# AdrienC21/CCSD

Measured on AMD Instinct MI355X. Metric: sampled complexes/sec at 1000 PC steps, QM9_CC batch=1024, 1/2/4/8 GPU, higher is better.
Workload: dtype f32; 1 GPU; qm9_CC N=9 F=4 E=36 K=466, B=1024 per GPU, VE x3, Reverse+Langevin snr=0.2 scale_eps=0.7 n_steps=1, 1000 scales; global_batch=1024, parallelism=batch-sharded x1, per-shard Langevin norms, all-gather at end, finite=True

## Files before the change

### ccsd_amd/_lib.py

```python
from __future__ import annotations

import ctypes as C
import os
from typing import Optional

HERE = os.path.dirname(os.path.abspath(__file__))
HIP_LIB_PATH = os.path.join(HERE, "libccsd_hip.so")

ABI_VERSION = 5
OK, ERR_INVALID, ERR_UNSUPPORTED, ERR_WEIGHTS, ERR_RUNTIME, ERR_WORKSPACE = range(6)
SDE_VP, SDE_VE, SDE_SUBVP = 0, 1, 2
PRED_EULER, PRED_REVERSE, PRED_S4 = 0, 1, 2
CORR_NONE, CORR_LANGEVIN = 0, 1
TARGET_X, TARGET_ADJ, TARGET_RANK2 = 0, 1, 2

EXPORTS = [
    "ccsd_plan_create", "ccsd_plan_destroy", "ccsd_weight_count", "ccsd_rank2_dims", "ccsd_workspace_bytes",
    "ccsd_last_error", "ccsd_score", "ccsd_init_state", "ccsd_corrector_norms", "ccsd_corrector_apply",
    "ccsd_predictor", "ccsd_s4_apply", "ccsd_sampler_run", "ccsd_quantize", "ccsd_rank2_cells", "ccsd_profile_kernel", "ccsd_profile_stride", "ccsd_profile_read", "ccsd_profile_launches", "ccsd_debug_stamps",
    "ccsd_noise_draws", "ccsd_plan_query",
]
QUERIES = {"fused_r2": 0, "xa_variant": 1, "r2_lds_bytes": 2, "xa_lds_bytes": 3, "fused_loop": 4, "merged_r2": 5, "ew1": 6, "large_graph": 7,
           "r2_family": 8, "r2_instance": 9, "loop_form": 10, "h_full": 11, "hp_full": 12, "p0_narrow": 13, "tiled_fuse": 14, "ew1_fuse": 15,
           "h_general": 16, "geo_ek": 17}
KERNEL_IDS = {"k_xa": 0, "k_gemm_p": 1, "k_hf_score": 2, "k_gemm_h": 3, "k_langevin_apply": 4, "k_r2": 5, "k_s4_apply": 6, "k_ew1": 7}


class StepCoef(C.Structure):
    _fields_ = [(n, C.c_float) for n in ("sscale", "alpha", "pa", "pb", "pc", "m1", "s1", "d", "m2", "s2")]


class Config(C.Structure):
    _fields_ = (
        [(n, C.c_int32) for n in (
            "abi_version", "N", "F", "is_cc", "d_min", "d_max",
            "x_depth", "x_nhid",
            "a_num_layers", "a_num_linears", "a_c_init", "a_c_hid", "a_c_final", "a_nhid", "a_adim", "a_num_heads",
            "a_is_cc_net", "h_num_layers", "h_num_linears", "h_nhid", "h_adim", "h_c_hid", "h_c_final", "h_num_heads",
            "f_num_layers", "f_num_linears", "f_nhid", "f_c_hid", "f_c_final", "f_cnum", "f_num_layers_mlp",
            "f_use_hodge_mask",
            "predictor", "corrector", "n_corr_steps", "probability_flow", "denoise")]
        + [("snr", C.c_float), ("scale_eps", C.c_float), ("diff_steps", C.c_int32), ("batch_hint", C.c_int32)]
        + [(n, C.c_int32) for n in ("x_gmh", "x_num_linears", "x_c_init", "x_c_hid", "x_c_final", "x_adim", "x_num_heads",
                                    "a_conv_mlp", "x_conv_mlp")]
    )


class State(C.Structure):
    _fields_ = [("x", C.c_void_p), ("adj", C.c_void_p), ("rank2", C.c_void_p)]


class Noise(C.Structure):
    _fields_ = [("zx", C.c_void_p), ("zadj", C.c_void_p), ("zrank2", C.c_void_p)]


class CcsdError(RuntimeError):
    pass


def raise_status(lib, status: int):
    if status == OK:
        return
    msg = lib.ccsd_last_error().decode("utf-8", "replace")
    if status == ERR_UNSUPPORTED:
        raise NotImplementedError(msg)
    if status in (ERR_INVALID, ERR_WEIGHTS, ERR_WORKSPACE):
        raise ValueError(msg)
    raise CcsdError(msg)


class Library:

    def __init__(self, path: str, is_hip: bool):
        if not os.path.exists(path):
            raise FileNotFoundError(path)
        self.path = path
        self.is_hip = is_hip
        L = self.c = C.CDLL(path)
        vp, i32, i64, u64, f32, sz = C.c_void_p, C.c_int32, C.c_int64, C.c_uint64, C.c_float, C.c_size_t
        P = C.POINTER
        L.ccsd_plan_create.argtypes = [P(Config), P(C.c_float), sz, P(StepCoef), P(vp)]
        L.ccsd_plan_create.restype = C.c_int
        L.ccsd_plan_destroy.argtypes = [vp]
        L.ccsd_plan_destroy.restype = None
        L.ccsd_weight_count.argtypes = [P(Config)]
        L.ccsd_weight_count.restype = sz
        L.ccsd_rank2_dims.argtypes = [P(Config), P(i32), P(i64)]
        L.ccsd_rank2_dims.restype = None
        L.ccsd_workspace_bytes.argtypes = [vp, i32]
        L.ccsd_workspace_bytes.restype = sz
        L.ccsd_last_error.argtypes = []
        L.ccsd_last_error.restype = C.c_char_p
        L.ccsd_score.argtypes = [vp, i32, i32, P(State), vp, f32, vp, vp, sz, vp]
        L.ccsd_score.restype = C.c_int
        L.ccsd_init_state.argtypes = [vp, i32, vp, P(Noise), u64, i64, P(State), vp]
        L.ccsd_init_state.restype = C.c_int
        L.ccsd_corrector_norms.argtypes = [vp, i32, i32, i32, P(State), P(State), vp, P(Noise), u64, i64, vp, vp, sz, vp]
        L.ccsd_corrector_norms.restype = C.c_int
        L.ccsd_corrector_apply.argtypes = [vp, i32, i32, i32, P(State), vp, P(Noise), u64, i64, vp, P(State), vp, sz, vp]
        L.ccsd_corrector_apply.restype = C.c_int
        L.ccsd_predictor.argtypes = [vp, i32, i32, P(State), vp, P(Noise), u64, i64, P(State), P(State), vp, sz, vp]
        L.ccsd_predictor.restype = C.c_int
        L.ccsd_s4_apply.argtypes = [vp, i32, i32, P(State), vp, P(Noise), P(Noise), P(Noise), u64, i64, vp, P(State), P(State), vp, sz, vp]
        L.ccsd_s4_apply.restype = C.c_int
        L.ccsd_sampler_run.argtypes = [vp, i32, vp, u64, i64, i32, i32, P(State), P(State), P(State), vp, vp, sz, vp]
        L.ccsd_sampler_run.restype = C.c_int
        L.ccsd_quantize.argtypes = [vp, i64, f32, vp, vp]
        L.ccsd_quantize.restype = C.c_int
        L.ccsd_rank2_cells.argtypes = [vp, i32, i32, i64, f32, vp, vp, vp]
        L.ccsd_rank2_cells.restype = C.c_int
        L.ccsd_profile_kernel.argtypes = [vp, i32]
        L.ccsd_profile_kernel.restype = C.c_int
        L.ccsd_profile_stride.argtypes = [vp, i32]
        L.ccsd_profile_stride.restype = C.c_int
        L.ccsd_profile_read.argtypes = [vp, i32, P(i64), P(C.c_double)]
        L.ccsd_profile_read.restype = C.c_int
        L.ccsd_profile_launches.argtypes = [vp, i32, P(i64)]
        L.ccsd_profile_launches.restype = C.c_int
        L.ccsd_debug_stamps.argtypes = [vp, vp]
        L.ccsd_debug_stamps.restype = C.c_int
        L.ccsd_noise_draws.argtypes = [vp, i32, vp, u64, i64, i32, i32, P(State), vp]
        L.ccsd_noise_draws.restype = C.c_int
        L.ccsd_plan_query.argtypes = [vp, i32, P(i64)]
        L.ccsd_plan_query.restype = C.c_int

    def __getattr__(self, name):
        return getattr(self.c, name)

    def check(self, status: int):
        raise_status(self.c, status)


_hip: Optional[Library] = None


def get_library() -> Library:
    global _hip
    if _hip is None:
        import torch

        path = os.environ.get("CCSD_LIB_PATH") or HIP_LIB_PATH
        if not os.path.exists(path):
            raise CcsdError(
                f"{path} is missing: build it with `python -c 'import __graft_entry__ as g; g.build()'` "
                "(hipcc --offload-arch=gfx950).  ccsd_amd has no CPU fallback."
            )
        _hip = Library(path, is_hip=True)
    return _hip
```

### ccsd_amd/csrc/ccsd_api.h

```cpp
#pragma once
#include "ccsd_kernels.h"
#define CCSD_INST_TABLES
#include "ccsd_instances.h"
#include <stdio.h>
#include <stdlib.h>
#include <string>
#include <vector>

static thread_local std::string g_last_error;
static int set_err(int st, const std::string& m) { g_last_error = m; return st; }

static inline int fnet_width(const PlanD& p) {
    int fw = p.f_fdim > p.f_cnum ? p.f_fdim : p.f_cnum;
    for (int l = 0; l < p.f_L; ++l) {
        const MlpD& m = p.fl[l];
        const int wd = m.n > 1 && m.hid > m.in ? (m.hid > m.out ? m.hid : m.out) : (m.in > m.out ? m.in : m.out);
        if (wd > fw) fw = wd;
    }
    if (p.f_fin.n > 1 && p.f_fin.hid > fw) fw = p.f_fin.hid;
    return fw;
}

struct Knobs {
    int no_fused_r2 = 0, hodge_general = 0, geo_off = 0, no_fused_apply = 0, no_h_full = 0, no_hp_full = 0, hp_full_norms = 0, split_bf16 = 0;
    int xa_threads = 0, xa_prio = 0, xa_stagger_mask = 0, xa_stagger_sleep = 0, r2_stagger_mask = 0, r2_stagger_sleep = 0;
    int lg_force = 0, xa_pass = -1, xa_gch = 0, no_mlp_wt = 0, verbose = 0;
    const char *dump_plan = nullptr, *dump_plan_name = nullptr;
};
static Knobs read_knobs() {
    Knobs k;
    auto on = [](const char* name) { return getenv(name) != nullptr; };
    k.no_fused_r2 = on("CCSD_NO_FUSED_R2"); k.hodge_general = on("CCSD_HODGE_GENERAL");
    k.geo_off = on("CCSD_NO_GEO") ? 1 : on("CCSD_NO_BAKE") ? 2 : 0;
    k.no_fused_apply = on("CCSD_NO_FUSED_APPLY"); k.no_h_full = on("CCSD_NO_H_FULL"); k.no_hp_full = on("CCSD_NO_HP_FULL");
    k.hp_full_norms = on("CCSD_HP_FULL_NORMS");
    if (const char* v = getenv("CCSD_SPLIT_BF16")) k.split_bf16 = atoi(v) == 3 ? 3 : 0;
    if (const char* v = getenv("CCSD_XA_THREADS")) { const int t = atoi(v); if (t >= 64 && t <= 1024 && t % 64 == 0) k.xa_threads = t; }
    if (const char* v = getenv("CCSD_XA_PRIO")) k.xa_prio = atoi(v);
    if (const char* v = getenv("CCSD_XA_STAGGER")) sscanf(v, "%d,%d", &k.xa_stagger_mask, &k.xa_stagger_sleep);
    if (const char* v = getenv("CCSD_R2_STAGGER")) sscanf(v, "%d,%d", &k.r2_stagger_mask, &k.r2_stagger_sleep);
    if (const char* v = getenv("CCSD_LARGE_GRAPH")) k.lg_force = atoi(v) == 1;
    if (const char* v = getenv("CCSD_XA_PASS")) k.xa_pass = atoi(v);
    k.xa_gch = on("CCSD_XA_GCH"); k.no_mlp_wt = on("CCSD_NO_MLP_WT"); k.verbose = on("CCSD_VERBOSE");
    k.dump_plan = getenv("CCSD_DUMP_PLAN"); k.dump_plan_name = getenv("CCSD_DUMP_PLAN_NAME");
    return k;
}

enum { R2_NONE = 0, R2_FUSED = 1, R2_EW1 = 2, R2_TILED = 3 };
enum { LOOP_PRED_ONLY = 0, LOOP_LANGEVIN = 1, LOOP_LANGEVIN_FUSED = 2, LOOP_S4 = 3, LOOP_STEPWISE = 4 };
struct Route {
    int lg = 0;
    int xa_variant = 0;
    const XaEntry* xa = nullptr;
    const XaEntry* xa_twin = nullptr;
    int xa_threads = 0;
    int r2_family = R2_NONE;
    const R2Entry* r2 = nullptr;
    int r2_ldk = 0, r2_ldh = 0;
    size_t r2_lds = 0;
    int h_general = 0;
    int geo = 0;
    int p0 = -1;
    int h_full = 0;
    unsigned hp_full_modes = 0;
    int loop = LOOP_PRED_ONLY;
    int merged = 0;
    int tiled_fuse = 0;
    int ew1_fuse = 0;
    int corrector_flat = 0, predictor_flat = 0;
};

struct ccsd_plan {
    ccsd_config_t cfg;
    PlanD h;
    PlanD* d = nullptr;
    float* w = nullptr;
    float* wp = nullptr;
    unsigned char* hpairs = nullptr;
    size_t npacked = 0;
    unsigned char* edges = nullptr;
    unsigned long long* cells = nullptr;
    std::vector<ccsd_step_coef_t> coef;
    size_t nweights = 0;
    long long* dbg = nullptr;
    unsigned long long* init_off = nullptr;
    size_t init_off_cap = 0;
    Knobs knobs;
    Route rt;
    unsigned prof_mask = 0;
    size_t prof_used[8] = {0, 0, 0, 0, 0, 0, 0, 0};
    int prof_stride = 1;
    size_t prof_calls[8] = {0, 0, 0, 0, 0, 0, 0, 0};
#ifndef CCSD_EMU
    std::vector<hipEvent_t> prof_ev[8];
#endif
};

enum { KID_XA = 0, KID_GEMM_P = 1, KID_HF = 2, KID_GEMM_H = 3, KID_LANGEVIN = 4, KID_R2 = 5, KID_S4 = 6, KID_EW1 = 7 };
static void prof_mark(ccsd_plan* pl, int kid, void* stream) {
#ifndef CCSD_EMU
    if (!(pl->prof_mask & (1u << kid))) return;
    const size_t call = pl->prof_calls[kid]++;
    if (pl->prof_stride > 1 && (call >> 1) % (size_t)pl->prof_stride != 0) return;
    std::vector<hipEvent_t>& ev = pl->prof_ev[kid];
    if (pl->prof_used[kid] == ev.size()) {
        hipEvent_t e;
        if (hipEventCreate(&e) != hipSuccess) return;
        ev.push_back(e);
    }
    (void)hipEventRecord(ev[pl->prof_used[kid]++], (hipStream_t)stream);
#else
    (void)pl; (void)kid; (void)stream;
#endif
}
#define RT_CHECK(expr)                                                                    \
    do {                                                                                  \
        rtError_t _e = (expr);                                                            \
        if (_e != RT_OK) return set_err(CCSD_ERR_RUNTIME, std::string(#expr) + ": " + rt_error_string(_e)); \
    } while (0)
#define LAUNCH_CHECK()                                                                    \
    do {                                                                                  \
        rtError_t _e = rt_last_error();                                                   \
        if (_e != RT_OK) return set_err(CCSD_ERR_RUNTIME, std::string("kernel launch: ") + rt_error_string(_e)); \
    } while (0)

static int resolve_route(ccsd_plan* pl) {
    const PlanD& p = pl->h;
    const ccsd_config_t& c = pl->cfg;
    const Knobs& k = pl->knobs;
    Route& r = pl->rt;
    const int E = p.E, K = p.K;
    const bool s4 = c.predictor == CCSD_PRED_S4, langevin = c.corrector == CCSD_CORR_LANGEVIN;
    unsigned char arch[sizeof(PlanD)];
    ccsd_plan_arch_bytes(p, arch);
    auto baked = [&](const unsigned char* plan, size_t size) { return size == sizeof(PlanD) && p.geo_off == 0 && memcmp(arch, plan, size) == 0; };

    bool conv_mlp = false;
    for (int l = 0; l < p.a_L; ++l) conv_mlp = conv_mlp || p.al[l].conv_mlp;
    if (p.x_gmh) for (int l = 0; l < p.x_depth; ++l) conv_mlp = conv_mlp || p.gl[l].conv_mlp;
    int v = p.hb_L ? XA_HB : p.x_gmh ? XA_GMH : XA_PLAIN;
    if (conv_mlp || (p.hb_L && p.x_gmh) || p.h_L > 2 || (!p.chan_global && !p.hb_L && p.a_fin.chain >= 5)) v = XA_GEN;
    if (v == XA_PLAIN && !p.chan_global && baked(CCSD_BAKED_QM9_PLAN, CCSD_BAKED_QM9_SIZE)) v = XA_BAKED9;
    else if (v == XA_PLAIN && p.chan_global && baked(CCSD_BAKED_CS_PLAN, CCSD_BAKED_CS_SIZE)) v = XA_BAKED20;
    else if (v == XA_PLAIN && p.chan_global && baked(CCSD_BAKED_Z_PLAN, CCSD_BAKED_Z_SIZE)) v = XA_BAKED38;
    else if (v == XA_GEN && !p.chan_global && baked(CCSD_BAKED_ENZ_PLAN, CCSD_BAKED_ENZ_SIZE)) v = XA_BAKEDENZ;
    else if (v == XA_PLAIN && p.geo_off != 1)
        for (const auto& g : XA_GEO_TABLE)
            if ((p.chan_global != 0) == (g.gch != 0) && p.N == g.N && (!g.F || p.F == g.F) && E == g.E && p.ldn == g.ldn) v = g.var;
    r.xa_variant = v;
    r.xa_threads = k.xa_threads;
    for (const XaEntry& e : XA_TABLE) {
        if ((e.gch != 0) != (p.chan_global != 0)) continue;
        if (e.var == v) r.xa = &e;
        if (e.var == XA_PLAIN) r.xa_twin = &e;
    }
    if (!r.xa || !r.xa_twin) return set_err(CCSD_ERR_RUNTIME, "k_xa variant " + std::to_string(v) + " has no instance in CCSD_XA_LIST");
    if (!r.xa->fixed256) r.xa_twin = nullptr;

    const bool aff = p.f_affine != 0, gen1 = p.h_L > 1 && p.hl[0].mval.n > 1;
    const int mt = (E + 15) / 16, rem = E & 15, rs = (!aff || rem == 0 || rem > 12) ? 0 : (rem + 3) / 4;
    auto r2_find = [&](int qm9) -> const R2Entry* {
        for (const R2Entry& e : R2_TABLE)
            if (e.mt == mt && e.rs == rs && (e.affine != 0) == aff && (e.gen1 != 0) == gen1 && e.qm9 == qm9) return &e;
        return nullptr;
    };
    bool fused = false;
    if (c.is_cc && E <= 64 && !k.no_fused_r2) {
        const int Kp4 = (K + 31) & ~31, Ep4 = (E + 3) & ~3;
        int ldk = Kp4; while ((ldk & 31) != 8 && (ldk & 31) != 24) ldk += 4;
        const int ldh = Ep4;
        const size_t fl = (size_t)E * ldk + (size_t)E * ldh + 64 * 2 + (size_t)p.a_cinit * E + 3 * c.N * c.N + 64 + (Kp4 + 3) / 4 + 4;
        if (fl * 4 + 64 <= 160 * 1024 && fnet_width(p) <= CCSD_FW && r2_find(0) && p.f_cnum <= 2) {
            fused = true; r.r2_ldk = ldk; r.r2_ldh = ldh; r.r2_lds = fl * 4;
            const bool qm9 = p.geo_off != 1 && !gen1 && E == CCSD_R2_QM9_E && K == CCSD_R2_QM9_K && p.N == CCSD_R2_QM9_N &&
                             ldk == CCSD_R2_QM9_LDK && ldh == CCSD_R2_QM9_LDH;
            r.r2 = r2_find(!qm9 ? 0 : aff && baked(CCSD_BAKED_QM9_PLAN, CCSD_BAKED_QM9_SIZE) ? 2 : 1);
            if (!r.r2) return set_err(CCSD_ERR_RUNTIME, "k_r2: the qm9-geometry instance is missing from CCSD_R2_LIST_*");
        }
    }
    if (p.h_L > 2) {
        bool affine_values = true;
        for (int l = 0; l + 1 < p.h_L; ++l) affine_values = affine_values && ccsd_hl(p, l).mval.n == 1;
        if (!affine_values || !fused || p.h_L > 4 || k.hodge_general) { r.h_general = 1; fused = false; r.r2 = nullptr; }
    }
    const bool ew1 = c.is_cc && !fused && aff && p.f_cnum == 1 && !s4;
    r.r2_family = !c.is_cc ? R2_NONE : fused ? R2_FUSED : ew1 ? R2_EW1 : R2_TILED;
    if (p.geo_off != 1) for (const GeoEntry& g : GEO_TABLE) if (E == g.E && K == g.K) r.geo = g.idx;
    if (p.h_L >= 1) {
        auto p0_find = [&](int kc) {
            for (int i = 0; i < (int)(sizeof(P0_TABLE) / sizeof(P0_TABLE[0])); ++i)
                if (P0_TABLE[i].nt == (p.hl[0].wc + 15) / 16 && P0_TABLE[i].kc == kc) return i;
            return -1;
        };
        if (p.geo_off != 1) r.p0 = p0_find(K);
        if (r.p0 < 0) r.p0 = p0_find(0);
    }
    r.tiled_fuse = r.r2_family == R2_TILED && p.h_L == 1 && (K & 3) == 0 && !s4 && langevin;
    r.ew1_fuse = ew1 && p.h_L == 1 && (K & 3) == 0 && langevin;
    const bool full_geo = c.is_cc && E == CCSD_FULL_E && K == CCSD_FULL_K && p.geo_off != 1 && !k.no_h_full;
    r.h_full = full_geo && r.r2_family == R2_TILED && p.f_cnum >= 2;

    const bool fused_apply = (fused || (ew1 && p.h_L <= 1) || r.tiled_fuse) && !k.no_fused_apply;
    r.loop = s4 ? LOOP_S4 : !langevin ? LOOP_PRED_ONLY : c.n_corr_steps != 1 ? LOOP_STEPWISE : fused_apply ? LOOP_LANGEVIN_FUSED : LOOP_LANGEVIN;
    if (full_geo && r.tiled_fuse && p.hl[0].wc <= 16 && p.f_cnum == 2 && !k.no_hp_full)
        r.hp_full_modes = (r.loop == LOOP_LANGEVIN_FUSED ? 1u << 2 : 0u) | (k.hp_full_norms ? 1u << 1 : 0u);
    r.merged = r.loop == LOOP_LANGEVIN_FUSED && fused && mt == 3 && rs == 1 && aff && !gen1 && (K & 1) == 0 && ((E * K) & 3) == 0;
    r.corrector_flat = !s4;
    r.predictor_flat = ew1;
    return CCSD_OK;
}
static inline bool use_h_full(const Route& r, int B) { return r.h_full && B >= 256; }
static inline bool use_hp_full(const Route& r, int B, int mode) { return B >= 256 && ((r.hp_full_modes >> mode) & 1u); }
#define HP_FULL_LDS ((size_t)(2 * 192 * H_LD + 2 * 16 * H_LD) * 4)
static inline const XaEntry* xa_launch(const Route& r, int B, int* threads) {
    const XaEntry* e = r.xa;
    int t = r.xa_threads;
    if (t == 0) t = e->max_threads == 256 ? 256 : B <= 256 ? 1024 : B <= 512 ? 512 : 256;
    if (e->fixed256 && t != 256) e = r.xa_twin;
    *threads = t > e->max_threads ? e->max_threads : t;
    return e;
}
static inline int normsum_threads(int B) { return B > 512 ? 1024 : B > 256 ? 512 : 256; }

extern "C" const char* ccsd_last_error(void) { return g_last_error.c_str(); }

extern "C" void ccsd_rank2_dims(const ccsd_config_t* cfg, int32_t* E, int64_t* K) {
    int e = 0; int64_t k = 0;
    if (cfg) ccsd_dims(cfg, &e, &k);
    if (E) *E = e;
    if (K) *K = k;
}

extern "C" size_t ccsd_weight_count(const ccsd_config_t* cfg) {
    PlanD p; PlanBuilder pb;
    size_t n = ccsd_build_plan(cfg, &p, pb);
    if (pb.status != CCSD_OK) { set_err(pb.status, pb.err); return 0; }
    return n;
}

extern "C" int ccsd_debug_stamps(ccsd_plan_t* plan, void* dev_buffer) {
    if (!plan) return set_err(CCSD_ERR_INVALID, "NULL plan");
    plan->dbg = (long long*)dev_buffer;
    return CCSD_OK;
}
extern "C" int ccsd_profile_kernel(ccsd_plan_t* plan, int32_t kernel_id) {
    if (!plan) return set_err(CCSD_ERR_INVALID, "NULL plan");
    if (kernel_id < 0) plan->prof_mask = 0;
    else if (kernel_id < 8) plan->prof_mask |= 1u << kernel_id;
    for (int k = 0; k < 8; ++k) { plan->prof_used[k] = 0; plan->prof_calls[k] = 0; }
    return CCSD_OK;
}
extern "C" int ccsd_profile_stride(ccsd_plan_t* plan, int32_t stride) {
    if (!plan || stride < 1) return set_err(CCSD_ERR_INVALID, "bad argument");
    plan->prof_stride = stride;
    for (int k = 0; k < 8; ++k) plan->prof_calls[k] = 0;
    return CCSD_OK;
}
extern "C" int ccsd_profile_launches(ccsd_plan_t* plan, int32_t kernel_id, int64_t* launches) {
    if (!plan || !launches || kernel_id < 0 || kernel_id >= 8) return set_err(CCSD_ERR_INVALID, "bad argument");
    *launches = (int64_t)(plan->prof_calls[kernel_id] >> 1);
    return CCSD_OK;
}
extern "C" int ccsd_profile_read(ccsd_plan_t* plan, int32_t kernel_id, int64_t* launches, double* total_ms) {
    if (!plan || !launches || !total_ms || kernel_id < 0 || kernel_id >= 8) return set_err(CCSD_ERR_INVALID, "bad argument");
    *launches = 0; *total_ms = 0.0;
#ifndef CCSD_EMU
    for (size_t i = 0; i + 1 < plan->prof_used[kernel_id]; i += 2) {
        float ms = 0.f;
        RT_CHECK(hipEventSynchronize(plan->prof_ev[kernel_id][i + 1]));
        RT_CHECK(hipEventElapsedTime(&ms, plan->prof_ev[kernel_id][i], plan->prof_ev[kernel_id][i + 1]));
        *total_ms += ms; *launches += 1;
    }
#endif
    plan->prof_used[kernel_id] = 0;
    return CCSD_OK;
}

extern "C" void ccsd_plan_destroy(ccsd_plan_t* plan) {
    if (!plan) return;
#ifndef CCSD_EMU
    for (int k = 0; k < 8; ++k) for (hipEvent_t e : plan->prof_ev[k]) (void)hipEventDestroy(e);
#endif
    if (plan->d) (void)rt_free(plan->d);
    if (plan->w) (void)rt_free(plan->w);
    if (plan->wp) (void)rt_free(plan->wp);
    if (plan->hpairs) (void)rt_free(plan->hpairs);
    if (plan->edges) (void)rt_free(plan->edges);
    if (plan->cells) (void)rt_free(plan->cells);
    if (plan->init_off) (void)rt_free(plan->init_off);
    delete plan;
}

extern "C" int ccsd_plan_create(const ccsd_config_t* cfg, const float* weights, size_t n_weights,
                                const ccsd_step_coef_t* step_coef, ccsd_plan_t** out) {
    if (!cfg || !weights || !step_coef || !out) return set_err(CCSD_ERR_INVALID, "NULL argument");
    *out = nullptr;
    ccsd_plan* pl = new ccsd_plan();
    pl->cfg = *cfg;
    const Knobs& k = pl->knobs = read_knobs();
    PlanBuilder pb;
    pb.lg_force = k.lg_force; pb.xa_pass = k.xa_pass; pb.xa_gch = k.xa_gch; pb.no_mlp_wt = k.no_mlp_wt; pb.verbose = k.verbose;
    pl->nweights = ccsd_build_plan(cfg, &pl->h, pb);
    if (pb.status != CCSD_OK) { delete pl; return set_err(pb.status, pb.err); }
    pl->rt.lg = pb.lg;
    pl->h.geo_off = k.geo_off;
    pl->npacked = (size_t)pb.pcur;
    if (pl->nweights != n_weights) {
        delete pl;
        return set_err(CCSD_ERR_WEIGHTS, "weight blob has " + std::to_string(n_weights) + " floats, config needs " +
                                             std::to_string(pl->nweights));
    }
    if (cfg->predictor != CCSD_PRED_EULER && cfg->predictor != CCSD_PRED_REVERSE && cfg->predictor != CCSD_PRED_S4) { delete pl; return set_err(CCSD_ERR_UNSUPPORTED, "unknown predictor"); }
    if (cfg->corrector != CCSD_CORR_NONE && cfg->corrector != CCSD_CORR_LANGEVIN) { delete pl; return set_err(CCSD_ERR_UNSUPPORTED, "unknown corrector"); }
    if (cfg->diff_steps < 1 || cfg->n_corr_steps < 0) { delete pl; return set_err(CCSD_ERR_INVALID, "bad step counts"); }
    ccsd_fold_fnet(&pl->h, weights);
    pl->coef.assign(step_coef, step_coef + (size_t)cfg->diff_steps * 3);
    const int N = cfg->N, E = pl->h.E, K = pl->h.K;
    std::vector<unsigned char> edges((size_t)2 * E + 2);
    {
        int e = 0;
        for (int i = 0; i < N; ++i)
            for (int j = i + 1; j < N; ++j) { edges[2 * e] = (unsigned char)i; edges[2 * e + 1] = (unsigned char)j; ++e; }
    }
    std::vector<unsigned long long> cells((size_t)K + 1);
    if (cfg->is_cc) {
        size_t c = 0;
        std::vector<int> idx;
        for (int k = cfg->d_min; k <= cfg->d_max; ++k) {
            idx.resize(k);
            for (int i = 0; i < k; ++i) idx[i] = i;
            while (true) {
                unsigned long long m = 0;
                for (int i = 0; i < k; ++i) m |= 1ull << idx[i];
                cells[c++] = m;
                int i = k - 1;
                while (i >= 0 && idx[i] == N - k + i) --i;
                if (i < 0) break;
                ++idx[i];
                for (int j = i + 1; j < k; ++j) idx[j] = idx[j - 1] + 1;
            }
        }
        if ((int)c != K) { delete pl; return set_err(CCSD_ERR_INVALID, "cell enumeration mismatch"); }
    }
#define PC(expr) do { rtError_t _e = (expr); if (_e != RT_OK) { ccsd_plan_destroy(pl); return set_err(CCSD_ERR_RUNTIME, std::string(#expr) + ": " + rt_error_string(_e)); } } while (0)
    PC(rt_malloc((void**)&pl->d, sizeof(PlanD)));
    PC(rt_h2d(pl->d, &pl->h, sizeof(PlanD)));
    {
        const size_t wtotal = pl->h.f_blk >= 0 ? (size_t)pl->h.f_blk + CCSD_FBLK_FLOATS : n_weights;
        PC(rt_malloc((void**)&pl->w, wtotal * sizeof(float)));
        PC(rt_h2d(pl->w, weights, n_weights * sizeof(float)));
        if (pl->h.f_blk >= 0) {
            std::vector<float> blk(CCSD_FBLK_FLOATS);
            ccsd_pack_fnet_blocks(&pl->h, weights, blk.data());
            PC(rt_h2d(pl->w + pl->h.f_blk, blk.data(), blk.size() * sizeof(float)));
        }
    }
    {
        std::vector<float> packed(pl->npacked + 4, 0.f);
        ccsd_pack_mlp(pl->h.x_fin, weights, packed.data());
        for (int l = 0; l < pl->h.a_L; ++l) {
            ccsd_pack_mlp(pl->h.al[l].mlp, weights, packed.data()); ccsd_pack_mlp(pl->h.al[l].mc, weights, packed.data());
            ccsd_pack_qkv(pl->h.al[l], weights, packed.data()); ccsd_pack_mc(pl->h.al[l], weights, packed.data());
        }
        if (pl->h.x_gmh) for (int l = 0; l < pl->h.x_depth; ++l) {
            ccsd_pack_mlp(pl->h.gl[l].mlp, weights, packed.data()); ccsd_pack_mlp(pl->h.gl[l].mc, weights, packed.data());
            ccsd_pack_qkv(pl->h.gl[l], weights, packed.data()); ccsd_pack_mc(pl->h.gl[l], weights, packed.data());
        }
        if (pl->h.hb_L) ccsd_pack_mlp(pl->h.hb[0].mh, weights, packed.data());
        for (int l = 0; l < pl->h.hb_L; ++l) {
            const HodgeBaseD& h = pl->h.hb[l];
            for (int c = 0; c < h.cin; ++c) {
                const float* blk = weights + h.blk_base + (size_t)c * h.blk_stride;
                const float* w2 = blk + h.hid * E + h.hid;
                for (int e = 0; e < E; ++e)
                    for (int hh = 0; hh < h.hid; ++hh) {
                        packed[(size_t)h.w2t + ((size_t)c * h.hid + hh) * E + e] = w2[e * h.hid + hh];
                        packed[(size_t)h.w1t + ((size_t)c * E + e) * h.hid + hh] = blk[hh * E + e];
                    }
            }
        }
        ccsd_pack_mlp(pl->h.a_fin, weights, packed.data());
        for (int l = 0; l < pl->h.h_L; ++l) {
            const HodgeLayerD& h = ccsd_hl(pl->h, l);
            const int Kp = (K + 31) & ~31;
            for (int k = 0; k < K; ++k)
                for (int n = 0; n < h.wc; ++n) packed[(size_t)h.wcatT + (size_t)n * Kp + k] = weights[(size_t)h.wcat + (size_t)k * h.wc + n];
        }
        PC(rt_malloc((void**)&pl->wp, packed.size() * sizeof(float)));
        PC(rt_h2d(pl->wp, packed.data(), packed.size() * sizeof(float)));
    }
    if (pl->h.h_L > 1) {
        if (E > 255) { ccsd_plan_destroy(pl); return set_err(CCSD_ERR_UNSUPPORTED, "dense hodge layer needs E <= 255"); }
        std::vector<unsigned char> hp;
        for (int e = 0; e < E; ++e)
            for (int e2 = e; e2 < E; ++e2) { hp.push_back((unsigned char)e); hp.push_back((unsigned char)e2); }
        PC(rt_malloc((void**)&pl->hpairs, hp.size()));
        PC(rt_h2d(pl->hpairs, hp.data(), hp.size()));
    }
    PC(rt_malloc((void**)&pl->edges, edges.size()));
    PC(rt_h2d(pl->edges, edges.data(), edges.size()));
    PC(rt_malloc((void**)&pl->cells, cells.size() * sizeof(unsigned long long)));
    PC(rt_h2d(pl->cells, cells.data(), cells.size() * sizeof(unsigned long long)));
    if (int st = resolve_route(pl)) { ccsd_plan_destroy(pl); return st; }
    {
        const Route& r = pl->rt;
        const size_t xlds = (size_t)pl->h.xa_lds_floats * 4;
        if (xlds > 64 * 1024) {
            PC(rt_set_max_dyn_smem((const void*)r.xa->fn, xlds));
            if (r.xa_twin) PC(rt_set_max_dyn_smem((const void*)r.xa_twin->fn, xlds));
        }
        if (r.r2 && r.r2_lds > 64 * 1024) PC(rt_set_max_dyn_smem((const void*)r.r2->fn, r.r2_lds));
        if (r.lg && lg_nmlp_lds(pl->h) > 64 * 1024) PC(rt_set_max_dyn_smem((const void*)k_lg_nmlp, lg_nmlp_lds(pl->h)));
#ifndef CCSD_EMU
        if (r.hp_full_modes) {
            PC(rt_set_max_dyn_smem((const void*)k_hp_full<CCSD_FULL_E, CCSD_FULL_K, 1>, HP_FULL_LDS));
            PC(rt_set_max_dyn_smem((const void*)k_hp_full<CCSD_FULL_E, CCSD_FULL_K, 2>, HP_FULL_LDS));
        }
#endif
    }
#undef PC
    if (const char* path = k.dump_plan) {
        const char* nm = k.dump_plan_name ? k.dump_plan_name : "QM9";
        std::vector<unsigned char> bytes(sizeof(PlanD));
        ccsd_plan_arch_bytes(pl->h, bytes.data());
        if (FILE* f = fopen(path, "w")) {
            fprintf(f, "// GENERATED by tools/bake_plan.py (do not edit): the PlanD of a shipped configuration at its bench batch as a compile-time\n"
                       "// constant (architecture bytes: ccsd_plan_arch_bytes, the weight-derived affine fold zeroed).  The baked kernel instances read\n"
                       "// their plan from it instead of from memory; the host selects them only for plans whose architecture bytes are equal.\n"
                       "#pragma once\n#define CCSD_BAKED_%s_SIZE %zu\n#define CCSD_BAKED_%s_A_L %d      /* AttentionLayers of ScoreNetworkA: unroll count */\n"
                       "alignas(16) static constexpr unsigned char CCSD_BAKED_%s_PLAN[CCSD_BAKED_%s_SIZE] = {", nm, sizeof(PlanD), nm, pl->h.a_L, nm, nm);
            for (size_t i = 0; i < bytes.size(); ++i) fprintf(f, "%s%u,", (i % 40) ? "" : "\n    ", (unsigned)bytes[i]);
            fprintf(f, "\n};\n");
            fclose(f);
        }
    }
    *out = pl;
    return CCSD_OK;
}


#define CCSD_P_SPLITS 8

struct Workspace {
    unsigned long long* offbits;
    unsigned char *mfr, *mfl;
    int Kp, Ep;
    float *H, *P0, *P1, *U1, *acoef, *net_x, *net_adj, *net_r, *norm2, *part, *sums, *chan, *zpart, *part2;
    float* psplit; size_t psplit_floats;
    float *P0b, *P1b, *U1b;
    int ntiles, nchunk;
    float *hgH, *hgR[2], *hgP[CCSD_MAXHL + CCSD_MAXHLX - 1];
    size_t hg_hstride;
    float *lg_S, *lg_att, *lg_dis, *lg_Y, *lg_QKV, *lg_x[2], *lg_xcat, *lg_xY, *lg_xnet, *lg_part;
    int lg_tiles;
    size_t bytes;
};
struct Pass {
    const float* h_src = nullptr;
    int p1_raw = 0;
};
static inline int r2_p1_raw(const PlanD& p) { return p.h_L > 1 && p.hl[0].mval.n == 1; }
static Workspace carve_ws(const ccsd_plan* pl, int B, void* base) {
    const PlanD& p = pl->h;
    Workspace w{};
    size_t o = 0;
    auto take = [&](size_t nbytes) { size_t r = o; o += (nbytes + 255) / 256 * 256; return base ? (char*)base + r : (char*)nullptr; };
    w.offbits = (unsigned long long*)take((size_t)B * 8);
    const size_t E = p.E, K = p.K;
    w.Kp = p.is_cc ? (p.K + 3) & ~3 : 0; w.Ep = p.is_cc ? (p.E + 3) & ~3 : 0;
    w.mfr = (unsigned char*)take((size_t)B * w.Kp);
    w.mfl = (unsigned char*)take((size_t)B * w.Ep);
    w.H = (float*)take(p.is_cc ? (size_t)B * E * h_ld((int)E) * 4 * (p.f_cnum > 2 ? p.f_cnum - 1 : 1) : 0);
    w.P0 = (float*)take(p.h_L > 0 ? (size_t)B * E * p.hl[0].wc * 4 : 0);
    w.P1 = (float*)take(p.h_L > 1 ? (size_t)B * E * p.h_pw * 4 : 0);
    w.U1 = (float*)take(p.h_L > 1 ? (size_t)B * p.h_pw * 4 : 0);
    w.psplit_floats = p.h_L > 1 ? (size_t)CCSD_P_SPLITS * B * E * p.h_pw : 0;
    w.psplit = (float*)take(w.psplit_floats * 4);
    const bool two = pl->rt.r2_family == R2_FUSED;
    w.P0b = (float*)take(two && p.h_L > 0 ? (size_t)B * E * p.hl[0].wc * 4 : 0);
    w.P1b = (float*)take(two && p.h_L > 1 ? (size_t)B * E * p.h_pw * 4 : 0);
    w.U1b = (float*)take(two && p.h_L > 1 ? (size_t)B * p.h_pw * 4 : 0);
    w.acoef = (float*)take(p.h_L > 1 ? (size_t)B * p.a_cinit * E * 4 : 0);
    if (pl->rt.h_general) {
        int cmax = 1;
        for (int l = 0; l + 1 < p.h_L; ++l) cmax = ccsd_hl(p, l).cout > cmax ? ccsd_hl(p, l).cout : cmax;
        w.hg_hstride = (size_t)cmax * E * E;
        w.hgH = (float*)take((size_t)B * w.hg_hstride * 4);
        w.hgR[0] = (float*)take((size_t)B * E * K * 4);
        w.hgR[1] = (float*)take((size_t)B * E * K * 4);
        for (int l = 1; l < p.h_L; ++l) w.hgP[l - 1] = (float*)take((size_t)B * E * ccsd_hl(p, l).wc * 4);
    }
    w.net_x = (float*)take((size_t)B * p.N * p.F * 4);
    w.net_adj = (float*)take((size_t)B * p.N * p.N * 4);
    w.net_r = (float*)take(p.is_cc ? (size_t)B * E * K * 4 : 0);
    w.norm2 = (float*)take((size_t)B * 4 * 4);
    w.ntiles = p.is_cc ? ((p.K + T_BN - 1) / T_BN) * ((p.E + T_BM - 1) / T_BM) : 0;
    w.nchunk = p.is_cc ? (int)((((size_t)p.E * p.K + 3) / 4 + CCSD_NN_CH - 1) / CCSD_NN_CH) : 0;
    { int np = w.ntiles > w.nchunk ? w.ntiles : w.nchunk; if ((int)E > np) np = (int)E;
      w.part = (float*)take((size_t)B * (np ? np : 1) * 2 * 4); }
    w.zpart = (float*)take((size_t)B * ((size_t)w.nchunk > E ? (size_t)w.nchunk : E ? E : 1) * 4);
    w.part2 = (float*)take((size_t)B * 2 * 4);
    w.sums = (float*)take(64);
    w.chan = (float*)take(p.chan_global ? (size_t)B * p.chan_rows * p.N * p.N * 4 : 0);
    if (pl->rt.lg) {
        const size_t N = p.N, NN = N * N;
        int cin = 1, cp = 1, fx = p.F > p.x_nhid ? p.F : p.x_nhid;
        for (int l = 0; l < p.a_L; ++l) {
            if (p.al[l].cin > cin) cin = p.al[l].cin;
            if (p.al[l].cp > cp) cp = p.al[l].cp;
            if (p.al[l].fout > fx) fx = p.al[l].fout;
        }
        w.lg_tiles = (int)((NN + CCSD_LG_FIN_ROWS - 1) / CCSD_LG_FIN_ROWS);
        w.lg_S = (float*)take((size_t)B * p.a_fdim * NN * 4);
        w.lg_att = (float*)take((size_t)B * cin * NN * 4);
        w.lg_dis = (float*)take((size_t)B * cin * N * 4);
        w.lg_Y = (float*)take((size_t)B * cin * N * cp * 4);
        w.lg_QKV = (float*)take((size_t)B * cin * N * cp * 4);
        w.lg_x[0] = (float*)take((size_t)B * N * fx * 4);
        w.lg_x[1] = (float*)take((size_t)B * N * fx * 4);
        w.lg_xcat = (float*)take((size_t)B * N * p.x_fdim * 4);
        w.lg_xY = (float*)take((size_t)B * N * p.x_nhid * 4);
        w.lg_xnet = (float*)take((size_t)B * N * p.F * 4);
        w.lg_part = (float*)take((size_t)B * w.lg_tiles * 2 * 4);
    }
    w.bytes = o;
    return w;
}
extern "C" size_t ccsd_workspace_bytes(const ccsd_plan_t* plan, int32_t B) {
    if (!plan || B < 1) return 0;
    return carve_ws(plan, B, nullptr).bytes;
}

static int grid_for(long long n, int block) {
    long long g = (n + block - 1) / block;
    if (g > 2048) g = 2048;
    if (g < 1) g = 1;
    return (int)g;
}

static int check_common(const ccsd_plan* pl, int B, const void* flags, const void* ws, size_t ws_bytes) {
    if (!pl) return set_err(CCSD_ERR_INVALID, "NULL plan");
    if (B < 1) return set_err(CCSD_ERR_INVALID, "B must be >= 1");
    if (!flags) return set_err(CCSD_ERR_INVALID, "NULL flags");
    if (!ws || ws_bytes < carve_ws(pl, B, nullptr).bytes) return set_err(CCSD_ERR_WORKSPACE, "workspace too small");
    return CCSD_OK;
}
static int check_state(const ccsd_plan* pl, const ccsd_state_t* s, const char* what) {
    if (!s || !s->x || !s->adj || (pl->h.is_cc && !s->rank2)) return set_err(CCSD_ERR_INVALID, std::string("NULL tensor in ") + what);
    return CCSD_OK;
}

static int launch_flagbits(const ccsd_plan* pl, int B, const float* flags, Workspace& w, void* stream) {
    if (pl->rt.lg) return CCSD_OK;
    CCSD_LAUNCH(k_flagbits, dim3(grid_for(B, 256)), dim3(CCSD_NTHREADS), 0, stream, flags, w.offbits, B, pl->h.N);
    LAUNCH_CHECK();
    if (pl->h.is_cc) {
        CCSD_LAUNCH(k_masktab, dim3(grid_for((long long)B * (w.Kp + w.Ep), 256)), dim3(CCSD_NTHREADS), 0, stream,
                    (const unsigned long long*)w.offbits, (const unsigned char*)pl->edges, (const unsigned long long*)pl->cells, w.mfr, w.mfl,
                    B, pl->h.E, pl->h.K, w.Kp, w.Ep);
        LAUNCH_CHECK();
    }
    return CCSD_OK;
}

static int launch_h(const ccsd_plan* pl, int B, const float* rank2, Pass& ps, Workspace& w, void* stream) {
    const PlanD& p = pl->h;
    if (!p.is_cc || p.f_cnum < 2) return CCSD_OK;
    if (ps.h_src == rank2) return CCSD_OK;
    const bool full = use_h_full(pl->rt, B);
    const int nth_ = (p.E + T_BM - 1) / T_BM;
    dim3 g(xcd_grid(B, nth_ * (nth_ + 1) / 2));
    prof_mark(const_cast<ccsd_plan*>(pl), KID_GEMM_H, stream);
#ifndef CCSD_EMU
    if (full && pl->knobs.split_bf16 == 3) hipLaunchKernelGGL((k_gemm_h_full<CCSD_FULL_E, CCSD_FULL_K, 2>), dim3(B), dim3(256), 0, (hipStream_t)stream, rank2, w.H, p.f_hmask);
    else if (full) hipLaunchKernelGGL((k_gemm_h_full<CCSD_FULL_E, CCSD_FULL_K>), dim3(B), dim3(256), 0, (hipStream_t)stream, rank2, w.H, p.f_hmask);
    else
#endif
    {
        (void)full;
#define H_GO(EC_, KC_) CCSD_LAUNCH((k_gemm_h<EC_, KC_>), g, dim3(CCSD_NTHREADS), 0, stream, rank2, w.H, p.E, p.K, p.f_hmask, B)
        GEO_EK(pl->rt.geo, H_GO);
#undef H_GO
    }
    prof_mark(const_cast<ccsd_plan*>(pl), KID_GEMM_H, stream);
    LAUNCH_CHECK();
    for (int j = 2; j < p.f_cnum; ++j) {
        const size_t slab = (size_t)B * p.E * h_ld(p.E);
        const int nt = (p.E + 15) / 16, per = CCSD_NTHREADS >= 64 ? CCSD_NTHREADS / 64 : 1;
        CCSD_LAUNCH(k_gemm_pow, dim3((nt * nt + per - 1) / per, 1, B), dim3(CCSD_NTHREADS), 0, stream,
                    (const float*)(w.H + (size_t)(j - 2) * slab), (const float*)w.H, w.H + (size_t)(j - 1) * slab, p.E);
        LAUNCH_CHECK();
    }
    return CCSD_OK;
}
struct RankEpi;
static int launch_r2(const ccsd_plan* pl, int B, const float* rank2, const float* adj, const float* flags, int want_p,
                     RankEpi& ep, NoiseArgs& na, Pass& ps, Workspace& w, void* stream, const CorrFuse* cf, int merge_draw);
static int launch_p(const ccsd_plan* pl, int B, const float* adj, const float* rank2, Pass& ps, Workspace& w, void* stream, const P0Fuse* fuse = nullptr) {
    const PlanD& p = pl->h;
    const Route& rt = pl->rt;
    if (p.h_L < 1) return CCSD_OK;
    if (p.h_L > 2 && !rt.h_general) {
        RankEpi ep{};
        ep.mode = MODE_SCORE; ep.sscale = 0.f; ep.out = w.net_r;
        NoiseArgs na0{};
        return launch_r2(pl, B, rank2, adj, nullptr, 1, ep, na0, ps, w, stream, nullptr, -1);
    }
    ps.p1_raw = 0;
    const int rows = B * p.E;
    const bool hp_full = fuse && use_hp_full(rt, B, fuse->mode);
#ifndef CCSD_EMU
    if (hp_full) {
        const HodgeLayerD& h = p.hl[0];
        const float* WT = (const float*)pl->wp + h.wcatT;
        prof_mark(const_cast<ccsd_plan*>(pl), KID_GEMM_H, stream);
        if (fuse->mode == 1)
            hipLaunchKernelGGL((k_hp_full<CCSD_FULL_E, CCSD_FULL_K, 1>), dim3(B), dim3(512), HP_FULL_LDS, (hipStream_t)stream, rank2, WT, w.H, w.P0, h.wc, p.f_hmask, *fuse);
        else
            hipLaunchKernelGGL((k_hp_full<CCSD_FULL_E, CCSD_FULL_K, 2>), dim3(B), dim3(512), HP_FULL_LDS, (hipStream_t)stream, rank2, WT, w.H, w.P0, h.wc, p.f_hmask, *fuse);
        prof_mark(const_cast<ccsd_plan*>(pl), KID_GEMM_H, stream);
        LAUNCH_CHECK();
        ps.h_src = fuse->mode == 2 ? fuse->f1 : rank2;
        return CCSD_OK;
    }
#endif
    (void)hp_full;
    {
        const HodgeLayerD& h = p.hl[0];
        dim3 g((h.wc + T_BN - 1) / T_BN, (rows + T_BM - 1) / T_BM, 1);
        prof_mark(const_cast<ccsd_plan*>(pl), KID_GEMM_P, stream);
        P0Fuse pf{};
        if (fuse) pf = *fuse;
#ifndef CCSD_EMU
        if (rt.p0 >= 0)
            hipLaunchKernelGGL(P0_TABLE[rt.p0].fn[pf.mode], dim3((rows + T_BM - 1) / T_BM), dim3(256), 0, (hipStream_t)stream, rank2,
                               (const float*)pl->wp + h.wcatT, w.P0, rows, p.K, (p.K + 31) & ~31, h.wc, pf);
        else
#endif
        {
            const float* src = rank2;
            if (pf.mode) {
                CCSD_LAUNCH(k_p0_fuse_ew, dim3(grid_for(rows, 256)), dim3(CCSD_NTHREADS), 0, stream, rank2, pf, rows, p.K);
                LAUNCH_CHECK();
                if (pf.mode == 2 || pf.mode == 4) src = pf.f1;
            }
            CCSD_LAUNCH(k_gemm_p, g, dim3(CCSD_NTHREADS), 0, stream, src, (const float*)pl->w, w.P0, rows, p.E, p.K, h.wc,
                        h.wcat, 0, h.mval, h.cin, (const float*)nullptr, (const unsigned long long*)w.offbits,
                        (const unsigned char*)pl->edges, (const unsigned long long*)pl->cells, p.K);
        }
        prof_mark(const_cast<ccsd_plan*>(pl), KID_GEMM_P, stream);
        LAUNCH_CHECK();
    }
    if (p.h_L > 1) {
        CCSD_LAUNCH(k_edgecoef, dim3(B), dim3(CCSD_NTHREADS), (size_t)3 * p.N * p.N * 4, stream, adj, w.acoef, p.N, p.E,
                    p.a_cinit, (const unsigned char*)pl->edges);
        LAUNCH_CHECK();
        const HodgeLayerD& h0 = p.hl[0];
        const HodgeLayerD& h = p.hl[1];
        dim3 g((h.wc + T_BN - 1) / T_BN, (rows + T_BM - 1) / T_BM, 1);
        const int nslab = (p.K + T_BK - 1) / T_BK;
        int S = CCSD_P_SPLITS < nslab ? CCSD_P_SPLITS : nslab;
        if ((size_t)S * rows * h.wc > w.psplit_floats) S = 1;
        const int kchunk = ((nslab + S - 1) / S) * T_BK;
        S = (p.K + kchunk - 1) / kchunk;
        g.z = S;
        float* P1 = rt.h_general ? w.hgP[0] : w.P1;
        CCSD_LAUNCH(k_gemm_p, g, dim3(CCSD_NTHREADS), 0, stream, rank2, (const float*)pl->w, S > 1 ? w.psplit : P1, rows, p.E, p.K, h.wc,
                    h.wcat, 1, h0.mval, h0.cin, (const float*)w.acoef, (const unsigned long long*)w.offbits,
                    (const unsigned char*)pl->edges, (const unsigned long long*)pl->cells, kchunk);
        LAUNCH_CHECK();
        if (S > 1) {
            const long long n = (long long)rows * h.wc;
            CCSD_LAUNCH(k_sum_splits, dim3(grid_for(n, 256)), dim3(CCSD_NTHREADS), 0, stream, (const float*)w.psplit, P1, n, S);
            LAUNCH_CHECK();
        }
        if (rt.h_general) {
            const int cw = p.E > 128 ? 32 : 64;
            CCSD_LAUNCH(k_hodge_value, dim3((p.K + cw - 1) / cw, B), dim3(CCSD_NTHREADS), (size_t)p.E * cw * 4, stream, rank2, (const float*)nullptr, 0,
                        (const float*)w.acoef, (const float*)pl->w, h0.mval, h0.cin, w.hgR[0], p.E, p.K, cw,
                        (const unsigned long long*)w.offbits, (const unsigned char*)pl->edges, (const unsigned long long*)pl->cells);
            LAUNCH_CHECK();
        }
    }
    return CCSD_OK;
}
static int launch_lg(const ccsd_plan* pl, int B, XaArgs& xa, NoiseArgs& na, Workspace& w, void* stream);
static int launch_xa(const ccsd_plan* pl, int B, XaArgs& xa, NoiseArgs& na, const Pass& ps, Workspace& w, void* stream, bool set_b = false) {
    const Route& rt = pl->rt;
    if (rt.lg) return launch_lg(pl, B, xa, na, w, stream);
    xa.P0 = set_b ? w.P0b : w.P0; xa.P1 = set_b ? w.P1b : w.P1; xa.U1 = set_b ? w.U1b : w.U1; xa.chan_ws = w.chan;
    xa.p1_raw = ps.p1_raw; xa.dbg = pl->dbg ? pl->dbg + 32 : nullptr;
    xa.stagger_mask = pl->knobs.xa_stagger_mask; xa.stagger_sleep = pl->knobs.xa_stagger_sleep; xa.prio_mode = pl->knobs.xa_prio;
    int xa_threads;
    const XaEntry* inst = xa_launch(rt, B, &xa_threads);
    prof_mark(const_cast<ccsd_plan*>(pl), KID_XA, stream);
    xa.wp = pl->wp; xa.hpairs = pl->hpairs;
    const dim3 xblk(CCSD_NTHREADS == 1 ? 1 : xa_threads);
    const size_t xlds = (size_t)pl->h.xa_lds_floats * 4;
#define XA_LAUNCH(XA_) CCSD_LAUNCH(inst->fn, dim3(B), xblk, xlds, stream, (const PlanD*)pl->d, (const float*)pl->w, (const unsigned char*)pl->edges, XA_, na)
    if (rt.h_general) {
        const PlanD& p = pl->h;
        if (rt.xa_variant != XA_GEN) return set_err(CCSD_ERR_RUNTIME, "general hodge stack needs k_xa<., XA_GEN>");
        xa.pdirect = 1;
        for (int l = 1; l < p.h_L; ++l) xa.Pd[l - 1] = w.hgP[l - 1];
        const int rows = B * p.E;
        for (int l = 2; l < p.h_L; ++l) {
            XaArgs pre = xa;
            pre.hdump_layer = l - 1; pre.hdump = w.hgH; pre.hdump_stride = (int)w.hg_hstride;
            XA_LAUNCH(pre);
            LAUNCH_CHECK();
            const HodgeLayerD& hp = ccsd_hl(p, l - 1);
            const HodgeLayerD& h = ccsd_hl(p, l);
            float* Rl = w.hgR[(l - 1) & 1];
            const int cw = p.E > 128 ? 32 : 64;
            CCSD_LAUNCH(k_hodge_value, dim3((p.K + cw - 1) / cw, B), dim3(CCSD_NTHREADS), (size_t)p.E * cw * 4, stream, (const float*)w.hgR[(l - 2) & 1],
                        (const float*)w.hgH, (int)w.hg_hstride, (const float*)nullptr, (const float*)pl->w, hp.mval, hp.cin, Rl, p.E, p.K, cw,
                        (const unsigned long long*)w.offbits, (const unsigned char*)pl->edges, (const unsigned long long*)pl->cells);
            LAUNCH_CHECK();
            CCSD_LAUNCH(k_gemm_p, dim3((h.wc + T_BN - 1) / T_BN, (rows + T_BM - 1) / T_BM, 1), dim3(CCSD_NTHREADS), 0, stream, (const float*)Rl,
                        (const float*)pl->w, w.hgP[l - 1], rows, p.E, p.K, h.wc, h.wcat, 0, h.mval, h.cin, (const float*)nullptr,
                        (const unsigned long long*)w.offbits, (const unsigned char*)pl->edges, (const unsigned long long*)pl->cells, p.K);
            LAUNCH_CHECK();
        }
    }
    XA_LAUNCH(xa);
#undef XA_LAUNCH
    prof_mark(const_cast<ccsd_plan*>(pl), KID_XA, stream);
    LAUNCH_CHECK();
    return CCSD_OK;
}
static int launch_lg(const ccsd_plan* pl, int B, XaArgs& xa, NoiseArgs& na, Workspace& w, void* stream) {
    const PlanD& p = pl->h;
    if (xa.cf.on) return set_err(CCSD_ERR_RUNTIME, "tiled graph-network route: no fused corrector apply");
    const int N = p.N, F = p.F, NN = N * N, H = p.x_nhid, XF = p.x_fdim;
    const int rt = (N + 15) / 16, gt = (N + CCSD_LG_GT - 1) / CCSD_LG_GT, at = (N + CCSD_LG_AT - 1) / CCSD_LG_AT;
    const dim3 blk(CCSD_NTHREADS);
    auto cdiv = [](int a, int b_) { return (a + b_ - 1) / b_; };
    prof_mark(const_cast<ccsd_plan*>(pl), KID_XA, stream);
    if (xa.do_x) {
        CCSD_LAUNCH(k_lg_dis, dim3(grid_for(N, 256), B), blk, 0, stream, xa.adjX, (long long)NN, 0, 1, N, w.lg_dis);
        CCSD_LAUNCH(k_lg_put, dim3(grid_for((long long)B * N * F, 256)), blk, 0, stream, xa.xX, F, w.lg_xcat, XF, B * N);
        for (int l = 0; l < p.x_depth; ++l) {
            const int fin = l ? H : F;
            const float* src = l ? w.lg_xcat + F + (l - 1) * H : xa.xX;
            CCSD_LAUNCH(k_lg_xw, dim3(grid_for((long long)N * H, 256), B), blk, 0, stream, src, (long long)N * (l ? XF : F), l ? XF : F, fin,
                        (const float*)pl->w + p.x_gw[l], 0, H, 1, N, (const float*)w.lg_dis, w.lg_xY);
            CCSD_LAUNCH(k_lg_gcn, dim3(gt * cdiv(H, CCSD_LG_GT), 1, B), blk, 0, stream, xa.adjX, (long long)NN, 0, (const float*)w.lg_xY,
                        (const float*)w.lg_dis, (const float*)pl->w + p.x_gb[l], 0, H, H, 1, N, w.lg_xcat, (long long)N * XF, 0, XF, F + l * H, 1);
        }
        CCSD_LAUNCH(k_lg_nmlp, dim3(rt, B), blk, lg_nmlp_lds_of(p.x_fin), stream, p.x_fin, (const float*)pl->w,
                    (LgGather{w.lg_xcat, (long long)N * XF, 0, XF, 0, XF}), N, xa.flags, 0, w.lg_xnet);
        LAUNCH_CHECK();
    }
    if (xa.do_a) {
        const long long ss = (long long)p.a_fdim * NN;
        for (int c = 0; c < p.a_cinit; ++c)
            CCSD_LAUNCH(k_lg_pow, dim3(grid_for(NN, 256), B), blk, 0, stream, xa.adjA, w.lg_S, ss, N, c);
        for (int l = 0; l < p.a_L; ++l) {
            const AttnLayerD& L = p.al[l];
            const float* xin = l ? w.lg_x[(l - 1) & 1] : xa.xA;
            const float* wq = pl->wp + L.qkvp;
            const int wcs = L.fin * L.cp + L.cp;
            CCSD_LAUNCH(k_lg_dis, dim3(grid_for((long long)L.cin * N, 256), B), blk, 0, stream, (const float*)w.lg_S, ss, L.ci0, L.cin, N, w.lg_dis);
            CCSD_LAUNCH(k_lg_xw, dim3(grid_for((long long)L.cin * N * L.cp, 256), B), blk, 0, stream, xin, (long long)N * L.fin, L.fin, L.fin,
                        wq, wcs, L.cp, L.cin, N, (const float*)w.lg_dis, w.lg_Y);
            CCSD_LAUNCH(k_lg_gcn, dim3(gt * cdiv(L.cp, CCSD_LG_GT), L.cin, B), blk, 0, stream, (const float*)w.lg_S, ss, L.ci0, (const float*)w.lg_Y,
                        (const float*)w.lg_dis, wq + L.fin * L.cp, wcs, L.cp, L.cp, L.cin, N, w.lg_QKV, (long long)L.cin * N * L.cp, N * L.cp, L.cp, 0, 0);
            CCSD_LAUNCH(k_lg_nmlp, dim3(rt, B), blk, lg_nmlp_lds_of(L.mc), stream, L.mc, (const float*)pl->w,
                        (LgGather{w.lg_QKV, (long long)L.cin * N * L.cp, N * L.cp, L.cp, 2 * L.adim, L.fout}), N, xa.flags, 1, w.lg_x[l & 1]);
            const float inv_scale = (float)sqrt((double)L.fout);
            CCSD_LAUNCH(k_lg_att, dim3(at * at, L.cin, B), blk, 0, stream, (const float*)w.lg_QKV, L.cp, L.adim, L.nchunk, L.dsplit, 1.0f / inv_scale,
                        0.5f / (float)L.nchunk, L.cin, N, w.lg_att);
            CCSD_LAUNCH(k_lg_edge, dim3(w.lg_tiles, B), blk, 0, stream, L.mlp, (const float*)pl->wp, (const float*)w.lg_att, w.lg_S, ss, L.ci0, L.co0,
                        L.cin, N);
            CCSD_LAUNCH(k_lg_sym, dim3(grid_for((long long)L.cout * NN, 256), B), blk, 0, stream, w.lg_S, ss, L.co0, L.cout, N, xa.flags);
            LAUNCH_CHECK();
        }
        CCSD_LAUNCH(k_lg_fin, dim3(w.lg_tiles, B), blk, 0, stream, p.a_fin, (const float*)pl->wp, (const float*)w.lg_S, ss, N, xa.flags, xa.adjA,
                    xa, na, w.lg_part);
        LAUNCH_CHECK();
    }
    CCSD_LAUNCH(k_lg_epi, dim3(B), blk, 0, stream, (const float*)w.lg_xnet, xa.xX, xa.flags, xa, na, (const float*)w.lg_part, w.lg_tiles, N, F);
    prof_mark(const_cast<ccsd_plan*>(pl), KID_XA, stream);
    LAUNCH_CHECK();
    return CCSD_OK;
}

static int launch_hf(const ccsd_plan* pl, int B, const float* rank2, RankEpi& ep, NoiseArgs& na, Workspace& w, void* stream) {
    const PlanD& p = pl->h;
    dim3 g(xcd_grid(B, ((p.K + T_BN - 1) / T_BN) * ((p.E + T_BM - 1) / T_BM)));
    prof_mark(const_cast<ccsd_plan*>(pl), KID_HF, stream);
#define HF_ARGS (const PlanD*)pl->d, (const float*)pl->w, rank2, (const float*)w.H, (const unsigned long long*)w.offbits, \
                (const unsigned char*)pl->edges, (const unsigned long long*)pl->cells, ep, na, B, (MaskTab{w.mfr, w.mfl, w.Kp, w.Ep})
    const int fw = fnet_width(p);
#define HF_AFF1(EC_, KC_) CCSD_LAUNCH((k_hf_score<true, 8, 1, EC_, KC_>), g, dim3(CCSD_NTHREADS), 0, stream, HF_ARGS)
#define HF_GEN1(EC_, KC_) CCSD_LAUNCH((k_hf_score<false, 8, 1, EC_, KC_>), g, dim3(CCSD_NTHREADS), 0, stream, HF_ARGS)
#define HF_GO(NP_) \
    do { \
        if (p.f_affine && NP_ == 1) GEO_EK(pl->rt.geo, HF_AFF1); \
        else if (p.f_affine) CCSD_LAUNCH((k_hf_score<true, 8, NP_>), g, dim3(CCSD_NTHREADS), 0, stream, HF_ARGS); \
        else if (fw <= 8 && NP_ == 1) GEO_EK(pl->rt.geo, HF_GEN1); \
        else if (fw <= 8) CCSD_LAUNCH((k_hf_score<false, 8, NP_>), g, dim3(CCSD_NTHREADS), 0, stream, HF_ARGS); \
        else if (fw <= CCSD_FW) CCSD_LAUNCH((k_hf_score<false, CCSD_FW, NP_>), g, dim3(CCSD_NTHREADS), 0, stream, HF_ARGS); \
        else CCSD_LAUNCH((k_hf_score<false, CCSD_FWMAX, NP_>), g, dim3(CCSD_NTHREADS), 0, stream, HF_ARGS); \
    } while (0)
    if (p.f_cnum <= 2) HF_GO(1); else HF_GO(CCSD_MAXCN - 1);
#undef HF_GO
#undef HF_AFF1
#undef HF_GEN1
#undef HF_ARGS
    prof_mark(const_cast<ccsd_plan*>(pl), KID_HF, stream);
    LAUNCH_CHECK();
    return CCSD_OK;
}

static int launch_ew1(const ccsd_plan* pl, int B, const float* rank2, RankEpi& ep, NoiseArgs& na, Workspace& w, void* stream,
                      float* net_out = nullptr, const CorrFuse* cf = nullptr, float* f1 = nullptr) {
    const PlanD& p = pl->h;
    Ew1Args a{};
    a.r = rank2; a.out = ep.out; a.mean = ep.mean; a.f1 = f1; a.net_out = net_out; a.part = ep.part;
    a.mode = ep.mode; a.apply = (cf && cf->on) ? 1 : 0;
    a.sscale = ep.sscale; a.pa = ep.pa; a.pb = ep.pb; a.pc = ep.pc; a.alpha = p.f_alpha; a.gamma = p.f_gamma;
    if (a.apply) { a.sums = cf->sums; a.ss = cf->ss[2]; a.sde_alpha = cf->alpha[2]; a.snr = cf->snr; a.seps = cf->seps; a.draw_corr = cf->draw_r; }
    a.E = p.E; a.K = p.K; a.mt = MaskTab{w.mfr, w.mfl, w.Kp, w.Ep};
    prof_mark(const_cast<ccsd_plan*>(pl), KID_EW1, stream);
#define EW1_GO(EC_, KC_) CCSD_LAUNCH((k_ew1<EC_, KC_>), dim3(w.nchunk, B), dim3(CCSD_NTHREADS), 0, stream, a, na)
    GEO_EK(pl->rt.geo, EW1_GO);
#undef EW1_GO
    prof_mark(const_cast<ccsd_plan*>(pl), KID_EW1, stream);
    LAUNCH_CHECK();
    return CCSD_OK;
}

static int launch_r2(const ccsd_plan* pl, int B, const float* rank2, const float* adj, const float* flags, int want_p,
                     RankEpi& ep, NoiseArgs& na, Pass& ps, Workspace& w, void* stream, const CorrFuse* cf = nullptr, int merge_draw = -1) {
    const Route& rt = pl->rt;
    R2Args ra{};
    if (cf) ra.cf = *cf;
    ra.masked = (cf && cf->on) ? 1 : 0;
    if (merge_draw >= 0) {
        ra.merge = 1; ra.draw_r2 = (unsigned)merge_draw;
        ra.P0b = w.P0b; ra.P1b = w.P1b; ra.U1b = w.U1b; ra.net2 = w.net_r; ra.part2 = w.part;
    }
    ra.rank2 = rank2; ra.adj = adj; ra.flags = flags; ra.offbits = w.offbits; ra.P0 = w.P0; ra.P1 = w.P1; ra.U1 = w.U1; ra.want_p = want_p;
    ra.ldk = rt.r2_ldk; ra.ldh = rt.r2_ldh; ra.dbg = pl->dbg; ra.wp = pl->wp;
    ra.stagger_mask = pl->knobs.r2_stagger_mask; ra.stagger_sleep = pl->knobs.r2_stagger_sleep;
    if (want_p && pl->h.h_L > 1) ps.p1_raw = r2_p1_raw(pl->h);
    prof_mark(const_cast<ccsd_plan*>(pl), KID_R2, stream);
    CCSD_LAUNCH(rt.r2->fn, dim3(B), dim3(CCSD_NTHREADS == 1 ? 1 : 512), rt.r2_lds, stream, (const PlanD*)pl->d, (const float*)pl->w,
                (const unsigned char*)pl->edges, (const unsigned long long*)pl->cells, ra, ep, na);
    prof_mark(const_cast<ccsd_plan*>(pl), KID_R2, stream);
    LAUNCH_CHECK();
    return CCSD_OK;
}

static unsigned int draw_base(const ccsd_plan* pl, int step, int phase) {
    const int per_step = pl->cfg.predictor == CCSD_PRED_S4 ? 3 : pl->cfg.n_corr_steps + 1;
    return 3u + (unsigned)((step * per_step + phase) * 3);
}
static NoiseArgs make_noise(const ccsd_noise_t* n, uint64_t seed, int64_t off, unsigned int base, int flat_r = 0) {
    NoiseArgs na{};
    if (n) { na.zx = n->zx; na.zadj = n->zadj; na.zr = n->zrank2; }
    na.seed = seed; na.b_off = off;
    na.draw_x = base; na.draw_adj = base + 1; na.draw_r = base + 2;
    na.flat_r = flat_r;
    return na;
}

extern "C" int ccsd_score(ccsd_plan_t* pl, int32_t target, int32_t B, const ccsd_state_t* in, const float* flags,
                          float sscale, float* out, void* workspace, size_t ws_bytes, void* stream) {
    int st = check_common(pl, B, flags, workspace, ws_bytes);
    if (st) return st;
    if ((st = check_state(pl, in, "in"))) return st;
    if (!out) return set_err(CCSD_ERR_INVALID, "NULL out");
    Workspace w = carve_ws(pl, B, workspace);
    if ((st = launch_flagbits(pl, B, flags, w, stream))) return st;
    NoiseArgs na{};
    Pass ps;
    if (target == CCSD_TARGET_X || target == CCSD_TARGET_ADJ) {
        XaArgs xa{};
        xa.xX = xa.xA = in->x; xa.adjX = xa.adjA = in->adj; xa.flags = flags;
        xa.do_x = target == CCSD_TARGET_X; xa.do_a = !xa.do_x; xa.mode = MODE_SCORE;
        xa.ss_x = xa.ss_a = sscale; xa.out_x = xa.out_a = out;
        if (xa.do_a && (st = launch_p(pl, B, in->adj, in->rank2, ps, w, stream))) return st;
        return launch_xa(pl, B, xa, na, ps, w, stream);
    }
    if (target == CCSD_TARGET_RANK2) {
        if (!pl->h.is_cc) return set_err(CCSD_ERR_INVALID, "rank2 score requested from a graph-only plan");
        RankEpi ep{};
        ep.mode = MODE_SCORE; ep.sscale = sscale; ep.out = out;
        if (pl->rt.r2_family == R2_FUSED) return launch_r2(pl, B, in->rank2, in->adj, flags, 0, ep, na, ps, w, stream);
        if (pl->rt.r2_family == R2_EW1) return launch_ew1(pl, B, in->rank2, ep, na, w, stream);
        if ((st = launch_h(pl, B, in->rank2, ps, w, stream))) return st;
        return launch_hf(pl, B, in->rank2, ep, na, w, stream);
    }
    return set_err(CCSD_ERR_UNSUPPORTED, "Object not yet supported. Select from [x, adj, rank2].");
}

static int draws_to_state(ccsd_plan* pl, int32_t B, const float* flags, const ccsd_noise_t* raw, uint64_t seed, int64_t sample_offset,
                          unsigned int base, ccsd_state_t* state, void* stream, int flat_r = 0) {
    if (!pl || B < 1 || !flags) return set_err(CCSD_ERR_INVALID, "bad argument");
    int st = check_state(pl, state, "state");
    if (st) return st;
    const PlanD& p = pl->h;
    if (pl->init_off_cap < (size_t)B) {
        if (pl->init_off) {
#ifndef CCSD_EMU
            (void)hipDeviceSynchronize();
#endif
            (void)rt_free(pl->init_off);
            pl->init_off = nullptr; pl->init_off_cap = 0;
        }
        RT_CHECK(rt_malloc((void**)&pl->init_off, (size_t)B * 8));
        pl->init_off_cap = (size_t)B;
    }
    unsigned long long* offbits = pl->init_off;
    if (!pl->rt.lg) CCSD_LAUNCH(k_flagbits, dim3(grid_for(B, 256)), dim3(CCSD_NTHREADS), 0, stream, flags, offbits, B, p.N);
    NoiseArgs na = make_noise(raw, seed, sample_offset, base, flat_r);
    const long long total = (long long)B * (p.N * p.F + p.N * p.N) +
                            (p.is_cc ? (flat_r ? (long long)B * (((long long)p.E * p.K + 3) / 4) : (long long)B * ((p.E + 3) / 4) * p.K) : 0);
    CCSD_LAUNCH(k_init_state, dim3(grid_for(total, 256)), dim3(CCSD_NTHREADS), 0, stream, state->x, state->adj, state->rank2,
                flags, na, (const unsigned long long*)offbits, (const unsigned char*)pl->edges,
                (const unsigned long long*)pl->cells, B, p.N, p.F, p.E, p.K, p.is_cc);
    LAUNCH_CHECK();
    return CCSD_OK;
}

extern "C" int ccsd_init_state(ccsd_plan_t* pl, int32_t B, const float* flags, const ccsd_noise_t* prior, uint64_t seed,
                               int64_t sample_offset, ccsd_state_t* state, void* stream) {
    return draws_to_state(pl, B, flags, prior, seed, sample_offset, 0, state, stream);
}

extern "C" int ccsd_noise_draws(ccsd_plan_t* pl, int32_t B, const float* flags, uint64_t seed, int64_t sample_offset, int32_t step,
                                int32_t phase, ccsd_state_t* out, void* stream) {
    if (!pl) return set_err(CCSD_ERR_INVALID, "NULL plan");
    const int per_step = pl->cfg.predictor == CCSD_PRED_S4 ? 3 : pl->cfg.n_corr_steps + 1;
    if (step < 0 || step >= pl->cfg.diff_steps || phase < 0 || phase >= per_step) return set_err(CCSD_ERR_INVALID, "step / phase out of range");
    const bool corr = pl->cfg.predictor != CCSD_PRED_S4 && phase < pl->cfg.n_corr_steps && pl->cfg.corrector == CCSD_CORR_LANGEVIN;
    return draws_to_state(pl, B, flags, nullptr, seed, sample_offset, draw_base(pl, step, phase), out, stream,
                          corr ? pl->rt.corrector_flat : pl->rt.predictor_flat);
}

extern "C" int ccsd_plan_query(const ccsd_plan_t* pl, int32_t what, int64_t* value) {
    if (!pl || !value) return set_err(CCSD_ERR_INVALID, "NULL argument");
    const Route& r = pl->rt;
    const int hint = pl->cfg.batch_hint;
    switch (what) {
        case CCSD_QUERY_FUSED_R2: *value = r.r2_family == R2_FUSED; break;
        case CCSD_QUERY_XA_VARIANT: *value = r.xa_variant; break;
        case CCSD_QUERY_R2_LDS_BYTES: *value = (int64_t)r.r2_lds; break;
        case CCSD_QUERY_XA_LDS_BYTES: *value = (int64_t)pl->h.xa_lds_floats * 4; break;
        case CCSD_QUERY_FUSED_LOOP: *value = r.loop == LOOP_LANGEVIN_FUSED; break;
        case CCSD_QUERY_MERGED_R2: *value = r.merged; break;
        case CCSD_QUERY_EW1: *value = r.r2_family == R2_EW1; break;
        case CCSD_QUERY_LARGE_GRAPH: *value = r.lg; break;
        case CCSD_QUERY_R2_FAMILY: *value = r.r2_family; break;
        case CCSD_QUERY_R2_INSTANCE: *value = r.r2 ? ((((int64_t)r.r2->mt * 10 + r.r2->rs) * 10 + r.r2->affine) * 10 + r.r2->gen1) * 10 + r.r2->qm9 : -1; break;
        case CCSD_QUERY_LOOP_FORM: *value = r.loop; break;
        case CCSD_QUERY_H_FULL: *value = use_h_full(r, hint); break;
        case CCSD_QUERY_HP_FULL: *value = (use_hp_full(r, hint, 2) ? 1 : 0) | (use_hp_full(r, hint, 1) ? 2 : 0); break;
        case CCSD_QUERY_P0_NARROW: *value = r.p0 >= 0 ? (int64_t)P0_TABLE[r.p0].nt * 100000 + P0_TABLE[r.p0].kc : 0; break;
        case CCSD_QUERY_TILED_FUSE: *value = r.tiled_fuse; break;
        case CCSD_QUERY_EW1_FUSE: *value = r.ew1_fuse; break;
        case CCSD_QUERY_H_GENERAL: *value = r.h_general; break;
        case CCSD_QUERY_GEO_EK: *value = r.geo; break;
        default: return set_err(CCSD_ERR_INVALID, "unknown query");
    }
    return CCSD_OK;
}

static int corrector_norms(ccsd_plan* pl, int B, int step, int it, const ccsd_state_t* base, const ccsd_state_t* cur,
                           const float* flags, const ccsd_noise_t* noise, uint64_t seed, int64_t off, float* sums,
                           Workspace& w, void* stream, bool keep_net = true, bool r2_done = false) {
    const PlanD& p = pl->h;
    int st;
    NoiseArgs na = make_noise(noise, seed, off, draw_base(pl, step, it), pl->rt.corrector_flat);
    const Route& rt = pl->rt;
    Pass ps;
    const bool fused = rt.r2_family == R2_FUSED && cur->rank2 == base->rank2;
    const bool zfuse = !fused && rt.tiled_fuse && na.flat_r && !na.zr;
    const bool e1fuse = !fused && rt.ew1_fuse && na.flat_r && !na.zr;
    int ntiles = w.ntiles;
    if (fused) {
        RankEpi ep{};
        ep.mode = MODE_NORMS; ep.out = w.net_r; ep.part = w.part;
        if (r2_done) ps.p1_raw = r2_p1_raw(p);
        else if ((st = launch_r2(pl, B, cur->rank2, cur->adj, flags, 1, ep, na, ps, w, stream))) return st;
        ntiles = 1;
    } else {
        P0Fuse pf{};
        if (zfuse) {
            pf.mode = 1; pf.zrow = w.zpart; pf.seed = na.seed; pf.b_off = na.b_off; pf.draw = na.draw_r;
            pf.mt = MaskTab{w.mfr, w.mfl, w.Kp, w.Ep}; pf.E = p.E;
        }
        if (e1fuse && cur->rank2 == base->rank2) {
            pf.mode = 3; pf.zrow = w.part; pf.seed = na.seed; pf.b_off = na.b_off; pf.draw = na.draw_r;
            pf.mt = MaskTab{w.mfr, w.mfl, w.Kp, w.Ep}; pf.E = p.E; pf.alpha = p.f_alpha; pf.gamma = p.f_gamma;
            pf.net_out = keep_net ? w.net_r : nullptr;
        }
        if ((st = launch_p(pl, B, cur->adj, base->rank2, ps, w, stream, pf.mode ? &pf : nullptr))) return st;
    }
    XaArgs xa{};
    xa.xX = cur->x; xa.adjX = base->adj;
    xa.xA = base->x; xa.adjA = cur->adj;
    xa.flags = flags; xa.do_x = xa.do_a = 1; xa.mode = MODE_NORMS;
    xa.out_x = w.net_x; xa.out_a = w.net_adj; xa.norm2 = w.norm2;
    if ((st = launch_xa(pl, B, xa, na, ps, w, stream, fused && r2_done))) return st;
    const bool ew1 = rt.r2_family == R2_EW1;
    if (p.is_cc && !fused && ew1 && e1fuse && cur->rank2 == base->rank2) {
        ntiles = p.E;
    } else if (p.is_cc && !fused && ew1) {
        RankEpi ep{};
        ep.mode = MODE_NORMS; ep.out = w.net_r; ep.part = w.part;
        if ((st = launch_ew1(pl, B, cur->rank2, ep, na, w, stream, keep_net ? w.net_r : nullptr))) return st;
        ntiles = w.nchunk;
    } else if (p.is_cc && !fused) {
        if ((st = launch_h(pl, B, cur->rank2, ps, w, stream))) return st;
        RankEpi ep{};
        ep.mode = MODE_NORMS; ep.out = w.net_r; ep.part = w.part;
        if ((st = launch_hf(pl, B, cur->rank2, ep, na, w, stream))) return st;
    }
    const float* part = w.part;
    if (p.is_cc && !fused) {
        const bool zk = na.flat_r && !na.zr && !ew1;
        if (zk && !zfuse) {
#define NN_GO(EC_, KC_) CCSD_LAUNCH((k_noise_norm<EC_, KC_>), dim3(w.nchunk, B), dim3(CCSD_NTHREADS), 0, stream, na, (MaskTab{w.mfr, w.mfl, w.Kp, w.Ep}), p.E, p.K, w.zpart)
            GEO_EK(pl->rt.geo, NN_GO);
#undef NN_GO
            LAUNCH_CHECK();
        }
        if (zk || ntiles > 8) {
            CCSD_LAUNCH(k_normpart, dim3(B), dim3(CCSD_NTHREADS), 0, stream, (const float*)w.part, ntiles, zk ? (const float*)w.zpart : (const float*)nullptr,
                        zfuse ? p.E : w.nchunk, w.part2);
            LAUNCH_CHECK();
            part = w.part2; ntiles = 1;
        }
    }
    CCSD_LAUNCH(k_normsum, dim3(1), dim3(CCSD_NTHREADS == 1 ? 1 : normsum_threads(B)), 0, stream, (const float*)w.norm2, part, B, ntiles,
                p.is_cc, sums);
    LAUNCH_CHECK();
    return CCSD_OK;
}
static int corrector_apply(ccsd_plan* pl, int B, int step, int it, const ccsd_state_t* cur, const float* flags,
                           const ccsd_noise_t* noise, uint64_t seed, int64_t off, const float* sums, ccsd_state_t* out,
                           Workspace& w, void* stream) {
    const PlanD& p = pl->h;
    NoiseArgs na = make_noise(noise, seed, off, draw_base(pl, step, it), pl->rt.corrector_flat);
    LangArgs a{};
    a.x = cur->x; a.adj = cur->adj; a.r = cur->rank2;
    a.nx = w.net_x; a.nadj = w.net_adj; a.nr = w.net_r;
    a.ox = out->x; a.oadj = out->adj; a.orr = out->rank2;
    a.flags = flags; a.sums = sums;
    for (int t = 0; t < 3; ++t) {
        const ccsd_step_coef_t& c = pl->coef[(size_t)step * 3 + t];
        a.ss[t] = c.sscale; a.alpha[t] = c.alpha;
    }
    a.snr = p.snr; a.seps = p.seps;
    a.B = B; a.N = p.N; a.F = p.F; a.E = p.E; a.K = p.K; a.is_cc = p.is_cc;
    const long long total = (long long)B * (p.N * p.F + p.N * p.N) + (p.is_cc ? (long long)B * (((long long)p.E * p.K + 3) / 4) : 0);
    prof_mark(pl, KID_LANGEVIN, stream);
#define LA_GO(EC_, KC_) CCSD_LAUNCH((k_langevin_apply<EC_, KC_>), dim3(grid_for(total, 256)), dim3(CCSD_NTHREADS), 0, stream, a, na, (MaskTab{w.mfr, w.mfl, w.Kp, w.Ep}))
    GEO_EK(pl->rt.geo, LA_GO);
#undef LA_GO
    prof_mark(pl, KID_LANGEVIN, stream);
    LAUNCH_CHECK();
    return CCSD_OK;
}
static int predictor(ccsd_plan* pl, int B, int step, const ccsd_state_t* in, const float* flags, const ccsd_noise_t* noise,
                     uint64_t seed, int64_t off, ccsd_state_t* out, ccsd_state_t* mean, Workspace& w, void* stream,
                     const float* fuse_sums = nullptr, bool merge_next = false) {
    const PlanD& p = pl->h;
    int st;
    NoiseArgs na = make_noise(noise, seed, off, draw_base(pl, step, pl->cfg.n_corr_steps), pl->rt.predictor_flat);
    const ccsd_step_coef_t* c = &pl->coef[(size_t)step * 3];
    const Route& rt = pl->rt;
    Pass ps;
    const bool fused = rt.r2_family == R2_FUSED, ew1 = rt.r2_family == R2_EW1;
    const float* r2_in = in->rank2;
    CorrFuse cf{};
    if (fuse_sums) {
        cf.on = 1; cf.net_x = w.net_x; cf.net_adj = w.net_adj; cf.net_r = w.net_r; cf.sums = fuse_sums;
        for (int t = 0; t < 3; ++t) { cf.ss[t] = c[t].sscale; cf.alpha[t] = c[t].alpha; }
        cf.snr = p.snr; cf.seps = p.seps;
        const unsigned int cb = draw_base(pl, step, 0);
        cf.draw_x = cb; cf.draw_adj = cb + 1; cf.draw_r = cb + 2;
    }
    if (fused) {
        RankEpi ep{};
        ep.mode = MODE_PRED; ep.pa = c[2].pa; ep.pb = c[2].pb; ep.pc = c[2].pc;
        ep.out = out->rank2; ep.mean = mean ? mean->rank2 : nullptr;
        const int md = merge_next ? (int)draw_base(pl, step + 1, 0) + 2 : -1;
        if ((st = launch_r2(pl, B, in->rank2, in->adj, flags, 1, ep, na, ps, w, stream, &cf, md))) return st;
    } else if (ew1 && cf.on && rt.ew1_fuse && !na.zr) {
        P0Fuse pf{};
        pf.mode = 4; pf.seed = na.seed; pf.b_off = na.b_off; pf.draw = cf.draw_r; pf.draw_pred = na.draw_r;
        pf.mt = MaskTab{w.mfr, w.mfl, w.Kp, w.Ep}; pf.E = p.E; pf.cf = cf;
        pf.alpha = p.f_alpha; pf.gamma = p.f_gamma; pf.pa = c[2].pa; pf.pb = c[2].pb; pf.pc = c[2].pc;
        pf.out = out->rank2; pf.mean = mean ? mean->rank2 : nullptr;
        pf.f1 = w.net_r;
        if ((st = launch_p(pl, B, in->adj, in->rank2, ps, w, stream, &pf))) return st;
    } else if (ew1) {
        RankEpi ep{};
        ep.mode = MODE_PRED; ep.pa = c[2].pa; ep.pb = c[2].pb; ep.pc = c[2].pc;
        ep.out = out->rank2; ep.mean = mean ? mean->rank2 : nullptr;
        if ((st = launch_ew1(pl, B, in->rank2, ep, na, w, stream, nullptr, &cf, w.net_r))) return st;
        if ((st = launch_p(pl, B, in->adj, cf.on ? (const float*)w.net_r : in->rank2, ps, w, stream))) return st;
    } else if (cf.on && rt.tiled_fuse) {
        P0Fuse pf{};
        pf.mode = 2; pf.net = w.net_r; pf.f1 = w.net_r; pf.seed = na.seed; pf.b_off = na.b_off; pf.draw = cf.draw_r;
        pf.mt = MaskTab{w.mfr, w.mfl, w.Kp, w.Ep}; pf.E = p.E; pf.cf = cf;
        if ((st = launch_p(pl, B, in->adj, in->rank2, ps, w, stream, &pf))) return st;
        r2_in = w.net_r;
    } else if ((st = launch_p(pl, B, in->adj, in->rank2, ps, w, stream))) return st;
    XaArgs xa{};
    xa.xX = xa.xA = in->x; xa.adjX = xa.adjA = in->adj; xa.flags = flags;
    xa.do_x = xa.do_a = 1; xa.mode = MODE_PRED;
    xa.pa_x = c[0].pa; xa.pb_x = c[0].pb; xa.pc_x = c[0].pc;
    xa.pa_a = c[1].pa; xa.pb_a = c[1].pb; xa.pc_a = c[1].pc;
    xa.out_x = out->x; xa.out_a = out->adj;
    xa.mean_x = mean ? mean->x : nullptr; xa.mean_a = mean ? mean->adj : nullptr;
    xa.cf = cf;
    if ((st = launch_xa(pl, B, xa, na, ps, w, stream))) return st;
    if (p.is_cc && !fused && !ew1) {
        if ((st = launch_h(pl, B, r2_in, ps, w, stream))) return st;
        RankEpi ep{};
        ep.mode = MODE_PRED; ep.pa = c[2].pa; ep.pb = c[2].pb; ep.pc = c[2].pc;
        ep.out = out->rank2; ep.mean = mean ? mean->rank2 : nullptr;
        if ((st = launch_hf(pl, B, r2_in, ep, na, w, stream))) return st;
    }
    return CCSD_OK;
}

static int s4_apply(ccsd_plan* pl, int B, int step, const ccsd_state_t* cur, const float* flags, const ccsd_noise_t* n1,
                    const ccsd_noise_t* n2, const ccsd_noise_t* n3, uint64_t seed, int64_t off, const float* sums,
                    ccsd_state_t* out, ccsd_state_t* mean, Workspace& w, void* stream) {
    const PlanD& p = pl->h;
    S4Args q{};
    LangArgs& a = q.a;
    a.x = cur->x; a.adj = cur->adj; a.r = cur->rank2;
    a.nx = w.net_x; a.nadj = w.net_adj; a.nr = w.net_r;
    a.ox = out->x; a.oadj = out->adj; a.orr = out->rank2;
    a.flags = flags; a.sums = sums;
    for (int t = 0; t < 3; ++t) {
        const ccsd_step_coef_t& c = pl->coef[(size_t)step * 3 + t];
        a.ss[t] = c.sscale; a.alpha[t] = c.alpha;
        q.m1[t] = c.m1; q.s1[t] = c.s1; q.d[t] = c.d; q.m2[t] = c.m2; q.s2[t] = c.s2;
    }
    a.snr = p.snr; a.seps = p.seps;
    a.B = B; a.N = p.N; a.F = p.F; a.E = p.E; a.K = p.K; a.is_cc = p.is_cc;
    q.mx = mean ? mean->x : nullptr; q.madj = mean ? mean->adj : nullptr; q.mr = mean ? mean->rank2 : nullptr;
    NoiseArgs na1 = make_noise(n1, seed, off, draw_base(pl, step, 0));
    NoiseArgs na2 = make_noise(n2, seed, off, draw_base(pl, step, 1));
    NoiseArgs na3 = make_noise(n3, seed, off, draw_base(pl, step, 2));
    const long long total = (long long)B * (p.N * p.F + p.N * p.N) + (p.is_cc ? (long long)B * ((p.E + 3) / 4) * p.K : 0);
    prof_mark(pl, KID_S4, stream);
    CCSD_LAUNCH(k_s4_apply, dim3(grid_for(total, 256)), dim3(CCSD_NTHREADS), 0, stream, q, na1, na2, na3,
                (const unsigned long long*)w.offbits, (const unsigned char*)pl->edges, (const unsigned long long*)pl->cells);
    prof_mark(pl, KID_S4, stream);
    LAUNCH_CHECK();
    return CCSD_OK;
}

static int check_step(const ccsd_plan* pl, int step) {
    if (step < 0 || step >= pl->cfg.diff_steps) return set_err(CCSD_ERR_INVALID, "step out of range");
    return CCSD_OK;
}

extern "C" int ccsd_corrector_norms(ccsd_plan_t* pl, int32_t B, int32_t step, int32_t corr_iter, const ccsd_state_t* base,
                                    const ccsd_state_t* cur, const float* flags, const ccsd_noise_t* noise, uint64_t seed,
                                    int64_t sample_offset, float* norm_sums, void* workspace, size_t ws_bytes, void* stream) {
    int st = check_common(pl, B, flags, workspace, ws_bytes);
    if (st || (st = check_step(pl, step)) || (st = check_state(pl, base, "base")) || (st = check_state(pl, cur, "cur"))) return st;
    if (!norm_sums) return set_err(CCSD_ERR_INVALID, "NULL norm_sums");
    Workspace w = carve_ws(pl, B, workspace);
    if ((st = launch_flagbits(pl, B, flags, w, stream))) return st;
    return corrector_norms(pl, B, step, corr_iter, base, cur, flags, noise, seed, sample_offset, norm_sums, w, stream);
}
extern "C" int ccsd_corrector_apply(ccsd_plan_t* pl, int32_t B, int32_t step, int32_t corr_iter, const ccsd_state_t* cur,
                                    const float* flags, const ccsd_noise_t* noise, uint64_t seed, int64_t sample_offset,
                                    const float* norm_sums, ccsd_state_t* out, void* workspace, size_t ws_bytes, void* stream) {
    int st = check_common(pl, B, flags, workspace, ws_bytes);
    if (st || (st = check_step(pl, step)) || (st = check_state(pl, cur, "cur")) || (st = check_state(pl, out, "out"))) return st;
    if (!norm_sums) return set_err(CCSD_ERR_INVALID, "NULL norm_sums");
    Workspace w = carve_ws(pl, B, workspace);
    if ((st = launch_flagbits(pl, B, flags, w, stream))) return st;
    return corrector_apply(pl, B, step, corr_iter, cur, flags, noise, seed, sample_offset, norm_sums, out, w, stream);
}
extern "C" int ccsd_predictor(ccsd_plan_t* pl, int32_t B, int32_t step, const ccsd_state_t* in, const float* flags,
                              const ccsd_noise_t* noise, uint64_t seed, int64_t sample_offset, ccsd_state_t* out,
                              ccsd_state_t* mean, void* workspace, size_t ws_bytes, void* stream) {
    int st = check_common(pl, B, flags, workspace, ws_bytes);
    if (!st && pl->cfg.predictor == CCSD_PRED_S4) return set_err(CCSD_ERR_INVALID, "S4 plans step with ccsd_corrector_norms + ccsd_s4_apply");
    if (st || (st = check_step(pl, step)) || (st = check_state(pl, in, "in")) || (st = check_state(pl, out, "out"))) return st;
    if (mean && (st = check_state(pl, mean, "mean"))) return st;
    if (in->x == out->x || in->adj == out->adj || (pl->h.is_cc && in->rank2 == out->rank2))
        return set_err(CCSD_ERR_INVALID, "predictor cannot run in place");
    Workspace w = carve_ws(pl, B, workspace);
    if ((st = launch_flagbits(pl, B, flags, w, stream))) return st;
    return predictor(pl, B, step, in, flags, noise, seed, sample_offset, out, mean, w, stream);
}

extern "C" int ccsd_s4_apply(ccsd_plan_t* pl, int32_t B, int32_t step, const ccsd_state_t* cur, const float* flags,
                             const ccsd_noise_t* noise1, const ccsd_noise_t* noise2, const ccsd_noise_t* noise3, uint64_t seed,
                             int64_t sample_offset, const float* norm_sums, ccsd_state_t* out, ccsd_state_t* mean,
                             void* workspace, size_t ws_bytes, void* stream) {
    int st = check_common(pl, B, flags, workspace, ws_bytes);
    if (st || (st = check_step(pl, step)) || (st = check_state(pl, cur, "cur")) || (st = check_state(pl, out, "out"))) return st;
    if (mean && (st = check_state(pl, mean, "mean"))) return st;
    if (pl->cfg.predictor != CCSD_PRED_S4) return set_err(CCSD_ERR_INVALID, "ccsd_s4_apply needs a plan created with CCSD_PRED_S4");
    if (!norm_sums) return set_err(CCSD_ERR_INVALID, "NULL norm_sums");
    Workspace w = carve_ws(pl, B, workspace);
    if ((st = launch_flagbits(pl, B, flags, w, stream))) return st;
    return s4_apply(pl, B, step, cur, flags, noise1, noise2, noise3, seed, sample_offset, norm_sums, out, mean, w, stream);
}

extern "C" int ccsd_sampler_run(ccsd_plan_t* pl, int32_t B, const float* flags, uint64_t seed, int64_t sample_offset,
                                int32_t first_step, int32_t last_step, ccsd_state_t* state, ccsd_state_t* scratch,
                                ccsd_state_t* result, float* traj, void* workspace, size_t ws_bytes, void* stream) {
    int st = check_common(pl, B, flags, workspace, ws_bytes);
    if (st || (st = check_state(pl, state, "state")) || (st = check_state(pl, scratch, "scratch")) ||
        (st = check_state(pl, result, "result"))) return st;
    if (first_step < 0 || last_step > pl->cfg.diff_steps || first_step >= last_step) return set_err(CCSD_ERR_INVALID, "bad step range");
    const Route& rt = pl->rt;
    if (rt.loop == LOOP_STEPWISE)
        return set_err(CCSD_ERR_UNSUPPORTED, "ccsd_sampler_run handles n_steps == 1; drive other values step by step");
    const PlanD& p = pl->h;
    Workspace w = carve_ws(pl, B, workspace);
    if ((st = launch_flagbits(pl, B, flags, w, stream))) return st;
    const size_t nx = (size_t)p.N * p.F, na = (size_t)p.N * p.N, nr = p.is_cc ? (size_t)p.E * p.K : 0;
    ccsd_state_t a = *state, b = *scratch;
    for (int step = first_step; step < last_step; ++step) {
        const bool lastone = step == last_step - 1;
        const bool want_mean = pl->cfg.denoise && (lastone || traj);
        if (rt.loop == LOOP_S4) {
            if ((st = corrector_norms(pl, B, step, 0, &a, &a, flags, nullptr, seed, sample_offset, w.sums, w, stream))) return st;
            if ((st = s4_apply(pl, B, step, &a, flags, nullptr, nullptr, nullptr, seed, sample_offset, w.sums, &b,
                               want_mean ? result : nullptr, w, stream))) return st;
            ccsd_state_t t = a; a = b; b = t;
        } else if (rt.loop == LOOP_LANGEVIN_FUSED) {
            const bool r2_done = rt.merged && step > first_step;
            const bool merge_next = rt.merged && !lastone;
            if ((st = corrector_norms(pl, B, step, 0, &a, &a, flags, nullptr, seed, sample_offset, w.sums, w, stream, rt.r2_family == R2_FUSED, r2_done))) return st;
            if (rt.merged && !r2_done && r2_p1_raw(p))
                RT_CHECK(rt_d2d_async(w.U1b, w.U1, (size_t)B * p.h_pw * 4, stream));
            if ((st = predictor(pl, B, step, &a, flags, nullptr, seed, sample_offset, &b, want_mean ? result : nullptr, w, stream, w.sums, merge_next))) return st;
            ccsd_state_t t = a; a = b; b = t;
        } else if (rt.loop == LOOP_LANGEVIN) {
            if ((st = corrector_norms(pl, B, step, 0, &a, &a, flags, nullptr, seed, sample_offset, w.sums, w, stream))) return st;
            if ((st = corrector_apply(pl, B, step, 0, &a, flags, nullptr, seed, sample_offset, w.sums, &b, w, stream))) return st;
            if ((st = predictor(pl, B, step, &b, flags, nullptr, seed, sample_offset, &a, want_mean ? result : nullptr, w, stream))) return st;
        } else {
            if ((st = predictor(pl, B, step, &a, flags, nullptr, seed, sample_offset, &b, want_mean ? result : nullptr, w, stream))) return st;
            ccsd_state_t t = a; a = b; b = t;
        }
        if (traj) {
            const ccsd_state_t* src = pl->cfg.denoise ? result : &a;
            float* slot = traj + (size_t)step * (nx + na + nr);
            RT_CHECK(rt_d2d_async(slot, src->x, nx * 4, stream));
            RT_CHECK(rt_d2d_async(slot + nx, src->adj, na * 4, stream));
            if (nr) RT_CHECK(rt_d2d_async(slot + nx + na, src->rank2, nr * 4, stream));
        }
    }
    if (a.x != state->x) {
        RT_CHECK(rt_d2d_async(state->x, a.x, (size_t)B * nx * 4, stream));
        RT_CHECK(rt_d2d_async(state->adj, a.adj, (size_t)B * na * 4, stream));
        if (nr) RT_CHECK(rt_d2d_async(state->rank2, a.rank2, (size_t)B * nr * 4, stream));
    }
    if (!pl->cfg.denoise) {
        RT_CHECK(rt_d2d_async(result->x, a.x, (size_t)B * nx * 4, stream));
        RT_CHECK(rt_d2d_async(result->adj, a.adj, (size_t)B * na * 4, stream));
        if (nr) RT_CHECK(rt_d2d_async(result->rank2, a.rank2, (size_t)B * nr * 4, stream));
    }
    return CCSD_OK;
}

extern "C" int ccsd_quantize(const float* in, int64_t n, float thr, int64_t* out, void* stream) {
    if (!in || !out || n < 0) return set_err(CCSD_ERR_INVALID, "bad argument");
    if (n == 0) return CCSD_OK;
    CCSD_LAUNCH(k_quantize, dim3(grid_for(n, 256)), dim3(CCSD_NTHREADS), 0, stream, in, (long long)n, thr, (long long*)out);
    LAUNCH_CHECK();
    return CCSD_OK;
}

extern "C" int ccsd_rank2_cells(const float* rank2, int32_t B, int32_t E, int64_t K, float thr, uint64_t* bits, int32_t* counts,
                                void* stream) {
    if (!rank2 || !bits || !counts || B < 1 || E < 1 || K < 1 || K > (1 << 24)) return set_err(CCSD_ERR_INVALID, "bad argument");
    CCSD_LAUNCH(k_rank2_cells, dim3(B), dim3(CCSD_NTHREADS), 0, stream, rank2, (int)E, (int)K, thr, (unsigned long long*)bits, (int*)counts);
    LAUNCH_CHECK();
    return CCSD_OK;
}
```

### ccsd_amd/csrc/ccsd_k_r2.h

```cpp
#pragma once
#include "ccsd_baked_qm9.h"
#include "ccsd_rank2_common.h"

#ifndef CCSD_R2_LB
#define CCSD_R2_LB 4
#endif
struct R2Args {
    const float* rank2; const float* adj; const float* flags;
    const unsigned long long* offbits;
    float* P0; float* P1;
    float* U1;
    int want_p;
    int masked;
    int stagger_mask, stagger_sleep;
    int merge;
    unsigned int draw_r2;
    float* P0b; float* P1b; float* U1b;
    float* net2; float* part2;
    int ldk, ldh;
    long long* dbg;
    const float* wp;
    CorrFuse cf;
};

template <int MT, int RS, bool AFFINE, bool GEN1, int QM9 = 0>
__global__ __launch_bounds__(512, 4) void k_r2(const PlanD* __restrict__ plan, const float* __restrict__ w,
                                            const unsigned char* __restrict__ edges,
                                            const unsigned long long* __restrict__ cells, R2Args ra, RankEpi ep,
                                            NoiseArgs na) {
    CCSD_DYN_SMEM(sm);
    constexpr bool BAKED = QM9 == 2 && CCSD_BAKED_QM9_SIZE == sizeof(PlanD);
    const PlanD& pw = *plan;
    const PlanD& p = BAKED ? *reinterpret_cast<const PlanD*>(CCSD_BAKED_QM9_PLAN) : *plan;
    const int E = QM9 ? 36 : p.E, K = QM9 ? 466 : p.K, N = QM9 ? 9 : p.N, NN = N * N, ldk = QM9 ? 488 : ra.ldk, ldh = QM9 ? 36 : ra.ldh;
    const int b = blockIdx.x, tid = threadIdx.x, nth = blockDim.x;
    const int Kp4 = (K + 31) & ~31, Ep4 = (E + 3) & ~3;
    float* sF = sm;
    float* sH = sF + E * ldk;
    float* sFl = sH + E * ldh;
    float* sRow = sFl + 64;
    float* sAco = sRow + 64;
    float* sAdj = sAco + p.a_cinit * E;
    float* sRed = sAdj + 3 * NN;
    unsigned char* sFrb = reinterpret_cast<unsigned char*>(sRed + 64);
#ifndef CCSD_EMU
    __shared__ int s_hdone;
#endif
    const float* Fg = ra.rank2 + (size_t)b * E * K;
    const FastDiv dK(K);
    constexpr bool ST = AFFINE && !GEN1 && MT == 3 && RS == 1;
    constexpr int MTF = ST ? MT - 1 : MT;
    constexpr int E0 = 16 * MTF;

    stamp(ra.dbg, 0);
#ifndef CCSD_EMU
    if (tid == 0) s_hdone = 0;
#endif
    const unsigned long long off = ra.offbits[b];
    const int hodge2 = (p.h_L > 1) && ra.want_p;
    const bool adjpow = hodge2 && p.hl[0].mval.n > 1;
    auto build_tables = [&](auto&& between) {
        unsigned long long cw[2];
        unsigned int ew = 0;
#pragma unroll
        for (int u = 0; u < 2; ++u) { const int k = tid + u * nth; cw[u] = cells[k < K ? k : K - 1]; }
        if (tid < 64) ew = *reinterpret_cast<const unsigned short*>(edges + 2 * (tid < E ? tid : E - 1));
        between();
#pragma unroll
        for (int u = 0; u < 2; ++u) { const int k = tid + u * nth; if (k < Kp4) sFrb[k] = (k < K && !(cw[u] & off)) ? 1 : 0; }
        for (int k = tid + 2 * nth; k < Kp4; k += nth) sFrb[k] = (k < K && !(cells[k] & off)) ? 1 : 0;
        if (tid < 64) sFl[tid] = (tid < E && !(((off >> (ew & 0xffu)) | (off >> (ew >> 8))) & 1ull)) ? 1.f : 0.f;
        for (int e = tid + nth; e < 64; e += nth) sFl[e] = e < E ? edge_on(off, edges, e) : 0.f;
        for (int t = tid; t < E * (Kp4 - K); t += nth) { const int e = t / (Kp4 - K), k = K + t % (Kp4 - K); sF[e * ldk + k] = 0.f; }
        if (adjpow) {
            float c1a = 0.f, c2a = 0.f;
            if (ra.cf.on) corr_coef(ra.cf, 1, &c1a, &c2a);
            for (int i = tid; i < NN; i += nth) {
                float v = ra.adj[(size_t)b * NN + i];
                if (ra.cf.on) {
                    NoiseArgs nc = na;
                    nc.zadj = nullptr; nc.draw_adj = ra.cf.draw_adj;
                    const int ii = i / N, jj = i % N;
                    const float z = raw_noise_adj(nc, b, ii, jj, N) * ra.flags[(size_t)b * N + ii] * ra.flags[(size_t)b * N + jj];
                    v = fmaf(c2a, z, fmaf(c1a, ra.cf.net_adj[(size_t)b * NN + i], v));
                }
                sAdj[i] = v; sAdj[NN + i] = v;
            }
        }
        __syncthreads();
        stamp(ra.dbg, 8);
    };
    float s_net = 0.f, s_z = 0.f;
    {
        float c1f = 0.f, c2f = 0.f;
        if (ra.cf.on) corr_coef(ra.cf, 2, &c1f, &c2f);
        NoiseArgs nc = na;
        if (ra.cf.on) { nc.zr = nullptr; nc.draw_r = ra.cf.draw_r; }
        const bool znorm = ep.mode == MODE_NORMS && na.flat_r, zuse = znorm || ra.cf.on;
        const float* Ng = ra.cf.on ? ra.cf.net_r + (size_t)b * E * K : Fg;
        const int EK = E * K;
        if ((EK & 3) == 0 && (K & 1) == 0) {
            const float4* F4 = reinterpret_cast<const float4*>(Fg);
            const float4* N4 = reinterpret_cast<const float4*>(Ng);
            const float4* Z4 = reinterpret_cast<const float4*>(nc.zr ? nc.zr + (size_t)b * EK : Fg);
            const int n4 = EK >> 2;
            const FastDiv dK2(K >> 1);
            auto phase0 = [&](auto LB_, auto CF_, auto ZN_) {
                constexpr int LB = decltype(LB_)::value;
                constexpr bool CF = decltype(CF_)::value;
                constexpr bool ZN = decltype(ZN_)::value;
                constexpr int LN = CF ? LB : 1;
                float4 va[LB], vb[LB], qa[LN], qb[LN];
                auto issue = [&](float4* v, float4* q, int base) {
#pragma unroll
                    for (int u = 0; u < LB; ++u) { const int i4 = base + u * nth; v[u] = F4[i4 < n4 ? i4 : n4 - 1]; }
                    if (CF) {
#pragma unroll
                        for (int u = 0; u < LB; ++u) { const int i4 = base + u * nth; q[CF ? u : 0] = N4[i4 < n4 ? i4 : n4 - 1]; }
                    }
                };
                auto consume = [&](const float4* v, const float4* q, int base) {
#pragma unroll
                    for (int u = 0; u < LB; ++u) {
                        const int i4 = base + u * nth;
                        if (i4 < n4) {
                            int e, kp;
                            dK2.divmod(2 * i4, e, kp);
                            const int k = 2 * kp;
                            const bool wrap = k + 2 == K;
                            const int e1 = wrap ? e + 1 : e, k1 = wrap ? 0 : k + 2;
                            float vv[4] = {v[u].x, v[u].y, v[u].z, v[u].w};
                            if (CF || ZN) {
                                float z[4];
                                if (nc.zr) { const float4 z4 = Z4[i4]; z[0] = z4.x; z[1] = z4.y; z[2] = z4.z; z[3] = z4.w; }
                                else philox_normal4(nc.seed, nc.draw_r, nc.b_off + b, (unsigned)i4, z);
                                const unsigned f0 = *reinterpret_cast<const unsigned short*>(sFrb + k), f1 = *reinterpret_cast<const unsigned short*>(sFrb + k1);
                                const float fl0 = sFl[e], fl1 = sFl[e1];
                                const float m[4] = {fl0 * (float)(f0 & 0xffu), fl0 * (float)(f0 >> 8), fl1 * (float)(f1 & 0xffu), fl1 * (float)(f1 >> 8)};
                                const float4 n4v = q[CF ? u : 0];
                                const float nn[4] = {n4v.x, n4v.y, n4v.z, n4v.w};
#pragma unroll
                                for (int j = 0; j < 4; ++j) {
                                    const float zz = z[j] * m[j];
                                    if (ZN && !CF) s_z = fmaf(zz, zz, s_z);
                                    if (CF) vv[j] = fmaf(c2f, zz, fmaf(c1f, nn[j], vv[j]));
                                }
                                if (CF && ZN) {
                                    float z2[4];
                                    philox_normal4(na.seed, ra.draw_r2, na.b_off + b, (unsigned)i4, z2);
#pragma unroll
                                    for (int j = 0; j < 4; ++j) { const float zz = z2[j] * m[j]; s_z = fmaf(zz, zz, s_z); }
                                }
                            }
                            *reinterpret_cast<float2*>(sF + e * ldk + k) = make_float2(vv[0], vv[1]);
                            *reinterpret_cast<float2*>(sF + e1 * ldk + k1) = make_float2(vv[2], vv[3]);
                        }
                    }
                };
                const int step = LB * nth;
                int base = tid;
                build_tables([&]() { issue(va, qa, base); });
                while (true) {
                    const bool more_b = base - tid + step < n4;
                    if (more_b) issue(vb, qb, base + step);
                    consume(va, qa, base);
                    if (!more_b) break;
                    base += step;
                    const bool more_a = base - tid + step < n4;
                    if (more_a) issue(va, qa, base + step);
                    consume(vb, qb, base);
                    if (!more_a) break;
                    base += step;
                }
            };
            typedef std::integral_constant<bool, true> T_;
            typedef std::integral_constant<bool, false> F_;
            if (ra.cf.on && ra.merge) phase0(std::integral_constant<int, 3>{}, T_{}, T_{});
            else if (ra.cf.on) phase0(std::integral_constant<int, 3>{}, T_{}, F_{});
            else if (znorm) phase0(std::integral_constant<int, 3>{}, F_{}, T_{});
            else phase0(std::integral_constant<int, 3>{}, F_{}, F_{});
        } else {
            build_tables([]() {});
            for (int t = tid; t < EK; t += nth) {
                int e, k;
                dK.divmod(t, e, k);
                float v = Fg[t];
                if (zuse) {
                    const float z = nc.zr ? nc.zr[(size_t)b * EK + t] : philox_normal1(nc.seed, nc.draw_r, nc.b_off + b, (unsigned)t);
                    const float zz = z * sFl[e] * (float)sFrb[k];
                    if (znorm) s_z = fmaf(zz, zz, s_z);
                    if (ra.cf.on) v = fmaf(c2f, zz, fmaf(c1f, Ng[t], v));
                }
                sF[e * ldk + k] = v;
            }
        }
    }
    stamp(ra.dbg, 9);
    if (adjpow) {
        float* A = sAdj; float* P0_ = sAdj + NN; float* P1_ = sAdj + 2 * NN;
        for (int c = 0; c < p.a_cinit; ++c) {
            for (int e = tid; e < E; e += nth) sAco[c * E + e] = P0_[edges[2 * e] * N + edges[2 * e + 1]];
            if (c + 1 < p.a_cinit) {
                for (int i = tid; i < NN; i += nth) {
                    const int r = i / N, cc = i % N;
                    float acc = 0.f;
                    for (int kk = 0; kk < N; ++kk) acc = fmaf(P0_[r * N + kk], A[kk * N + cc], acc);
                    P1_[i] = acc;
                }
                __syncthreads();
                float* t2 = P0_; P0_ = P1_; P1_ = t2;
            }
            __syncthreads();
        }
    }
    __syncthreads();
    const int npass = ra.merge ? 2 : 1;
    for (int pass = 0; pass < npass; ++pass) {
    const bool wb = ra.merge && pass == 0;
    if (pass == 1) {
        __syncthreads();
        ep.mode = MODE_NORMS; ep.out = ra.net2; ep.mean = nullptr; ep.part = ra.part2;
        na.zr = nullptr; na.draw_r = ra.draw_r2; na.flat_r = 1;
        ra.P0 = ra.P0b; ra.P1 = ra.P1b; ra.U1 = ra.U1b;
#ifndef CCSD_EMU
        if (tid == 0) s_hdone = 0;
#endif
        __syncthreads();
    }
    stamp(ra.dbg, 1);
#ifdef CCSD_STOP_DIAG
    const int diag = ra.dbg ? (int)ra.dbg[((size_t)gridDim.x + 254) * 64 + 62] : 0;
#else
    constexpr int diag = 0;
#endif
    const HodgeLayerD& h0 = p.hl[0];
    const HodgeLayerD& h1 = p.hl[1];
    const bool doP0 = ra.want_p && p.h_L > 0, doP1 = hodge2;
    const bool lin1 = doP1 && h0.mval.n == 1;
    const bool pm = !GEN1 && lin1 && ra.masked;
    const int wc0 = doP0 ? h0.wc : 0, wc1 = doP1 ? p.h_pw : 0;

    stamp(ra.dbg, 2);
    const int ks = Kp4 >> 2;
    int nHtasks = 0;
    const int nHf = p.f_cnum == 2 ? MTF * (MTF + 1) / 2 : 0, nHs = (ST && p.f_cnum == 2) ? MT : 0;
    const int nH = nHf + nHs;
    const int nt0 = doP0 ? (wc0 + 15) >> 4 : 0, nt1 = doP1 ? (wc1 + 15) >> 4 : 0;
    const int nPf = MTF * (nt0 + nt1);
    const int ntask = nH + nPf + (ST ? nt0 + nt1 : 0);
#ifdef CCSD_EMU
    (void)ks; (void)ntask;
    for (int m = 0; m < E; ++m) {
        for (int n = 0; n < E; ++n) {
            float acc = 0.f;
            if (p.f_cnum == 2) for (int kk = 0; kk < K; ++kk) acc = fmaf(sF[m * ldk + kk], sF[n * ldk + kk], acc);
            sH[m * ldh + n] = (p.f_hmask && m == n) ? 0.f : acc;
        }
        for (int n = 0; n < wc0; ++n) {
            float acc = 0.f;
            for (int kk = 0; kk < K; ++kk) acc = fmaf(sF[m * ldk + kk], w[h0.wcat + (size_t)kk * wc0 + n], acc);
            ra.P0[((size_t)b * E + m) * wc0 + n] = acc;
        }
        for (int n = 0; n < wc1; ++n) {
            float acc = 0.f, un = 0.f;
            int ll = 1;
            while (ll + 1 < p.h_L && n >= p.h_poff[ll + 1]) ++ll;
            const HodgeLayerD& hn = ccsd_hl(p, ll);
            const int nl = n - p.h_poff[ll];
            for (int kk = 0; kk < K; ++kk) {
                const float frk = (float)sFrb[kk], wv = nl < hn.wc ? w[hn.wcat + (size_t)kk * hn.wc + nl] : 0.f;
                float a;
                if (lin1) a = sF[m * ldk + kk] * frk;
                else {
                    float in[CCSD_SMALLW], out[CCSD_SMALLW];
                    for (int c = 0; c < CCSD_SMALLW; ++c) in[c] = c < h0.cin ? sAco[c * E + m] * sF[m * ldk + kk] : 0.f;
                    small_mlp<CCSD_SMALLW>(h0.mval, w, in, out);
                    a = sFl[m] * out[0] * frk;
                }
                acc = fmaf(a, wv, acc);
                un = fmaf(frk, wv, un);
            }
            ra.P1[((size_t)b * E + m) * wc1 + n] = acc;
            if (lin1 && m == 0 && !pm) ra.U1[(size_t)b * wc1 + n] = un;
        }
    }
#endif
#ifndef CCSD_EMU
    typedef float r2_f32x4 __attribute__((ext_vector_type(4)));
    const int nblk = Kp4 >> 4;
    const float* WT0 = ra.wp + h0.wcatT;
    const float* WT1 = ra.wp + h1.wcatT;
    const bool hmask = p.f_hmask != 0;
    auto run_tile = [&](int t) {
        const int lane = tid & 63, l15 = lane & 15, kq = lane >> 4;
        int type, i, c;
        bool strip = false;
        if (t < nHf) {
            type = 0; i = 0;
            int rem = t;
            while (rem >= MTF - i) { rem -= MTF - i; ++i; }
            c = i + rem;
        } else if (t < nH) {
            type = 0; i = MTF; c = t - nHf; strip = true;
        } else if (t < nH + MTF * nt0) {
            type = 1; i = (t - nH) / nt0; c = (t - nH) % nt0;
        } else if (t < nH + nPf) {
            type = 2; i = (t - nH - MTF * nt0) / nt1; c = (t - nH - MTF * nt0) % nt1;
        } else if (t < nH + nPf + nt0) {
            type = 1; i = MTF; c = t - nH - nPf; strip = true;
        } else {
            type = 2; i = MTF; c = t - nH - nPf - nt0; strip = true;
        }
        const int ra_ = strip ? E0 + (l15 & 3) : 16 * i + l15;
        const int arow = ra_ < E ? ra_ : E - 1;
        const float* pa = sF + arow * ldk + 4 * kq;
        int offB = 0;
        const float* wtp = WT0;
        if (type == 0) {
            const int rb_ = 16 * c + l15;
            offB = (rb_ < E ? rb_ : E - 1) * ldk + 4 * kq;
        } else {
            const int wcn = type == 1 ? wc0 : wc1, n = 16 * c + l15;
            wtp = (type == 1 ? WT0 : WT1) + (size_t)(n < wcn ? n : wcn - 1) * Kp4 + 4 * kq;
        }
        r2_f32x4 acc0 = {0.f, 0.f, 0.f, 0.f}, acc1 = {0.f, 0.f, 0.f, 0.f};
        float upart = 0.f;
        auto kloop = [&](auto LB, auto K1, auto SR) {
            constexpr bool lb = decltype(LB)::v, k1 = decltype(K1)::v, sr = decltype(SR)::v;
            auto ldB = [&](int blk) -> float4 {
                if (lb) return *reinterpret_cast<const float4*>(sF + offB + 16 * blk);
                return *reinterpret_cast<const float4*>(wtp + 16 * blk);
            };
            constexpr int D = 4;
            float4 ab[D], bb[D];
            unsigned int fb[D];
#pragma unroll
            for (int u = 0; u < D; ++u) {
                const int bl = u < nblk ? u : nblk - 1;
                ab[u] = *reinterpret_cast<const float4*>(pa + 16 * bl);
                bb[u] = ldB(bl);
                fb[u] = k1 ? *reinterpret_cast<const unsigned int*>(sFrb + 16 * bl + 4 * kq) : 0u;
            }
            auto block = [&](int u, int blk, bool refill) {
                float4 a4 = ab[u];
                const float4 b4 = bb[u];
                if (k1) {
                    const unsigned int f4 = fb[u];
                    const float fr0 = (float)(f4 & 0xffu), fr1 = (float)((f4 >> 8) & 0xffu), fr2 = (float)((f4 >> 16) & 0xffu),
                                fr3 = (float)(f4 >> 24);
                    if (GEN1) {
                        const int e = arow;
                        float fv[4] = {a4.x, a4.y, a4.z, a4.w};
                        const float frv[4] = {fr0, fr1, fr2, fr3};
#pragma unroll
                        for (int j = 0; j < 4; ++j) {
                            float iin[CCSD_SMALLW], out[CCSD_SMALLW];
#pragma unroll
                            for (int cc = 0; cc < CCSD_SMALLW; ++cc) iin[cc] = cc < h0.cin ? sAco[cc * E + e] * fv[j] : 0.f;
                            small_mlp<CCSD_SMALLW>(h0.mval, w, iin, out);
                            fv[j] = sFl[e] * out[0] * frv[j];
                        }
                        a4 = make_float4(fv[0], fv[1], fv[2], fv[3]);
                    } else {
                        a4.x *= fr0; a4.y *= fr1; a4.z *= fr2; a4.w *= fr3;
                        if (!sr) upart = fmaf(fr0, b4.x, fmaf(fr1, b4.y, fmaf(fr2, b4.z, fmaf(fr3, b4.w, upart))));
                    }
                }
                r2_f32x4& acc = (u & 1) ? acc1 : acc0;
                if (sr) {
                    acc = __builtin_amdgcn_mfma_f32_4x4x1f32(a4.x, b4.x, acc, 0, 0, 0);
                    acc = __builtin_amdgcn_mfma_f32_4x4x1f32(a4.y, b4.y, acc, 0, 0, 0);
                    acc = __builtin_amdgcn_mfma_f32_4x4x1f32(a4.z, b4.z, acc, 0, 0, 0);
                    acc = __builtin_amdgcn_mfma_f32_4x4x1f32(a4.w, b4.w, acc, 0, 0, 0);
                } else {
                    acc = __builtin_amdgcn_mfma_f32_16x16x4f32(a4.x, b4.x, acc, 0, 0, 0);
                    acc = __builtin_amdgcn_mfma_f32_16x16x4f32(a4.y, b4.y, acc, 0, 0, 0);
                    acc = __builtin_amdgcn_mfma_f32_16x16x4f32(a4.z, b4.z, acc, 0, 0, 0);
                    acc = __builtin_amdgcn_mfma_f32_16x16x4f32(a4.w, b4.w, acc, 0, 0, 0);
                }
                if (refill) {
                    __builtin_amdgcn_sched_barrier(0);
                    const int bl = blk + D < nblk ? blk + D : nblk - 1;
                    ab[u] = *reinterpret_cast<const float4*>(pa + 16 * bl);
                    bb[u] = ldB(bl);
                    if (k1) fb[u] = *reinterpret_cast<const unsigned int*>(sFrb + 16 * bl + 4 * kq);
                    __builtin_amdgcn_sched_barrier(0);
                }
            };
            int blk0 = 0;
            for (; blk0 + D <= nblk; blk0 += D) {
#pragma unroll
                for (int u = 0; u < D; ++u) block(u, blk0 + u, true);
            }
#pragma unroll
            for (int u = 0; u < D - 1; ++u)
                if (blk0 + u < nblk) block(u, blk0 + u, false);
        };
        if ((diag & 1) && type != 0) { (void)0; }
        else if ((diag & 2) && type == 0) { (void)0; }
        else
        if (ST && strip) {
            if (type == 2 && !pm) kloop(BoolTag<false>{}, BoolTag<true>{}, BoolTag<true>{});
            else if (type == 0) kloop(BoolTag<true>{}, BoolTag<false>{}, BoolTag<true>{});
            else kloop(BoolTag<false>{}, BoolTag<false>{}, BoolTag<true>{});
        } else {
            if (type == 2 && !pm) kloop(BoolTag<false>{}, BoolTag<true>{}, BoolTag<false>{});
            else if (type == 0) kloop(BoolTag<true>{}, BoolTag<false>{}, BoolTag<false>{});
            else kloop(BoolTag<false>{}, BoolTag<false>{}, BoolTag<false>{});
        }
        r2_f32x4 acc = acc0 + acc1;
        const int n = 16 * c + l15;
        if (ST && strip) {
            float v = 0.f;
#pragma unroll
            for (int r = 0; r < 4; ++r) {
                const float tot = rows_allsum(acc[r]);
                v = kq == r ? tot : v;
            }
            const int m = E0 + kq;
            if (type == 0) {
                if (n < E && m < E) {
                    const float hv = (hmask && m == n) ? 0.f : v;
                    sH[m * ldh + n] = hv;
                    sH[n * ldh + m] = hv;
                }
                __builtin_amdgcn_fence(__ATOMIC_RELEASE, "workgroup");
                if (lane == 0) atomicAdd(&s_hdone, 1);
            } else {
                const int wcn = type == 1 ? wc0 : wc1;
                float* const dstp = type == 1 ? ra.P0 : ra.P1;
                if (n < wcn && m < E) dstp[((size_t)b * E + m) * wcn + n] = v;
            }
            return;
        }
        const int mb = 16 * i + 4 * kq;
        if (type == 0) {
            if (n < E) {
#pragma unroll
                for (int r = 0; r < 4; ++r) {
                    const int m = mb + r;
                    if (m < E) {
                        const float hv = (hmask && m == n) ? 0.f : acc[r];
                        sH[m * ldh + n] = hv;
                        sH[n * ldh + m] = hv;
                    }
                }
            }
            __builtin_amdgcn_fence(__ATOMIC_RELEASE, "workgroup");
            if (lane == 0) atomicAdd(&s_hdone, 1);
        } else if (type == 1) {
            if (n < wc0) {
                float* dst = ra.P0 + ((size_t)b * E + mb) * wc0 + n;
#pragma unroll
                for (int r = 0; r < 4; ++r)
                    if (mb + r < E) dst[(size_t)r * wc0] = acc[r];
            }
        } else {
            float un = upart;
            un += __shfl_xor(un, 16, 64);
            un += __shfl_xor(un, 32, 64);
            if (n < wc1) {
                float* dst = ra.P1 + ((size_t)b * E + mb) * wc1 + n;
#pragma unroll
                for (int r = 0; r < 4; ++r)
                    if (mb + r < E) dst[(size_t)r * wc1] = acc[r];
                if (!GEN1 && i == 0 && kq == 0 && !pm) ra.U1[(size_t)b * wc1 + n] = un;
            }
        }
    };
    nHtasks = nH;
    const int nw1 = nth >> 6, wave1 = wave_index();
    int n1 = ntask;
    if (AFFINE && !wb) {
        n1 = ((nH + nw1 - 1) / nw1) * nw1;
        if (n1 > ntask) n1 = ntask;
    }
    for (int t = wave1; t < n1; t += nw1) {
        run_tile(t);
        if (t == 0) stamp(ra.dbg, 6);
    }

    stamp(ra.dbg, 7);
    if (wb) __syncthreads();
    else if (nHtasks > 0) {
        unsigned spins = 0;
        while (__hip_atomic_load(&s_hdone, __ATOMIC_ACQUIRE, __HIP_MEMORY_SCOPE_WORKGROUP) < nHtasks) {
            __builtin_amdgcn_s_sleep(8);
            if (++spins == (1u << 27)) __builtin_trap();
        }
    }
#endif

    stamp(ra.dbg, 3);
    const bool eznorm = !na.flat_r;
    const int ntn = (K + 15) >> 4, ksE = Ep4 >> 2;
    auto epi4 = [&](int e0, int k, const float* hf) {
        if (e0 >= E || k >= K) return;
        float z[4] = {0.f, 0.f, 0.f, 0.f};
        if (ep.mode == MODE_PRED || (ep.mode == MODE_NORMS && eznorm)) raw_noise_r4(na, b, e0 >> 2, k, E, K, z);
        const float fr = (float)sFrb[k];
#pragma unroll
        for (int r = 0; r < 4; ++r) {
            const int e = e0 + r;
            if (e >= E) continue;
            const float f = sF[e * ldk + k];
            const float m = sFl[e] * fr;
            const float hf1[CCSD_MAXCN - 1] = {hf[r], 0.f, 0.f};
            const float net = fnet_element<AFFINE>(pw, w, f, hf1, m);
            const size_t gi = ((size_t)b * E + e) * K + k;
            if (ep.mode == MODE_SCORE) {
                ep.out[gi] = ep.sscale * net;
            } else {
                const float zz = z[r] * m;
                if (ep.mode == MODE_NORMS) {
                    ep.out[gi] = net;
                    s_net = fmaf(net, net, s_net);
                    if (eznorm) s_z = fmaf(zz, zz, s_z);
                } else {
                    const float mean = fmaf(ep.pa, f, ep.pb * net);
                    if (ep.mean) ep.mean[gi] = mean;
                    const float nv = fmaf(ep.pc, zz, mean);
                    ep.out[gi] = nv;
                    if (wb) sF[e * ldk + k] = nv;
                }
            }
        }
    };
#ifdef CCSD_EMU
    for (int tn = 0; tn < ntn; ++tn) {
        float hfv[64][16];
        for (int e = 0; e < E; ++e)
            for (int j = 0; j < 16; ++j) {
                const int k = 16 * tn + j;
                float acc = 0.f;
                if (p.f_cnum == 2 && k < K)
                    for (int e2 = 0; e2 < E; ++e2) acc = fmaf(sH[e * ldh + e2], sF[e2 * ldk + k], acc);
                hfv[e][j] = acc;
            }
        for (int e0 = 0; e0 < E; e0 += 4)
            for (int j = 0; j < 16; ++j) {
                const float v[4] = {hfv[e0][j], e0 + 1 < E ? hfv[e0 + 1][j] : 0.f, e0 + 2 < E ? hfv[e0 + 2][j] : 0.f, e0 + 3 < E ? hfv[e0 + 3][j] : 0.f};
                epi4(e0, 16 * tn + j, v);
            }
    }
#else
    if constexpr (AFFINE && ST) {
        typedef float f32x4 __attribute__((ext_vector_type(4)));
        const int wave = wave_index(), nw = nth >> 6, lane = tid & 63, l15 = lane & 15, kq = lane >> 4;
        constexpr int TF = MT - 1;
        const int ar0 = l15 * ldh + 4 * kq;
        const int srow = E0 + (l15 & 3) < E ? E0 + (l15 & 3) : E - 1;
        const int as0 = srow * ldh + 4 * kq;
        const int brow = 4 * kq * ldk;
        const unsigned vo = (unsigned)(4 * kq * K + l15);
        const bool cn2 = p.f_cnum == 2;
        float* const outp = ep.out + (size_t)b * E * K;
        auto coltile = [&](auto MODE_, auto INJ_, int tn) -> f32x4 {
            constexpr int MODE = decltype(MODE_)::value;
            constexpr bool INJ = decltype(INJ_)::value;
            const float s_ = MODE == 0 ? ep.sscale : MODE == 1 ? 1.f : ep.pb;
            const float sa = s_ * pw.f_alpha, sb = s_ * pw.f_beta, sg = s_ * pw.f_gamma;
            const float pa = ep.pa, pc = ep.pc;
            float* const meanp = MODE == 3 ? ep.mean + (size_t)b * E * K : nullptr;
            const float* const zrp = INJ ? na.zr + (size_t)b * E * K : nullptr;
            const int n = 16 * tn + l15;
            const bool nin = n < K;
            const int nc = nin ? n : K - 1;
            float bv[4 * TF], bvr[RS];
            const float* fb = sF + brow + nc;
#pragma unroll
            for (int t = 0; t < TF; ++t)
#pragma unroll
                for (int j = 0; j < 4; ++j) bv[4 * t + j] = fb[(16 * t + j) * ldk];
#pragma unroll
            for (int s0 = 0; s0 < RS; ++s0) {
                const int c = E0 + 4 * s0 + kq;
                bvr[s0] = sF[(c < E ? c : E - 1) * ldk + nc];
            }
            f32x4 acc[TF], sacc = {0.f, 0.f, 0.f, 0.f};
#pragma unroll
            for (int i = 0; i < TF; ++i) acc[i] = (f32x4){0.f, 0.f, 0.f, 0.f};
            if (cn2) {
                int ao = ar0, so = as0;
                asm volatile("" : "+v"(ao), "+v"(so));
#pragma unroll
                for (int t = 0; t < TF; ++t) {
                    float4 a4[TF];
#pragma unroll
                    for (int i = 0; i < TF; ++i) a4[i] = *reinterpret_cast<const float4*>(sH + ao + 16 * i * ldh + 16 * t);
                    const float4 h4 = *reinterpret_cast<const float4*>(sH + so + 16 * t);
#pragma unroll
                    for (int i = 0; i < TF; ++i) acc[i] = __builtin_amdgcn_mfma_f32_16x16x4f32(a4[i].x, bv[4 * t + 0], acc[i], 0, 0, 0);
                    sacc = __builtin_amdgcn_mfma_f32_4x4x1f32(h4.x, bv[4 * t + 0], sacc, 0, 0, 0);
#pragma unroll
                    for (int i = 0; i < TF; ++i) acc[i] = __builtin_amdgcn_mfma_f32_16x16x4f32(a4[i].y, bv[4 * t + 1], acc[i], 0, 0, 0);
                    sacc = __builtin_amdgcn_mfma_f32_4x4x1f32(h4.y, bv[4 * t + 1], sacc, 0, 0, 0);
#pragma unroll
                    for (int i = 0; i < TF; ++i) acc[i] = __builtin_amdgcn_mfma_f32_16x16x4f32(a4[i].z, bv[4 * t + 2], acc[i], 0, 0, 0);
                    sacc = __builtin_amdgcn_mfma_f32_4x4x1f32(h4.z, bv[4 * t + 2], sacc, 0, 0, 0);
#pragma unroll
                    for (int i = 0; i < TF; ++i) acc[i] = __builtin_amdgcn_mfma_f32_16x16x4f32(a4[i].w, bv[4 * t + 3], acc[i], 0, 0, 0);
                    sacc = __builtin_amdgcn_mfma_f32_4x4x1f32(h4.w, bv[4 * t + 3], sacc, 0, 0, 0);
                }
#pragma unroll
                for (int s0 = 0; s0 < RS; ++s0) {
                    const int c = E0 + 4 * s0 + kq;
                    const int cc = (c < E ? c : E - 1) - 4 * kq;
#pragma unroll
                    for (int i = 0; i < TF; ++i) {
                        const float av = sH[ao + 16 * i * ldh + cc];
                        acc[i] = __builtin_amdgcn_mfma_f32_16x16x4f32(c < E ? av : 0.f, bvr[s0], acc[i], 0, 0, 0);
                    }
                    const float hv = sH[so + cc];
                    sacc = __builtin_amdgcn_mfma_f32_4x4x1f32(c < E ? hv : 0.f, bvr[s0], sacc, 0, 0, 0);
                }
            }
            if (nin && !(diag & 4)) {
                const float fr = (float)sFrb[n];
                unsigned gi = vo + 16u * (unsigned)tn;
#pragma unroll
                for (int i = 0; i < TF; ++i) {
                    const int e0 = 16 * i + 4 * kq;
                    float z[4] = {0.f, 0.f, 0.f, 0.f};
                    if ((MODE >= 2 || (MODE == 1 && eznorm)) && !(diag & 8)) {
                        if (INJ) {
#pragma unroll
                            for (int r = 0; r < 4; ++r) z[r] = zrp[gi + (unsigned)(r * K)];
                        } else {
                            philox_normal4(na.seed, na.draw_r, na.b_off + b, (unsigned)((4 * i + kq) * K + n), z);
                        }
                    }
                    const float4 fl4 = *reinterpret_cast<const float4*>(sFl + e0);
                    const float flv[4] = {fl4.x, fl4.y, fl4.z, fl4.w};
#pragma unroll
                    for (int r = 0; r < 4; ++r) {
                        const float f = bv[4 * i + r];
                        const float m = flv[r] * fr;
                        const float net = m * fmaf(sb, acc[i][r], fmaf(sa, f, sg));
                        const unsigned g = gi + (unsigned)(r * K);
                        if (MODE == 0) {
                            outp[g] = net;
                        } else {
                            const float zz = z[r] * m;
                            if (MODE == 1) {
                                outp[g] = net;
                                s_net = fmaf(net, net, s_net);
                                if (eznorm) s_z = fmaf(zz, zz, s_z);
                            } else {
                                const float mean = fmaf(pa, f, net);
                                if (MODE == 3) meanp[g] = mean;
                                const float nv = fmaf(pc, zz, mean);
                                outp[g] = nv;
                                if (wb) sF[(e0 + r) * ldk + n] = nv;
                            }
                        }
                    }
                    gi += 16u * (unsigned)K;
                }
            }
            return sacc;
        };
        auto strip_finish = [&](auto MODE_, auto INJ_, const f32x4& p0, const f32x4& p1, const f32x4& p2, const f32x4& p3, int tn0) {
            constexpr int MODE = decltype(MODE_)::value;
            constexpr bool INJ = decltype(INJ_)::value;
            float hf[4];
#pragma unroll
            for (int r = 0; r < 4; ++r) {
                float a = p0[r], c = p1[r], d = p2[r], e = p3[r];
                lane_swap16(a, c);
                const float a01 = a + c;
                lane_swap16(d, e);
                const float a23 = d + e;
                float u = a01, v = a23;
                lane_swap32(u, v);
                hf[r] = u + v;
            }
            const int tn = tn0 + kq * nw;
            const int n = 16 * tn + l15;
            if (tn < ntn && n < K && !(diag & 4)) {
                const float s_ = MODE == 0 ? ep.sscale : MODE == 1 ? 1.f : ep.pb;
                const float sa = s_ * pw.f_alpha, sb = s_ * pw.f_beta, sg = s_ * pw.f_gamma;
                const float pa = ep.pa, pc = ep.pc;
                float* const meanp = MODE == 3 ? ep.mean + (size_t)b * E * K : nullptr;
                const float fr = (float)sFrb[n];
                const unsigned gi = (unsigned)(E0 * K + n);
                float z[4] = {0.f, 0.f, 0.f, 0.f};
                if ((MODE >= 2 || (MODE == 1 && eznorm)) && !(diag & 8)) {
                    if (INJ) {
                        const float* const zrp = na.zr + (size_t)b * E * K;
#pragma unroll
                        for (int r = 0; r < 4; ++r) z[r] = E0 + r < E ? zrp[gi + (unsigned)(r * K)] : 0.f;
                    } else {
                        philox_normal4(na.seed, na.draw_r, na.b_off + b, (unsigned)((E0 >> 2) * K + n), z);
                    }
                }
                const float4 fl4 = *reinterpret_cast<const float4*>(sFl + E0);
                const float flv[4] = {fl4.x, fl4.y, fl4.z, fl4.w};
#pragma unroll
                for (int r = 0; r < 4; ++r) {
                    const int e = E0 + r;
                    if (e < E) {
                        const float f = sF[e * ldk + n];
                        const float m = flv[r] * fr;
                        const float net = m * fmaf(sb, hf[r], fmaf(sa, f, sg));
                        const unsigned g = gi + (unsigned)(r * K);
                        if (MODE == 0) {
                            outp[g] = net;
                        } else {
                            const float zz = z[r] * m;
                            if (MODE == 1) {
                                outp[g] = net;
                                s_net = fmaf(net, net, s_net);
                                if (eznorm) s_z = fmaf(zz, zz, s_z);
                            } else {
                                const float mean = fmaf(pa, f, net);
                                if (MODE == 3) meanp[g] = mean;
                                const float nv = fmaf(pc, zz, mean);
                                outp[g] = nv;
                                if (wb) sF[e * ldk + n] = nv;
                            }
                        }
                    }
                }
            }
        };
        typedef std::integral_constant<bool, false> NoInj;
        typedef std::integral_constant<bool, true> Inj;
        const bool inj = na.zr != nullptr && ep.mode != MODE_SCORE;
        const int cmode = ep.mode == MODE_SCORE ? 0 : ep.mode == MODE_NORMS ? 1 : ep.mean == nullptr ? 2 : 3;
        const int sel = cmode * 2 + (inj ? 1 : 0);
        int pt = n1 + (wave + nw - (nHf % nw)) % nw;
        const int pslot = wave < (nw >> 1) ? 0 : 2;
        int cnt = 0;
        const f32x4 zero4 = {0.f, 0.f, 0.f, 0.f};
        f32x4 sp0 = zero4, sp1 = zero4, sp2 = zero4, sp3 = zero4;
        for (int tn = wave; tn < ntn; tn += nw, ++cnt) {
            if (cnt == pslot && pt < ntask) { run_tile(pt); pt += nw; }
            if (diag & 16) continue;
            f32x4 sacc;
            switch (sel) {
                case 0: case 1: sacc = coltile(std::integral_constant<int, 0>{}, NoInj{}, tn); break;
                case 2: sacc = coltile(std::integral_constant<int, 1>{}, NoInj{}, tn); break;
                case 3: sacc = coltile(std::integral_constant<int, 1>{}, Inj{}, tn); break;
                case 4: sacc = coltile(std::integral_constant<int, 2>{}, NoInj{}, tn); break;
                case 5: sacc = coltile(std::integral_constant<int, 2>{}, Inj{}, tn); break;
                case 6: sacc = coltile(std::integral_constant<int, 3>{}, NoInj{}, tn); break;
                default: sacc = coltile(std::integral_constant<int, 3>{}, Inj{}, tn); break;
            }
            const int c4 = cnt & 3;
            if (c4 == 0) sp0 = sacc; else if (c4 == 1) sp1 = sacc; else if (c4 == 2) sp2 = sacc; else sp3 = sacc;
            if (c4 == 3 || tn + nw >= ntn) {
                const int tn0 = tn - c4 * nw;
                switch (sel) {
                    case 0: case 1: strip_finish(std::integral_constant<int, 0>{}, NoInj{}, sp0, sp1, sp2, sp3, tn0); break;
                    case 2: strip_finish(std::integral_constant<int, 1>{}, NoInj{}, sp0, sp1, sp2, sp3, tn0); break;
                    case 3: strip_finish(std::integral_constant<int, 1>{}, Inj{}, sp0, sp1, sp2, sp3, tn0); break;
                    case 4: strip_finish(std::integral_constant<int, 2>{}, NoInj{}, sp0, sp1, sp2, sp3, tn0); break;
                    case 5: strip_finish(std::integral_constant<int, 2>{}, Inj{}, sp0, sp1, sp2, sp3, tn0); break;
                    case 6: strip_finish(std::integral_constant<int, 3>{}, NoInj{}, sp0, sp1, sp2, sp3, tn0); break;
                    default: strip_finish(std::integral_constant<int, 3>{}, Inj{}, sp0, sp1, sp2, sp3, tn0); break;
                }
                sp0 = sp1 = sp2 = sp3 = zero4;
            }
        }
        for (; pt < ntask; pt += nw) run_tile(pt);
    } else if constexpr (AFFINE) {
        typedef float f32x4 __attribute__((ext_vector_type(4)));
        const int wave = wave_index(), nw = nth >> 6, lane = tid & 63, l15 = lane & 15, kq = lane >> 4;
        constexpr int TF = RS ? MT - 1 : MT;
        const bool padblk = RS == 0 && (E & 15) != 0;
        const int ar0 = (l15 < E ? l15 : E - 1) * ldh + 4 * kq;
        const int arL = ((16 * (MT - 1) + l15 < E) ? 16 * (MT - 1) + l15 : E - 1) * ldh + 4 * kq;
        const int brow = 4 * kq * ldk;
        const unsigned vo = (unsigned)(4 * kq * K + l15);
        const bool cn2 = p.f_cnum == 2;
        auto coltile = [&](auto MODE_, auto INJ_, int tn) {
            constexpr int MODE = decltype(MODE_)::value;
            constexpr bool INJ = decltype(INJ_)::value;
            const float s_ = MODE == 0 ? ep.sscale : MODE == 1 ? 1.f : ep.pb;
            const float sa = s_ * pw.f_alpha, sb = s_ * pw.f_beta, sg = s_ * pw.f_gamma;
            const float pa = ep.pa, pc = ep.pc;
            float* const outp = ep.out + (size_t)b * E * K;
            float* const meanp = MODE == 3 ? ep.mean + (size_t)b * E * K : nullptr;
            const float* const zrp = INJ ? na.zr + (size_t)b * E * K : nullptr;
            {
                const int n = 16 * tn + l15;
                const bool nin = n < K;
                const int nc = nin ? n : K - 1;
                float bv[TF ? 4 * TF : 1], bvr[RS ? RS : 1];
                const float* fb = sF + brow + nc;
#pragma unroll
                for (int t = 0; t < TF; ++t)
#pragma unroll
                    for (int j = 0; j < 4; ++j) {
                        const int c = 16 * t + 4 * kq + j;
                        bv[4 * t + j] = (t < MT - 1 || !padblk) ? fb[(16 * t + j) * ldk] : sF[(c < E ? c : E - 1) * ldk + nc];
                    }
#pragma unroll
                for (int s0 = 0; s0 < RS; ++s0) {
                    const int c = 16 * TF + 4 * s0 + kq;
                    bvr[s0] = sF[(c < E ? c : E - 1) * ldk + nc];
                }
                f32x4 acc[MT];
#pragma unroll
                for (int i = 0; i < MT; ++i) acc[i] = (f32x4){0.f, 0.f, 0.f, 0.f};
                if (cn2) {
                    int ao = ar0, aL = arL;
                    asm volatile("" : "+v"(ao), "+v"(aL));
#pragma unroll
                    for (int t = 0; t < TF; ++t) {
                        float4 a4[MT];
#pragma unroll
                        for (int i = 0; i < MT; ++i)
                            a4[i] = *reinterpret_cast<const float4*>(sH + (i < MT - 1 ? ao + 16 * i * ldh : aL) + 16 * t);
                        if (t == MT - 1 && padblk) {
                            const int c0 = 16 * t + 4 * kq;
#pragma unroll
                            for (int i = 0; i < MT; ++i) {
                                a4[i].x = c0 < E ? a4[i].x : 0.f; a4[i].y = c0 + 1 < E ? a4[i].y : 0.f;
                                a4[i].z = c0 + 2 < E ? a4[i].z : 0.f; a4[i].w = c0 + 3 < E ? a4[i].w : 0.f;
                            }
                        }
#pragma unroll
                        for (int i = 0; i < MT; ++i) {
                            acc[i] = __builtin_amdgcn_mfma_f32_16x16x4f32(a4[i].x, bv[4 * t + 0], acc[i], 0, 0, 0);
                            acc[i] = __builtin_amdgcn_mfma_f32_16x16x4f32(a4[i].y, bv[4 * t + 1], acc[i], 0, 0, 0);
                            acc[i] = __builtin_amdgcn_mfma_f32_16x16x4f32(a4[i].z, bv[4 * t + 2], acc[i], 0, 0, 0);
                            acc[i] = __builtin_amdgcn_mfma_f32_16x16x4f32(a4[i].w, bv[4 * t + 3], acc[i], 0, 0, 0);
                        }
                    }
#pragma unroll
                    for (int s0 = 0; s0 < RS; ++s0) {
                        const int c = 16 * TF + 4 * s0 + kq;
                        const int cc = (c < E ? c : E - 1) - 4 * kq;
#pragma unroll
                        for (int i = 0; i < MT; ++i) {
                            const float av = sH[(i < MT - 1 ? ao + 16 * i * ldh : aL) + cc];
                            acc[i] = __builtin_amdgcn_mfma_f32_16x16x4f32(c < E ? av : 0.f, bvr[s0], acc[i], 0, 0, 0);
                        }
                    }
                }
                if (nin) {
                    const float fr = (float)sFrb[n];
                    unsigned gi = vo + 16u * (unsigned)tn;
#pragma unroll
                    for (int i = 0; i < MT; ++i) {
                        const bool last = i == MT - 1;
                        const int e0 = 16 * i + 4 * kq;
                        if (!last || e0 < E) {
                            float z[4] = {0.f, 0.f, 0.f, 0.f};
                            if (MODE >= 2 || (MODE == 1 && eznorm)) {
                                if (INJ) {
#pragma unroll
                                    for (int r = 0; r < 4; ++r) z[r] = (!last || e0 + r < E) ? zrp[gi + (unsigned)(r * K)] : 0.f;
                                } else {
                                    philox_normal4(na.seed, na.draw_r, na.b_off + b, (unsigned)((4 * i + kq) * K + n), z);
                                }
                            }
                            const float4 fl4 = *reinterpret_cast<const float4*>(sFl + e0);
                            const float flv[4] = {fl4.x, fl4.y, fl4.z, fl4.w};
#pragma unroll
                            for (int r = 0; r < 4; ++r) {
                                const int e = e0 + r;
                                const float f = i < TF ? bv[4 * (i < TF ? i : 0) + r] : sF[(e < E ? e : E - 1) * ldk + n];
                                const float m = flv[r] * fr;
                                const float net = m * fmaf(sb, acc[i][r], fmaf(sa, f, sg));
                                const unsigned g = gi + (unsigned)(r * K);
                                if (!last || e < E) {
                                    if (MODE == 0) {
                                        outp[g] = net;
                                    } else {
                                        const float zz = z[r] * m;
                                        if (MODE == 1) {
                                            outp[g] = net;
                                            s_net = fmaf(net, net, s_net);
                                            if (eznorm) s_z = fmaf(zz, zz, s_z);
                                        } else {
                                            const float mean = fmaf(pa, f, net);
                                            if (MODE == 3) meanp[g] = mean;
                                            outp[g] = fmaf(pc, zz, mean);
                                        }
                                    }
                                }
                            }
                        }
                        gi += 16u * (unsigned)K;
                    }
                }
            }
        };
        typedef std::integral_constant<bool, false> NoInj;
        typedef std::integral_constant<bool, true> Inj;
        const bool inj = na.zr != nullptr && ep.mode != MODE_SCORE;
        const int cmode = ep.mode == MODE_SCORE ? 0 : ep.mode == MODE_NORMS ? 1 : ep.mean == nullptr ? 2 : 3;
        int pt = n1 + wave;
        const int pslot = wave < (nw >> 1) ? 0 : 2;
        int cnt = 0;
        for (int tn = wave; tn < ntn; tn += nw, ++cnt) {
            if (cnt == pslot && pt < ntask) { run_tile(pt); pt += nw; }
            switch (cmode * 2 + (inj ? 1 : 0)) {
                case 0: case 1: coltile(std::integral_constant<int, 0>{}, NoInj{}, tn); break;
                case 2: coltile(std::integral_constant<int, 1>{}, NoInj{}, tn); break;
                case 3: coltile(std::integral_constant<int, 1>{}, Inj{}, tn); break;
                case 4: coltile(std::integral_constant<int, 2>{}, NoInj{}, tn); break;
                case 5: coltile(std::integral_constant<int, 2>{}, Inj{}, tn); break;
                case 6: coltile(std::integral_constant<int, 3>{}, NoInj{}, tn); break;
                default: coltile(std::integral_constant<int, 3>{}, Inj{}, tn); break;
            }
        }
        for (; pt < ntask; pt += nw) run_tile(pt);
    } else {
        typedef float f32x4 __attribute__((ext_vector_type(4)));
        const int wave = wave_index(), nw = nth >> 6, lane = tid & 63, l15 = lane & 15, kq = lane >> 4;
        constexpr int KSE = 4 * MT;
        float hA[MT][KSE];
#pragma unroll
        for (int i = 0; i < MT; ++i)
#pragma unroll
            for (int s0 = 0; s0 < KSE; ++s0) {
                const int r = 16 * i + l15, c = 4 * s0 + kq;
                const float v = sH[(r < E ? r : E - 1) * ldh + (c < E ? c : E - 1)];
                hA[i][s0] = (r < E && c < E) ? v : 0.f;
            }
        for (int tn = wave; tn < ntn; tn += nw) {
            const int n = 16 * tn + l15;
            const bool nin = n < K;
            f32x4 acc[MT];
#pragma unroll
            for (int i = 0; i < MT; ++i) acc[i] = (f32x4){0.f, 0.f, 0.f, 0.f};
            if (p.f_cnum == 2) {
                float bv[KSE];
#pragma unroll
                for (int s0 = 0; s0 < KSE; ++s0) {
                    const int kk = 4 * s0 + kq;
                    const float v = sF[(kk < E ? kk : E - 1) * ldk + (nin ? n : K - 1)];
                    bv[s0] = (kk < E && nin) ? v : 0.f;
                }
#pragma unroll
                for (int s0 = 0; s0 < KSE; ++s0)
                    if (s0 < ksE) {
#pragma unroll
                        for (int i = 0; i < MT; ++i) acc[i] = __builtin_amdgcn_mfma_f32_16x16x4f32(hA[i][s0], bv[s0], acc[i], 0, 0, 0);
                    }
            }
#pragma unroll
            for (int i = 0; i < MT; ++i) {
                const float v[4] = {acc[i][0], acc[i][1], acc[i][2], acc[i][3]};
                epi4(16 * i + 4 * kq, n, v);
            }
        }
    }
#endif
    }
    stamp(ra.dbg, 4);
    if (ep.mode == MODE_NORMS) {
        float t2_[2] = {s_net, s_z};
        block_sums<2>(t2_, sRed);
        const float tn_ = t2_[0], tz_ = t2_[1];
        if (tid == 0) { ep.part[(size_t)b * 2 + 0] = tn_; ep.part[(size_t)b * 2 + 1] = tz_; }
    }
    stamp(ra.dbg, 5);
}
```

### ccsd_amd/csrc/ccsd_rank2_common.h

```cpp
#pragma once
#include "ccsd_dev.h"

CCSD_DEV float edge_on(unsigned long long off, const unsigned char* __restrict__ edges, int e) {
    return ((off >> edges[2 * e]) | (off >> edges[2 * e + 1])) & 1ull ? 0.f : 1.f;
}
CCSD_DEV float cell_on(unsigned long long off, const unsigned long long* __restrict__ cells, int k) {
    return (cells[k] & off) ? 0.f : 1.f;
}

static inline __host__ __device__ int h_ld(int E) { return (E + 3) & ~3; }
struct MaskTab { const unsigned char* mfr; const unsigned char* mfl; int Kp, Ep; };
CCSD_DEV void group_masks(const MaskTab& mt, int b, int E, int K, int e, int k, float* m) {
    const unsigned char* fr = mt.mfr + (size_t)b * mt.Kp;
    const unsigned char* fl = mt.mfl + (size_t)b * mt.Ep;
    if ((K & 3) == 0) {
        const unsigned f4 = *reinterpret_cast<const unsigned*>(fr + k);
        const float l = (float)fl[e < E ? e : E - 1];
        m[0] = l * (float)(f4 & 0xffu); m[1] = l * (float)((f4 >> 8) & 0xffu); m[2] = l * (float)((f4 >> 16) & 0xffu); m[3] = l * (float)(f4 >> 24);
    } else {
#pragma unroll
        for (int s = 0; s < 4; ++s) {
            m[s] = (float)fl[e < E ? e : E - 1] * (float)fr[k];
            if (++k == K) { k = 0; ++e; }
        }
    }
}

enum { MODE_SCORE = 0, MODE_NORMS = 1, MODE_PRED = 2 };

struct RankEpi {
    int mode;
    float sscale;
    float pa, pb, pc;
    float* out;
    float* mean;
    float* part;
};

template <bool AFFINE, int FW = CCSD_FW>
CCSD_DEV float fnet_element(const PlanD& p, const float* __restrict__ w, float f, const float* hf, float m) {
    if (AFFINE) {
        float t = fmaf(p.f_alpha, f, p.f_gamma);
#pragma unroll
        for (int j = 1; j < CCSD_MAXCN; ++j)
            if (j < p.f_cnum) t = fmaf(p.f_betas[j], hf[j - 1], t);
        return m * t;
    }
    if (p.f_blk >= 0) {
        const float* fb = w + p.f_blk;
        const float* hd = fb + CCSD_FBLK_HEAD;
        float prev[8] = {f, p.f_cnum > 1 ? hf[0] : 0.f, p.f_cnum > 2 ? hf[1] : 0.f, p.f_cnum > 3 ? hf[2] : 0.f, 0.f, 0.f, 0.f, 0.f};
        float acc = 0.f;
#pragma unroll
        for (int i = 0; i < 8; ++i) acc = fmaf(prev[i], hd[i], acc);
#pragma unroll
        for (int l = 0; l < CCSD_MAXFL; ++l)
            if (l < p.f_L) {
                float o8[8];
                small_mlp_lds<8>(fb + l * CCSD_MAXLIN * CCSD_HWBLK, p.fl[l].n, prev, o8);
#pragma unroll
                for (int i = 0; i < 8; ++i) {
                    prev[i] = m * o8[i];
                    acc = fmaf(prev[i], hd[(l + 1) * 8 + i], acc);
                }
            }
        return m * (acc + hd[(CCSD_MAXFL + 1) * 8]);
    }
    float ch[FW];
#pragma unroll
    for (int i = 0; i < FW; ++i) ch[i] = 0.f;
    ch[0] = f;
#pragma unroll
    for (int j = 1; j < CCSD_MAXCN; ++j)
        if (j < p.f_cnum) ch[j] = hf[j - 1];
    int ci0 = 0, co0 = p.f_cnum;
    for (int l = 0; l < p.f_L; ++l) {
        float in[FW], out[FW];
#pragma unroll
        for (int i = 0; i < FW; ++i) {
            float v = 0.f;
#pragma unroll
            for (int j = 0; j < FW; ++j)
                if (j == ci0 + i) v = ch[j];
            in[i] = v;
        }
        small_mlp<FW>(p.fl[l], w, in, out);
        const int no = p.fl[l].out;
#pragma unroll
        for (int j = 0; j < FW; ++j)
#pragma unroll
            for (int i = 0; i < FW; ++i)
                if (i < no && j == co0 + i) ch[j] = m * out[i];
        ci0 = co0; co0 += no;
    }
    float out[FW];
    small_mlp<FW>(p.f_fin, w, ch, out);
    return m * out[0];
}

template <int D = 4, class LA, class LB, class EP>
CCSD_DEV void wave_tile(int m0, int n0, int ks, LA la, LB lb, EP ep) {
#ifdef CCSD_EMU
    for (int i = 0; i < 16; ++i)
        for (int j = 0; j < 16; ++j) {
            float acc = 0.f;
            for (int k = 0; k < 4 * ks; ++k) acc = fmaf(la(m0 + i, k), lb(k, n0 + j), acc);
            ep(m0 + i, n0 + j, acc);
        }
#else
    typedef float f32x4 __attribute__((ext_vector_type(4)));
    const int lane = threadIdx.x & 63, l15 = lane & 15, kq = lane >> 4;
    f32x4 acc = {0.f, 0.f, 0.f, 0.f};
    for (int s = 0; s < ks; s += D) {
        float a[D], bv[D];
#pragma unroll
        for (int u = 0; u < D; ++u) {
            const int sc = s + u < ks ? s + u : ks - 1;
            a[u] = la(m0 + l15, 4 * sc + kq);
            bv[u] = lb(4 * sc + kq, n0 + l15);
        }
#pragma unroll
        for (int u = 0; u < D; ++u)
            if (s + u < ks) acc = __builtin_amdgcn_mfma_f32_16x16x4f32(a[u], bv[u], acc, 0, 0, 0);
    }
#pragma unroll
    for (int r = 0; r < 4; ++r) ep(m0 + 4 * kq + r, n0 + l15, acc[r]);
#endif
}

template <class LA, class LB, class EP>
CCSD_DEV void wave_coltile(int n0, int mt, int ks, LA la, LB lb, EP ep4) {
#ifdef CCSD_EMU
    float acc[64][16];
    for (int i = 0; i < 16 * mt; ++i)
        for (int j = 0; j < 16; ++j) {
            float a = 0.f;
            for (int k = 0; k < 4 * ks; ++k) a = fmaf(la(i, k), lb(k, n0 + j), a);
            acc[i][j] = a;
        }
    for (int i = 0; i < 16 * mt; i += 4)
        for (int j = 0; j < 16; ++j) {
            const float v[4] = {acc[i][j], acc[i + 1][j], acc[i + 2][j], acc[i + 3][j]};
            ep4(i, n0 + j, v);
        }
#else
    typedef float f32x4 __attribute__((ext_vector_type(4)));
    const int lane = threadIdx.x & 63, l15 = lane & 15, kq = lane >> 4;
    f32x4 acc[4];
#pragma unroll
    for (int t = 0; t < 4; ++t) acc[t] = (f32x4){0.f, 0.f, 0.f, 0.f};
    int s = 0;
    for (; s + 4 <= ks; s += 4) {
        float bv[4], a[4][4];
#pragma unroll
        for (int u = 0; u < 4; ++u) bv[u] = lb(4 * (s + u) + kq, n0 + l15);
#pragma unroll
        for (int u = 0; u < 4; ++u)
#pragma unroll
            for (int t = 0; t < 4; ++t) a[u][t] = t < mt ? la(16 * t + l15, 4 * (s + u) + kq) : 0.f;
#pragma unroll
        for (int u = 0; u < 4; ++u)
#pragma unroll
            for (int t = 0; t < 4; ++t)
                if (t < mt) acc[t] = __builtin_amdgcn_mfma_f32_16x16x4f32(a[u][t], bv[u], acc[t], 0, 0, 0);
    }
    for (; s < ks; ++s) {
        const float bv = lb(4 * s + kq, n0 + l15);
#pragma unroll
        for (int t = 0; t < 4; ++t)
            if (t < mt) acc[t] = __builtin_amdgcn_mfma_f32_16x16x4f32(la(16 * t + l15, 4 * s + kq), bv, acc[t], 0, 0, 0);
    }
#pragma unroll
    for (int t = 0; t < 4; ++t)
        if (t < mt) {
            const float v[4] = {acc[t][0], acc[t][1], acc[t][2], acc[t][3]};
            ep4(16 * t + 4 * kq, n0 + l15, v);
        }
#endif
}

CCSD_DEV float raw_noise_r1(const NoiseArgs& na, int b, int e, int k, int E, int K) {
    if (na.zr) return na.zr[((size_t)b * E + e) * K + k];
    float n[4];
    philox_normal4(na.seed, na.draw_r, na.b_off + b, (unsigned)((e >> 2) * K + k), n);
    const int s = e & 3;
    return s == 0 ? n[0] : s == 1 ? n[1] : s == 2 ? n[2] : n[3];
}

struct CorrFuse {
    int on;
    const float* net_x; const float* net_adj; const float* net_r;
    const float* sums;
    float ss[3], alpha[3];
    float snr, seps;
    unsigned int draw_x, draw_adj, draw_r;
};
CCSD_DEV void corr_coef(const CorrFuse& cf, int t, float* c1, float* c2) {
    const float gn = fabsf(cf.ss[t]) * cf.sums[t], zn = cf.sums[3 + t];
    const float q = cf.snr * zn / gn;
    const float step = q * q * 2.f * cf.alpha[t];
    *c1 = step * cf.ss[t];
    *c2 = sqrtf(step * 2.f) * cf.seps;
}
```

### include/ccsd_hip.h

```cpp
#ifndef CCSD_HIP_H
#define CCSD_HIP_H

#include <stddef.h>
#include <stdint.h>

#ifdef __cplusplus
extern "C" {
#endif

#define CCSD_ABI_VERSION 5

enum {
    CCSD_OK = 0,
    CCSD_ERR_INVALID = 1,
    CCSD_ERR_UNSUPPORTED = 2,
    CCSD_ERR_WEIGHTS = 3,
    CCSD_ERR_RUNTIME = 4,
    CCSD_ERR_WORKSPACE = 5
};

enum { CCSD_SDE_VP = 0, CCSD_SDE_VE = 1, CCSD_SDE_SUBVP = 2 };
enum { CCSD_PRED_EULER = 0, CCSD_PRED_REVERSE = 1, CCSD_PRED_S4 = 2 };
enum { CCSD_CORR_NONE = 0, CCSD_CORR_LANGEVIN = 1 };
enum { CCSD_TARGET_X = 0, CCSD_TARGET_ADJ = 1, CCSD_TARGET_RANK2 = 2 };

typedef struct {
    float sscale, alpha, pa, pb, pc;
    float m1, s1, d, m2, s2;
} ccsd_step_coef_t;

typedef struct {
    int32_t abi_version;
    int32_t N, F, is_cc, d_min, d_max;
    int32_t x_depth, x_nhid;
    int32_t a_num_layers, a_num_linears, a_c_init, a_c_hid, a_c_final, a_nhid, a_adim, a_num_heads;
    int32_t a_is_cc_net, h_num_layers, h_num_linears, h_nhid, h_adim, h_c_hid, h_c_final, h_num_heads;
    int32_t f_num_layers, f_num_linears, f_nhid, f_c_hid, f_c_final, f_cnum, f_num_layers_mlp, f_use_hodge_mask;
    int32_t predictor, corrector, n_corr_steps, probability_flow, denoise;
    float snr, scale_eps;
    int32_t diff_steps;
    int32_t batch_hint;
    int32_t x_gmh, x_num_linears, x_c_init, x_c_hid, x_c_final, x_adim, x_num_heads;
    int32_t a_conv_mlp, x_conv_mlp;
} ccsd_config_t;

typedef struct ccsd_plan ccsd_plan_t;

int ccsd_plan_create(const ccsd_config_t* cfg, const float* weights, size_t n_weights,
                     const ccsd_step_coef_t* step_coef, ccsd_plan_t** out);
void ccsd_plan_destroy(ccsd_plan_t* plan);

size_t ccsd_weight_count(const ccsd_config_t* cfg);
void ccsd_rank2_dims(const ccsd_config_t* cfg, int32_t* E, int64_t* K);
size_t ccsd_workspace_bytes(const ccsd_plan_t* plan, int32_t B);

const char* ccsd_last_error(void);

typedef struct {
    float* x;
    float* adj;
    float* rank2;
} ccsd_state_t;

typedef struct {
    const float* zx;
    const float* zadj;
    const float* zrank2;
} ccsd_noise_t;

int ccsd_score(ccsd_plan_t* plan, int32_t target, int32_t B, const ccsd_state_t* in, const float* flags_dev,
               float sscale, float* out_dev, void* workspace, size_t workspace_bytes, void* stream);

int ccsd_init_state(ccsd_plan_t* plan, int32_t B, const float* flags_dev, const ccsd_noise_t* prior,
                    uint64_t seed, int64_t sample_offset, ccsd_state_t* state, void* stream);

int ccsd_noise_draws(ccsd_plan_t* plan, int32_t B, const float* flags_dev, uint64_t seed, int64_t sample_offset,
                     int32_t step, int32_t phase, ccsd_state_t* out, void* stream);

enum {
    CCSD_QUERY_FUSED_R2 = 0,
    CCSD_QUERY_XA_VARIANT = 1,
    CCSD_QUERY_R2_LDS_BYTES = 2,
    CCSD_QUERY_XA_LDS_BYTES = 3,
    CCSD_QUERY_FUSED_LOOP = 4,
    CCSD_QUERY_MERGED_R2 = 5,
    CCSD_QUERY_EW1 = 6,
    CCSD_QUERY_LARGE_GRAPH = 7,
    CCSD_QUERY_R2_FAMILY = 8,
    CCSD_QUERY_R2_INSTANCE = 9,
    CCSD_QUERY_LOOP_FORM = 10,
    CCSD_QUERY_H_FULL = 11,
    CCSD_QUERY_HP_FULL = 12,
    CCSD_QUERY_P0_NARROW = 13,
    CCSD_QUERY_TILED_FUSE = 14,
    CCSD_QUERY_EW1_FUSE = 15,
    CCSD_QUERY_H_GENERAL = 16,
    CCSD_QUERY_GEO_EK = 17
};
int ccsd_plan_query(const ccsd_plan_t* plan, int32_t what, int64_t* value);

int ccsd_corrector_norms(ccsd_plan_t* plan, int32_t B, int32_t step, int32_t corr_iter,
                         const ccsd_state_t* base, const ccsd_state_t* cur, const float* flags_dev, const ccsd_noise_t* noise,
                         uint64_t seed, int64_t sample_offset, float* norm_sums_dev,
                         void* workspace, size_t workspace_bytes, void* stream);
int ccsd_corrector_apply(ccsd_plan_t* plan, int32_t B, int32_t step, int32_t corr_iter,
                         const ccsd_state_t* cur, const float* flags_dev, const ccsd_noise_t* noise,
                         uint64_t seed, int64_t sample_offset, const float* norm_sums_dev,
                         ccsd_state_t* out, void* workspace, size_t workspace_bytes, void* stream);

int ccsd_predictor(ccsd_plan_t* plan, int32_t B, int32_t step, const ccsd_state_t* in, const float* flags_dev,
                   const ccsd_noise_t* noise, uint64_t seed, int64_t sample_offset,
                   ccsd_state_t* out, ccsd_state_t* mean, void* workspace, size_t workspace_bytes, void* stream);

int ccsd_s4_apply(ccsd_plan_t* plan, int32_t B, int32_t step, const ccsd_state_t* cur, const float* flags_dev,
                  const ccsd_noise_t* noise1, const ccsd_noise_t* noise2, const ccsd_noise_t* noise3, uint64_t seed,
                  int64_t sample_offset, const float* norm_sums_dev, ccsd_state_t* out, ccsd_state_t* mean,
                  void* workspace, size_t workspace_bytes, void* stream);

int ccsd_sampler_run(ccsd_plan_t* plan, int32_t B, const float* flags_dev, uint64_t seed, int64_t sample_offset,
                     int32_t first_step, int32_t last_step, ccsd_state_t* state, ccsd_state_t* scratch,
                     ccsd_state_t* result, float* traj_dev, void* workspace, size_t workspace_bytes, void* stream);

int ccsd_quantize(const float* in_dev, int64_t n, float thr, int64_t* out_dev, void* stream);

int ccsd_rank2_cells(const float* rank2_dev, int32_t B, int32_t E, int64_t K, float thr, uint64_t* bits_dev,
                     int32_t* counts_dev, void* stream);

int ccsd_profile_kernel(ccsd_plan_t* plan, int32_t kernel_id);
int ccsd_profile_stride(ccsd_plan_t* plan, int32_t stride);
int ccsd_profile_read(ccsd_plan_t* plan, int32_t kernel_id, int64_t* launches, double* total_ms);
int ccsd_profile_launches(ccsd_plan_t* plan, int32_t kernel_id, int64_t* launches);
int ccsd_debug_stamps(ccsd_plan_t* plan, void* dev_buffer);

#ifdef __cplusplus
}
#endif
#endif
```

Baseline: 4286 complexes/s.

## Fold Langevin norm-sum reduction into rank-2 predictor kernel and add all-on mask fast path

Removes the separate single-block k_normsum launch in the fused Langevin loop. Each block of the rank-2 predictor kernel now re-reduces the batch norm partials itself while building its tables, then derives the corrector coefficients in-kernel. Partial buffers are double-buffered by step parity so the next step's merged norms do not overwrite the current ones. It also adds an 'all-on' specialization that skips the per-cell mask multiply when a sample has no off bits. The cost is redundant B-wide reduction work in every block and added template variants and register pressure.

Result: faster. 4344 complexes/s, median of 6 (+1.3%).

```diff
diff --git a/ccsd_amd/_lib.py b/ccsd_amd/_lib.py
--- a/ccsd_amd/_lib.py
+++ b/ccsd_amd/_lib.py
@@ -22,7 +22,7 @@
 ]
 QUERIES = {"fused_r2": 0, "xa_variant": 1, "r2_lds_bytes": 2, "xa_lds_bytes": 3, "fused_loop": 4, "merged_r2": 5, "ew1": 6, "large_graph": 7,
            "r2_family": 8, "r2_instance": 9, "loop_form": 10, "h_full": 11, "hp_full": 12, "p0_narrow": 13, "tiled_fuse": 14, "ew1_fuse": 15,
-           "h_general": 16, "geo_ek": 17}
+           "h_general": 16, "geo_ek": 17, "r2_sums": 18}
 KERNEL_IDS = {"k_xa": 0, "k_gemm_p": 1, "k_hf_score": 2, "k_gemm_h": 3, "k_langevin_apply": 4, "k_r2": 5, "k_s4_apply": 6, "k_ew1": 7}
 
 
diff --git a/ccsd_amd/csrc/ccsd_api.h b/ccsd_amd/csrc/ccsd_api.h
--- a/ccsd_amd/csrc/ccsd_api.h
+++ b/ccsd_amd/csrc/ccsd_api.h
@@ -25,6 +25,7 @@
     int no_fused_r2 = 0, hodge_general = 0, geo_off = 0, no_fused_apply = 0, no_h_full = 0, no_hp_full = 0, hp_full_norms = 0, split_bf16 = 0;
     int xa_threads = 0, xa_prio = 0, xa_stagger_mask = 0, xa_stagger_sleep = 0, r2_stagger_mask = 0, r2_stagger_sleep = 0;
     int lg_force = 0, xa_pass = -1, xa_gch = 0, no_mlp_wt = 0, verbose = 0;
+    int normsum_kernel = 0, no_allon = 0;
     const char *dump_plan = nullptr, *dump_plan_name = nullptr;
 };
 static Knobs read_knobs() {
@@ -34,6 +35,7 @@
     k.geo_off = on("CCSD_NO_GEO") ? 1 : on("CCSD_NO_BAKE") ? 2 : 0;
     k.no_fused_apply = on("CCSD_NO_FUSED_APPLY"); k.no_h_full = on("CCSD_NO_H_FULL"); k.no_hp_full = on("CCSD_NO_HP_FULL");
     k.hp_full_norms = on("CCSD_HP_FULL_NORMS");
+    k.normsum_kernel = on("CCSD_NORMSUM_KERNEL"); k.no_allon = on("CCSD_NO_ALLON");
     if (const char* v = getenv("CCSD_SPLIT_BF16")) k.split_bf16 = atoi(v) == 3 ? 3 : 0;
     if (const char* v = getenv("CCSD_XA_THREADS")) { const int t = atoi(v); if (t >= 64 && t <= 1024 && t % 64 == 0) k.xa_threads = t; }
     if (const char* v = getenv("CCSD_XA_PRIO")) k.xa_prio = atoi(v);
@@ -65,6 +67,7 @@
     unsigned hp_full_modes = 0;
     int loop = LOOP_PRED_ONLY;
     int merged = 0;
+    int r2_sums = 0;
     int tiled_fuse = 0;
     int ew1_fuse = 0;
     int corrector_flat = 0, predictor_flat = 0;
@@ -205,6 +208,7 @@
     if (full_geo && r.tiled_fuse && p.hl[0].wc <= 16 && p.f_cnum == 2 && !k.no_hp_full)
         r.hp_full_modes = (r.loop == LOOP_LANGEVIN_FUSED ? 1u << 2 : 0u) | (k.hp_full_norms ? 1u << 1 : 0u);
     r.merged = r.loop == LOOP_LANGEVIN_FUSED && fused && mt == 3 && rs == 1 && aff && !gen1 && (K & 1) == 0 && ((E * K) & 3) == 0;
+    r.r2_sums = r.merged && !k.normsum_kernel;
     r.corrector_flat = !s4;
     r.predictor_flat = ew1;
     return CCSD_OK;
@@ -220,7 +224,9 @@
     *threads = t > e->max_threads ? e->max_threads : t;
     return e;
 }
-static inline int normsum_threads(int B) { return B > 512 ? 1024 : B > 256 ? 512 : 256; }
+static inline int normsum_threads(int B) { return ccsd_normsum_threads(B); }
+#define CCSD_R2_SUMS_MAXB 1024
+static inline bool use_r2_sums(const Route& r, int B) { return r.r2_sums && B <= CCSD_R2_SUMS_MAXB; }
 
 extern "C" const char* ccsd_last_error(void) { return g_last_error.c_str(); }
 
@@ -595,7 +601,8 @@
 }
 struct RankEpi;
 static int launch_r2(const ccsd_plan* pl, int B, const float* rank2, const float* adj, const float* flags, int want_p,
-                     RankEpi& ep, NoiseArgs& na, Pass& ps, Workspace& w, void* stream, const CorrFuse* cf, int merge_draw);
+                     RankEpi& ep, NoiseArgs& na, Pass& ps, Workspace& w, void* stream, const CorrFuse* cf, int merge_draw,
+                     const float* ns_part = nullptr, float* part_next = nullptr);
 static int launch_p(const ccsd_plan* pl, int B, const float* adj, const float* rank2, Pass& ps, Workspace& w, void* stream, const P0Fuse* fuse = nullptr) {
     const PlanD& p = pl->h;
     const Route& rt = pl->rt;
@@ -833,15 +840,18 @@
 }
 
 static int launch_r2(const ccsd_plan* pl, int B, const float* rank2, const float* adj, const float* flags, int want_p,
-                     RankEpi& ep, NoiseArgs& na, Pass& ps, Workspace& w, void* stream, const CorrFuse* cf = nullptr, int merge_draw = -1) {
+                     RankEpi& ep, NoiseArgs& na, Pass& ps, Workspace& w, void* stream, const CorrFuse* cf = nullptr, int merge_draw = -1,
+                     const float* ns_part, float* part_next) {
     const Route& rt = pl->rt;
     R2Args ra{};
     if (cf) ra.cf = *cf;
     ra.masked = (cf && cf->on) ? 1 : 0;
+    ra.allon = ra.masked && !pl->knobs.no_allon;
     if (merge_draw >= 0) {
         ra.merge = 1; ra.draw_r2 = (unsigned)merge_draw;
-        ra.P0b = w.P0b; ra.P1b = w.P1b; ra.U1b = w.U1b; ra.net2 = w.net_r; ra.part2 = w.part;
-    }
+        ra.P0b = w.P0b; ra.P1b = w.P1b; ra.U1b = w.U1b; ra.net2 = w.net_r; ra.part2 = part_next ? part_next : w.part;
+    }
+    if (ns_part && cf && cf->on) { ra.ns_norm2 = w.norm2; ra.ns_part = ns_part; ra.ns_out = const_cast<float*>(cf->sums); ra.ns_B = B; }
     ra.rank2 = rank2; ra.adj = adj; ra.flags = flags; ra.offbits = w.offbits; ra.P0 = w.P0; ra.P1 = w.P1; ra.U1 = w.U1; ra.want_p = want_p;
     ra.ldk = rt.r2_ldk; ra.ldh = rt.r2_ldh; ra.dbg = pl->dbg; ra.wp = pl->wp;
     ra.stagger_mask = pl->knobs.r2_stagger_mask; ra.stagger_sleep = pl->knobs.r2_stagger_sleep;
@@ -964,6 +974,7 @@
         case CCSD_QUERY_EW1_FUSE: *value = r.ew1_fuse; break;
         case CCSD_QUERY_H_GENERAL: *value = r.h_general; break;
         case CCSD_QUERY_GEO_EK: *value = r.geo; break;
+        case CCSD_QUERY_R2_SUMS: *value = r.r2_sums; break;
         default: return set_err(CCSD_ERR_INVALID, "unknown query");
     }
     return CCSD_OK;
@@ -971,7 +982,7 @@
 
 static int corrector_norms(ccsd_plan* pl, int B, int step, int it, const ccsd_state_t* base, const ccsd_state_t* cur,
                            const float* flags, const ccsd_noise_t* noise, uint64_t seed, int64_t off, float* sums,
-                           Workspace& w, void* stream, bool keep_net = true, bool r2_done = false) {
+                           Workspace& w, void* stream, bool keep_net = true, bool r2_done = false, float* r2_part = nullptr) {
     const PlanD& p = pl->h;
     int st;
     NoiseArgs na = make_noise(noise, seed, off, draw_base(pl, step, it), pl->rt.corrector_flat);
@@ -983,7 +994,7 @@
     int ntiles = w.ntiles;
     if (fused) {
         RankEpi ep{};
-        ep.mode = MODE_NORMS; ep.out = w.net_r; ep.part = w.part;
+        ep.mode = MODE_NORMS; ep.out = w.net_r; ep.part = r2_part ? r2_part : w.part;
         if (r2_done) ps.p1_raw = r2_p1_raw(p);
         else if ((st = launch_r2(pl, B, cur->rank2, cur->adj, flags, 1, ep, na, ps, w, stream))) return st;
         ntiles = 1;
@@ -1036,6 +1047,7 @@
             part = w.part2; ntiles = 1;
         }
     }
+    if (r2_part) return CCSD_OK;
     CCSD_LAUNCH(k_normsum, dim3(1), dim3(CCSD_NTHREADS == 1 ? 1 : normsum_threads(B)), 0, stream, (const float*)w.norm2, part, B, ntiles,
                 p.is_cc, sums);
     LAUNCH_CHECK();
@@ -1068,7 +1080,7 @@
 }
 static int predictor(ccsd_plan* pl, int B, int step, const ccsd_state_t* in, const float* flags, const ccsd_noise_t* noise,
                      uint64_t seed, int64_t off, ccsd_state_t* out, ccsd_state_t* mean, Workspace& w, void* stream,
-                     const float* fuse_sums = nullptr, bool merge_next = false) {
+                     const float* fuse_sums = nullptr, bool merge_next = false, const float* ns_part = nullptr, float* part_next = nullptr) {
     const PlanD& p = pl->h;
     int st;
     NoiseArgs na = make_noise(noise, seed, off, draw_base(pl, step, pl->cfg.n_corr_steps), pl->rt.predictor_flat);
@@ -1090,7 +1102,7 @@
         ep.mode = MODE_PRED; ep.pa = c[2].pa; ep.pb = c[2].pb; ep.pc = c[2].pc;
         ep.out = out->rank2; ep.mean = mean ? mean->rank2 : nullptr;
         const int md = merge_next ? (int)draw_base(pl, step + 1, 0) + 2 : -1;
-        if ((st = launch_r2(pl, B, in->rank2, in->adj, flags, 1, ep, na, ps, w, stream, &cf, md))) return st;
+        if ((st = launch_r2(pl, B, in->rank2, in->adj, flags, 1, ep, na, ps, w, stream, &cf, md, ns_part, part_next))) return st;
     } else if (ew1 && cf.on && rt.ew1_fuse && !na.zr) {
         P0Fuse pf{};
         pf.mode = 4; pf.seed = na.seed; pf.b_off = na.b_off; pf.draw = cf.draw_r; pf.draw_pred = na.draw_r;
@@ -1161,6 +1173,8 @@
     return CCSD_OK;
 }
 
+static inline float* r2_step_part(const Workspace& w, int step) { return (step & 1) ? w.part2 : w.part; }
+
 static int check_step(const ccsd_plan* pl, int step) {
     if (step < 0 || step >= pl->cfg.diff_steps) return set_err(CCSD_ERR_INVALID, "step out of range");
     return CCSD_OK;
@@ -1229,6 +1243,7 @@
     if ((st = launch_flagbits(pl, B, flags, w, stream))) return st;
     const size_t nx = (size_t)p.N * p.F, na = (size_t)p.N * p.N, nr = p.is_cc ? (size_t)p.E * p.K : 0;
     ccsd_state_t a = *state, b = *scratch;
+    const bool insum = use_r2_sums(rt, B);
     for (int step = first_step; step < last_step; ++step) {
         const bool lastone = step == last_step - 1;
         const bool want_mean = pl->cfg.denoise && (lastone || traj);
@@ -1240,10 +1255,12 @@
         } else if (rt.loop == LOOP_LANGEVIN_FUSED) {
             const bool r2_done = rt.merged && step > first_step;
             const bool merge_next = rt.merged && !lastone;
-            if ((st = corrector_norms(pl, B, step, 0, &a, &a, flags, nullptr, seed, sample_offset, w.sums, w, stream, rt.r2_family == R2_FUSED, r2_done))) return st;
+            float* const pcur = insum ? r2_step_part(w, step) : nullptr;
+            float* const pnext = insum ? r2_step_part(w, step + 1) : nullptr;
+            if ((st = corrector_norms(pl, B, step, 0, &a, &a, flags, nullptr, seed, sample_offset, w.sums, w, stream, rt.r2_family == R2_FUSED, r2_done, pcur))) return st;
             if (rt.merged && !r2_done && r2_p1_raw(p))
                 RT_CHECK(rt_d2d_async(w.U1b, w.U1, (size_t)B * p.h_pw * 4, stream));
-            if ((st = predictor(pl, B, step, &a, flags, nullptr, seed, sample_offset, &b, want_mean ? result : nullptr, w, stream, w.sums, merge_next))) return st;
+            if ((st = predictor(pl, B, step, &a, flags, nullptr, seed, sample_offset, &b, want_mean ? result : nullptr, w, stream, w.sums, merge_next, pcur, pnext))) return st;
             ccsd_state_t t = a; a = b; b = t;
         } else if (rt.loop == LOOP_LANGEVIN) {
             if ((st = corrector_norms(pl, B, step, 0, &a, &a, flags, nullptr, seed, sample_offset, w.sums, w, stream))) return st;
diff --git a/ccsd_amd/csrc/ccsd_k_r2.h b/ccsd_amd/csrc/ccsd_k_r2.h
--- a/ccsd_amd/csrc/ccsd_k_r2.h
+++ b/ccsd_amd/csrc/ccsd_k_r2.h
@@ -21,6 +21,8 @@
     long long* dbg;
     const float* wp;
     CorrFuse cf;
+    const float* ns_norm2; const float* ns_part; float* ns_out; int ns_B;
+    int allon;
 };
 
 template <int MT, int RS, bool AFFINE, bool GEN1, int QM9 = 0>
@@ -51,12 +53,44 @@
     constexpr bool ST = AFFINE && !GEN1 && MT == 3 && RS == 1;
     constexpr int MTF = ST ? MT - 1 : MT;
     constexpr int E0 = 16 * MTF;
+    typedef std::integral_constant<bool, true> T_;
+    typedef std::integral_constant<bool, false> F_;
 
     stamp(ra.dbg, 0);
 #ifndef CCSD_EMU
     if (tid == 0) s_hdone = 0;
 #endif
     const unsigned long long off = ra.offbits[b];
+    const bool allon = ST && ra.allon && off == 0ull;
+    const bool nsum = ST && ra.ns_B > 0;
+    float* const sNs = sH;
+    NormSumRegs<6> ns6; NormSumRegs<2> ns2;
+    auto nsum_load = [&]() {
+        if (!nsum) return;
+        if (b == 0) normsums_load<6>(ra.ns_norm2, ra.ns_part, ra.ns_B, ns6);
+        else normsums_load<2>(ra.ns_norm2, ra.ns_part, ra.ns_B, ns2);
+    };
+    auto nsum_reduce = [&]() {
+        if (!nsum) return;
+        if (b == 0) normsums_reduce<6>(ns6, ra.ns_B, sNs);
+        else normsums_reduce<2>(ns2, ra.ns_B, sNs);
+    };
+    auto nsum_coef = [&](float* c1, float* c2) {
+        float gs, zs;
+        if (b == 0) {
+            const float t = normsums_finish<6>(sNs, ra.ns_B);
+#ifdef CCSD_EMU
+            for (int i = 0; i < 6; ++i) ra.ns_out[i] = sNs[i * 16];
+#else
+            if (tid < 6) ra.ns_out[tid] = t;
+#endif
+            gs = normsums_value(t, sNs, 2); zs = normsums_value(t, sNs, 5);
+        } else {
+            const float t = normsums_finish<2>(sNs, ra.ns_B);
+            gs = normsums_value(t, sNs, 0); zs = normsums_value(t, sNs, 1);
+        }
+        corr_coef_sums(ra.cf, 2, gs, zs, c1, c2);
+    };
     const int hodge2 = (p.h_L > 1) && ra.want_p;
     const bool adjpow = hodge2 && p.hl[0].mval.n > 1;
     auto build_tables = [&](auto&& between) {
@@ -93,7 +127,7 @@
     float s_net = 0.f, s_z = 0.f;
     {
         float c1f = 0.f, c2f = 0.f;
-        if (ra.cf.on) corr_coef(ra.cf, 2, &c1f, &c2f);
+        if (ra.cf.on && !nsum) corr_coef(ra.cf, 2, &c1f, &c2f);
         NoiseArgs nc = na;
         if (ra.cf.on) { nc.zr = nullptr; nc.draw_r = ra.cf.draw_r; }
         const bool znorm = ep.mode == MODE_NORMS && na.flat_r, zuse = znorm || ra.cf.on;
@@ -105,10 +139,11 @@
             const float4* Z4 = reinterpret_cast<const float4*>(nc.zr ? nc.zr + (size_t)b * EK : Fg);
             const int n4 = EK >> 2;
             const FastDiv dK2(K >> 1);
-            auto phase0 = [&](auto LB_, auto CF_, auto ZN_) {
+            auto phase0 = [&](auto LB_, auto CF_, auto ZN_, auto AO_) {
                 constexpr int LB = decltype(LB_)::value;
                 constexpr bool CF = decltype(CF_)::value;
                 constexpr bool ZN = decltype(ZN_)::value;
+                constexpr bool AO = decltype(AO_)::value;
                 constexpr int LN = CF ? LB : 1;
                 float4 va[LB], vb[LB], qa[LN], qb[LN];
                 auto issue = [&](float4* v, float4* q, int base) {
@@ -134,14 +169,17 @@
                                 float z[4];
                                 if (nc.zr) { const float4 z4 = Z4[i4]; z[0] = z4.x; z[1] = z4.y; z[2] = z4.z; z[3] = z4.w; }
                                 else philox_normal4(nc.seed, nc.draw_r, nc.b_off + b, (unsigned)i4, z);
-                                const unsigned f0 = *reinterpret_cast<const unsigned short*>(sFrb + k), f1 = *reinterpret_cast<const unsigned short*>(sFrb + k1);
-                                const float fl0 = sFl[e], fl1 = sFl[e1];
-                                const float m[4] = {fl0 * (float)(f0 & 0xffu), fl0 * (float)(f0 >> 8), fl1 * (float)(f1 & 0xffu), fl1 * (float)(f1 >> 8)};
+                                float m[4] = {1.f, 1.f, 1.f, 1.f};
+                                if (!AO) {
+                                    const unsigned f0 = *reinterpret_cast<const unsigned short*>(sFrb + k), f1 = *reinterpret_cast<const unsigned short*>(sFrb + k1);
+                                    const float fl0 = sFl[e], fl1 = sFl[e1];
+                                    m[0] = fl0 * (float)(f0 & 0xffu); m[1] = fl0 * (float)(f0 >> 8); m[2] = fl1 * (float)(f1 & 0xffu); m[3] = fl1 * (float)(f1 >> 8);
+                                }
                                 const float4 n4v = q[CF ? u : 0];
                                 const float nn[4] = {n4v.x, n4v.y, n4v.z, n4v.w};
 #pragma unroll
                                 for (int j = 0; j < 4; ++j) {
-                                    const float zz = z[j] * m[j];
+                                    const float zz = AO ? z[j] : z[j] * m[j];
                                     if (ZN && !CF) s_z = fmaf(zz, zz, s_z);
                                     if (CF) vv[j] = fmaf(c2f, zz, fmaf(c1f, nn[j], vv[j]));
                                 }
@@ -149,7 +187,7 @@
                                     float z2[4];
                                     philox_normal4(na.seed, ra.draw_r2, na.b_off + b, (unsigned)i4, z2);
 #pragma unroll
-                                    for (int j = 0; j < 4; ++j) { const float zz = z2[j] * m[j]; s_z = fmaf(zz, zz, s_z); }
+                                    for (int j = 0; j < 4; ++j) { const float zz = AO ? z2[j] : z2[j] * m[j]; s_z = fmaf(zz, zz, s_z); }
                                 }
                             }
                             *reinterpret_cast<float2*>(sF + e * ldk + k) = make_float2(vv[0], vv[1]);
@@ -159,7 +197,8 @@
                 };
                 const int step = LB * nth;
                 int base = tid;
-                build_tables([&]() { issue(va, qa, base); });
+                build_tables([&]() { if (CF && ST) nsum_load(); issue(va, qa, base); if (CF && ST) nsum_reduce(); });
+                if (CF && ST && nsum) nsum_coef(&c1f, &c2f);
                 while (true) {
                     const bool more_b = base - tid + step < n4;
                     if (more_b) issue(vb, qb, base + step);
@@ -173,12 +212,13 @@
                     base += step;
                 }
             };
-            typedef std::integral_constant<bool, true> T_;
-            typedef std::integral_constant<bool, false> F_;
-            if (ra.cf.on && ra.merge) phase0(std::integral_constant<int, 3>{}, T_{}, T_{});
-            else if (ra.cf.on) phase0(std::integral_constant<int, 3>{}, T_{}, F_{});
-            else if (znorm) phase0(std::integral_constant<int, 3>{}, F_{}, T_{});
-            else phase0(std::integral_constant<int, 3>{}, F_{}, F_{});
+            typedef std::integral_constant<int, 3> LB3;
+            if (allon && ra.cf.on && ra.merge) { if constexpr (ST) phase0(LB3{}, T_{}, T_{}, T_{}); }
+            else if (allon && ra.cf.on) { if constexpr (ST) phase0(LB3{}, T_{}, F_{}, T_{}); }
+            else if (ra.cf.on && ra.merge) phase0(LB3{}, T_{}, T_{}, F_{});
+            else if (ra.cf.on) phase0(LB3{}, T_{}, F_{}, F_{});
+            else if (znorm) phase0(LB3{}, F_{}, T_{}, F_{});
+            else phase0(LB3{}, F_{}, F_{}, F_{});
         } else {
             build_tables([]() {});
             for (int t = tid; t < EK; t += nth) {
@@ -555,9 +595,10 @@
         const unsigned vo = (unsigned)(4 * kq * K + l15);
         const bool cn2 = p.f_cnum == 2;
         float* const outp = ep.out + (size_t)b * E * K;
-        auto coltile = [&](auto MODE_, auto INJ_, int tn) -> f32x4 {
+        auto coltile = [&](auto MODE_, auto INJ_, auto AO_, int tn) -> f32x4 {
             constexpr int MODE = decltype(MODE_)::value;
             constexpr bool INJ = decltype(INJ_)::value;
+            constexpr bool AO = decltype(AO_)::value;
             const float s_ = MODE == 0 ? ep.sscale : MODE == 1 ? 1.f : ep.pb;
             const float sa = s_ * pw.f_alpha, sb = s_ * pw.f_beta, sg = s_ * pw.f_gamma;
             const float pa = ep.pa, pc = ep.pc;
@@ -616,7 +657,7 @@
                 }
             }
             if (nin && !(diag & 4)) {
-                const float fr = (float)sFrb[n];
+                const float fr = AO ? 1.f : (float)sFrb[n];
                 unsigned gi = vo + 16u * (unsigned)tn;
 #pragma unroll
                 for (int i = 0; i < TF; ++i) {
@@ -630,18 +671,22 @@
                             philox_normal4(na.seed, na.draw_r, na.b_off + b, (unsigned)((4 * i + kq) * K + n), z);
                         }
                     }
-                    const float4 fl4 = *reinterpret_cast<const float4*>(sFl + e0);
-                    const float flv[4] = {fl4.x, fl4.y, fl4.z, fl4.w};
+                    float flv[4] = {1.f, 1.f, 1.f, 1.f};
+                    if (!AO) {
+                        const float4 fl4 = *reinterpret_cast<const float4*>(sFl + e0);
+                        flv[0] = fl4.x; flv[1] = fl4.y; flv[2] = fl4.z; flv[3] = fl4.w;
+                    }
 #pragma unroll
                     for (int r = 0; r < 4; ++r) {
                         const float f = bv[4 * i + r];
                         const float m = flv[r] * fr;
-                        const float net = m * fmaf(sb, acc[i][r], fmaf(sa, f, sg));
+                        const float t = fmaf(sb, acc[i][r], fmaf(sa, f, sg));
+                        const float net = AO ? t : m * t;
                         const unsigned g = gi + (unsigned)(r * K);
                         if (MODE == 0) {
                             outp[g] = net;
                         } else {
-                            const float zz = z[r] * m;
+                            const float zz = AO ? z[r] : z[r] * m;
                             if (MODE == 1) {
                                 outp[g] = net;
                                 s_net = fmaf(net, net, s_net);
@@ -660,9 +705,10 @@
             }
             return sacc;
         };
-        auto strip_finish = [&](auto MODE_, auto INJ_, const f32x4& p0, const f32x4& p1, const f32x4& p2, const f32x4& p3, int tn0) {
+        auto strip_finish = [&](auto MODE_, auto INJ_, auto AO_, const f32x4& p0, const f32x4& p1, const f32x4& p2, const f32x4& p3, int tn0) {
             constexpr int MODE = decltype(MODE_)::value;
             constexpr bool INJ = decltype(INJ_)::value;
+            constexpr bool AO = decltype(AO_)::value;
             float hf[4];
 #pragma unroll
             for (int r = 0; r < 4; ++r) {
@@ -682,7 +728,7 @@
                 const float sa = s_ * pw.f_alpha, sb = s_ * pw.f_beta, sg = s_ * pw.f_gamma;
                 const float pa = ep.pa, pc = ep.pc;
                 float* const meanp = MODE == 3 ? ep.mean + (size_t)b * E * K : nullptr;
-                const float fr = (float)sFrb[n];
+                const float fr = AO ? 1.f : (float)sFrb[n];
                 const unsigned gi = (unsigned)(E0 * K + n);
                 float z[4] = {0.f, 0.f, 0.f, 0.f};
                 if ((MODE >= 2 || (MODE == 1 && eznorm)) && !(diag & 8)) {
@@ -694,20 +740,24 @@
                         philox_normal4(na.seed, na.draw_r, na.b_off + b, (unsigned)((E0 >> 2) * K + n), z);
                     }
                 }
-                const float4 fl4 = *reinterpret_cast<const float4*>(sFl + E0);
-                const float flv[4] = {fl4.x, fl4.y, fl4.z, fl4.w};
+                float flv[4] = {1.f, 1.f, 1.f, 1.f};
+                if (!AO) {
+                    const float4 fl4 = *reinterpret_cast<const float4*>(sFl + E0);
+                    flv[0] = fl4.x; flv[1] = fl4.y; flv[2] = fl4.z; flv[3] = fl4.w;
+                }
 #pragma unroll
                 for (int r = 0; r < 4; ++r) {
                     const int e = E0 + r;
                     if (e < E) {
                         const float f = sF[e * ldk + n];
                         const float m = flv[r] * fr;
-                        const float net = m * fmaf(sb, hf[r], fmaf(sa, f, sg));
+                        const float t = fmaf(sb, hf[r], fmaf(sa, f, sg));
+                        const float net = AO ? t : m * t;
                         const unsigned g = gi + (unsigned)(r * K);
                         if (MODE == 0) {
                             outp[g] = net;
                         } else {
-                            const float zz = z[r] * m;
+                            const float zz = AO ? z[r] : z[r] * m;
                             if (MODE == 1) {
                                 outp[g] = net;
                                 s_net = fmaf(net, net, s_net);
@@ -728,7 +778,8 @@
         typedef std::integral_constant<bool, true> Inj;
         const bool inj = na.zr != nullptr && ep.mode != MODE_SCORE;
         const int cmode = ep.mode == MODE_SCORE ? 0 : ep.mode == MODE_NORMS ? 1 : ep.mean == nullptr ? 2 : 3;
-        const int sel = cmode * 2 + (inj ? 1 : 0);
+        enum { SEL_AO_NORMS = 8, SEL_AO_PRED = 9, SEL_AO_PRED_MEAN = 10 };
+        const int sel = (allon && !inj && cmode >= 1) ? SEL_AO_NORMS + (cmode - 1) : cmode * 2 + (inj ? 1 : 0);
         int pt = n1 + (wave + nw - (nHf % nw)) % nw;
         const int pslot = wave < (nw >> 1) ? 0 : 2;
         int cnt = 0;
@@ -739,26 +790,32 @@
             if (diag & 16) continue;
             f32x4 sacc;
             switch (sel) {
-                case 0: case 1: sacc = coltile(std::integral_constant<int, 0>{}, NoInj{}, tn); break;
-                case 2: sacc = coltile(std::integral_constant<int, 1>{}, NoInj{}, tn); break;
-                case 3: sacc = coltile(std::integral_constant<int, 1>{}, Inj{}, tn); break;
-                case 4: sacc = coltile(std::integral_constant<int, 2>{}, NoInj{}, tn); break;
-                case 5: sacc = coltile(std::integral_constant<int, 2>{}, Inj{}, tn); break;
-                case 6: sacc = coltile(std::integral_constant<int, 3>{}, NoInj{}, tn); break;
-                default: sacc = coltile(std::integral_constant<int, 3>{}, Inj{}, tn); break;
+                case 0: case 1: sacc = coltile(std::integral_constant<int, 0>{}, NoInj{}, F_{}, tn); break;
+                case 2: sacc = coltile(std::integral_constant<int, 1>{}, NoInj{}, F_{}, tn); break;
+                case 3: sacc = coltile(std::integral_constant<int, 1>{}, Inj{}, F_{}, tn); break;
+                case 4: sacc = coltile(std::integral_constant<int, 2>{}, NoInj{}, F_{}, tn); break;
+                case 5: sacc = coltile(std::integral_constant<int, 2>{}, Inj{}, F_{}, tn); break;
+                case 6: sacc = coltile(std::integral_constant<int, 3>{}, NoInj{}, F_{}, tn); break;
+                case SEL_AO_NORMS: sacc = coltile(std::integral_constant<int, 1>{}, NoInj{}, T_{}, tn); break;
+                case SEL_AO_PRED: sacc = coltile(std::integral_constant<int, 2>{}, NoInj{}, T_{}, tn); break;
+                case SEL_AO_PRED_MEAN: sacc = coltile(std::integral_constant<int, 3>{}, NoInj{}, T_{}, tn); break;
+                default: sacc = coltile(std::integral_constant<int, 3>{}, Inj{}, F_{}, tn); break;
             }
             const int c4 = cnt & 3;
             if (c4 == 0) sp0 = sacc; else if (c4 == 1) sp1 = sacc; else if (c4 == 2) sp2 = sacc; else sp3 = sacc;
             if (c4 == 3 || tn + nw >= ntn) {
                 const int tn0 = tn - c4 * nw;
                 switch (sel) {
-                    case 0: case 1: strip_finish(std::integral_constant<int, 0>{}, NoInj{}, sp0, sp1, sp2, sp3, tn0); break;
-                    case 2: strip_finish(std::integral_constant<int, 1>{}, NoInj{}, sp0, sp1, sp2, sp3, tn0); break;
-                    case 3: strip_finish(std::integral_constant<int, 1>{}, Inj{}, sp0, sp1, sp2, sp3, tn0); break;
-                    case 4: strip_finish(std::integral_constant<int, 2>{}, NoInj{}, sp0, sp1, sp2, sp3, tn0); break;
-                    case 5: strip_finish(std::integral_constant<int, 2>{}, Inj{}, sp0, sp1, sp2, sp3, tn0); break;
-                    case 6: strip_finish(std::integral_constant<int, 3>{}, NoInj{}, sp0, sp1, sp2, sp3, tn0); break;
-                    default: strip_finish(std::integral_constant<int, 3>{}, Inj{}, sp0, sp1, sp2, sp3, tn0); break;
+                    case 0: case 1: strip_finish(std::integral_constant<int, 0>{}, NoInj{}, F_{}, sp0, sp1, sp2, sp3, tn0); break;
+                    case 2: strip_finish(std::integral_constant<int, 1>{}, NoInj{}, F_{}, sp0, sp1, sp2, sp3, tn0); break;
+                    case 3: strip_finish(std::integral_constant<int, 1>{}, Inj{}, F_{}, sp0, sp1, sp2, sp3, tn0); break;
+                    case 4: strip_finish(std::integral_constant<int, 2>{}, NoInj{}, F_{}, sp0, sp1, sp2, sp3, tn0); break;
+                    case 5: strip_finish(std::integral_constant<int, 2>{}, Inj{}, F_{}, sp0, sp1, sp2, sp3, tn0); break;
+                    case 6: strip_finish(std::integral_constant<int, 3>{}, NoInj{}, F_{}, sp0, sp1, sp2, sp3, tn0); break;
+                    case SEL_AO_NORMS: strip_finish(std::integral_constant<int, 1>{}, NoInj{}, T_{}, sp0, sp1, sp2, sp3, tn0); break;
+                    case SEL_AO_PRED: strip_finish(std::integral_constant<int, 2>{}, NoInj{}, T_{}, sp0, sp1, sp2, sp3, tn0); break;
+                    case SEL_AO_PRED_MEAN: strip_finish(std::integral_constant<int, 3>{}, NoInj{}, T_{}, sp0, sp1, sp2, sp3, tn0); break;
+                    default: strip_finish(std::integral_constant<int, 3>{}, Inj{}, F_{}, sp0, sp1, sp2, sp3, tn0); break;
                 }
                 sp0 = sp1 = sp2 = sp3 = zero4;
             }
diff --git a/ccsd_amd/csrc/ccsd_rank2_common.h b/ccsd_amd/csrc/ccsd_rank2_common.h
--- a/ccsd_amd/csrc/ccsd_rank2_common.h
+++ b/ccsd_amd/csrc/ccsd_rank2_common.h
@@ -202,3 +202,107 @@
     *c1 = step * cf.ss[t];
     *c2 = sqrtf(step * 2.f) * cf.seps;
 }
+CCSD_DEV void corr_coef_sums(const CorrFuse& cf, int t, float gsum, float zsum, float* c1, float* c2) {
+    const float gn = fabsf(cf.ss[t]) * gsum, zn = zsum;
+    const float q = cf.snr * zn / gn;
+    const float step = q * q * 2.f * cf.alpha[t];
+    *c1 = step * cf.ss[t];
+    *c2 = sqrtf(step * 2.f) * cf.seps;
+}
+
+static inline __host__ __device__ int ccsd_normsum_threads(int B) { return B > 512 ? 1024 : B > 256 ? 512 : 256; }
+template <int NV>
+struct NormSumRegs { float x[NV][2]; };
+template <int NV>
+CCSD_DEV void normsums_load(const float* __restrict__ norm2, const float* __restrict__ part, int B, NormSumRegs<NV>& r) {
+#ifdef CCSD_EMU
+    float acc[6] = {0.f, 0.f, 0.f, 0.f, 0.f, 0.f};
+    for (int b = 0; b < B; ++b) {
+        acc[0] += sqrtf(norm2[(size_t)b * 4 + 0]); acc[1] += sqrtf(norm2[(size_t)b * 4 + 1]);
+        acc[3] += sqrtf(norm2[(size_t)b * 4 + 2]); acc[4] += sqrtf(norm2[(size_t)b * 4 + 3]);
+        float sn = 0.f, sz = 0.f;
+        sn += part[(size_t)b * 2 + 0]; sz += part[(size_t)b * 2 + 1];
+        acc[2] += sqrtf(sn); acc[5] += sqrtf(sz);
+    }
+    for (int i = 0; i < NV; ++i) { r.x[i][0] = acc[NV == 6 ? i : 2 + 3 * i]; r.x[i][1] = 0.f; }
+#else
+    const int T = ccsd_normsum_threads(B), nvw = T >> 6, wave = wave_index(), lane = threadIdx.x & 63;
+#pragma unroll
+    for (int s = 0; s < 2; ++s) {
+        const int vw = wave + 8 * s;
+        float acc[6] = {0.f, 0.f, 0.f, 0.f, 0.f, 0.f};
+        if (vw < nvw)
+            for (int b = 64 * vw + lane; b < B; b += T) {
+                if (NV == 6) {
+                    const float4 n4 = *reinterpret_cast<const float4*>(norm2 + (size_t)b * 4);
+                    acc[0] += sqrtf(n4.x);
+                    acc[1] += sqrtf(n4.y);
+                    acc[3] += sqrtf(n4.z);
+                    acc[4] += sqrtf(n4.w);
+                }
+                const float2 p2 = *reinterpret_cast<const float2*>(part + (size_t)b * 2);
+                float sn = 0.f, sz = 0.f;
+                sn += p2.x;
+                sz += p2.y;
+                acc[2] += sqrtf(sn);
+                acc[5] += sqrtf(sz);
+            }
+#pragma unroll
+        for (int i = 0; i < NV; ++i) r.x[i][s] = acc[NV == 6 ? i : 2 + 3 * i];
+    }
+#endif
+}
+template <int NV>
+CCSD_DEV void normsums_reduce(const NormSumRegs<NV>& r, int B, float* red) {
+#ifdef CCSD_EMU
+    (void)B;
+    for (int i = 0; i < NV; ++i) red[i * 16] = r.x[i][0];
+#else
+    const int nvw = ccsd_normsum_threads(B) >> 6, wave = wave_index(), lane = threadIdx.x & 63, row = lane >> 4;
+    float z[NV / 2];
+#pragma unroll
+    for (int j = 0; j < NV / 2; ++j) {
+        float y[2];
+#pragma unroll
+        for (int h = 0; h < 2; ++h) {
+            float a = r.x[2 * j + h][0], c = r.x[2 * j + h][1];
+            lane_swap32(a, c);
+            y[h] = a + c;
+        }
+        lane_swap16(y[0], y[1]);
+        z[j] = y[0] + y[1];
+#pragma unroll
+        for (int o = 8; o > 0; o >>= 1) z[j] += __shfl_xor(z[j], o, 64);
+    }
+    const int vw = wave + 8 * (row >> 1);
+    if ((lane & 15) == 0 && vw < nvw) {
+#pragma unroll
+        for (int j = 0; j < NV / 2; ++j) red[(2 * j + (row & 1)) * 16 + vw] = z[j];
+    }
+#endif
+}
+template <int NV>
+CCSD_DEV float normsums_finish(const float* red, int B) {
+#ifdef CCSD_EMU
+    (void)red; (void)B;
+    return 0.f;
+#else
+    const int nvw = ccsd_normsum_threads(B) >> 6, lane = threadIdx.x & 63;
+    const float* rp = red + (lane < NV ? lane : 0) * 16;
+    float t = 0.f;
+    for (int w = 0; w < nvw; w += 4) {
+        const float4 v = *reinterpret_cast<const float4*>(rp + w);
+        t += v.x; t += v.y; t += v.z; t += v.w;
+    }
+    return t;
+#endif
+}
+CCSD_DEV float normsums_value(float t, const float* red, int i) {
+#ifdef CCSD_EMU
+    (void)t;
+    return red[i * 16];
+#else
+    (void)red;
+    return __int_as_float(__builtin_amdgcn_readlane(__float_as_int(t), i));
+#endif
+}
diff --git a/include/ccsd_hip.h b/include/ccsd_hip.h
--- a/include/ccsd_hip.h
+++ b/include/ccsd_hip.h
@@ -95,7 +95,8 @@
     CCSD_QUERY_TILED_FUSE = 14,
     CCSD_QUERY_EW1_FUSE = 15,
     CCSD_QUERY_H_GENERAL = 16,
-    CCSD_QUERY_GEO_EK = 17
+    CCSD_QUERY_GEO_EK = 17,
+    CCSD_QUERY_R2_SUMS = 18
 };
 int ccsd_plan_query(const ccsd_plan_t* plan, int32_t what, int64_t* value);
 
```
